# srvk/eesen

Measured on AMD Instinct MI355X. Metric: CTC training frames/sec (whole node), 4x512 BiLSTM, higher is better.
Workload: dtype f32

## Files before the change

eesen_amd/csrc/capi.cpp:

```cpp
#include <cstdio>
#include <cstring>

#include <algorithm>

#include "guard.h"
#include "net.h"

using namespace eesen;

#include "handles.h"

namespace eesen {
std::string& last_error_slot() {
  thread_local std::string g_err;
  return g_err;
}
}

extern "C" {

const char* eesen_last_error(void) { return last_error_slot().c_str(); }
const char* eesen_version(void) { return "eesen_hip 0.1.0 (gfx950)"; }

int eesen_device_count(int* count) {
// ... 107 lines not shown
}
int eesen_net_set_train_options(eesen_net_t* net, float learn_rate, float momentum) {
  return guard([&] { REQ_PTR(net); net->lr = learn_rate; net->mmt = momentum; });
}
int eesen_net_set_update_algorithm(eesen_net_t* net, const char* name) {
  return guard([&] {
    REQ_PTR(net); REQ_PTR(name);
    const std::string a(name);
    if (a == "SGD") net->rule = 0;
    else if (a == "Adagrad") net->rule = 1;
    else if (a == "RMSProp") net->rule = 2;
    else throw Error(EESEN_ERR_INVALID, "unknown optimization algorithm '" + a + "' (SGD|Adagrad|RMSProp)");
  });
}
int eesen_net_set_adaptive_options(eesen_net_t* net, float adagrad_epsilon, float rmsprop_rho) {
  return guard([&] { REQ_PTR(net); net->ada_eps = adagrad_epsilon; net->rms_rho = rmsprop_rho; net->rms_one_minus_rho = 1.0f - rmsprop_rho; });
}
int eesen_net_get_accumulators(eesen_net_t* net, float* host_flat, long n) {
  return guard([&] { REQ_PTR(net); REQ_PTR(host_flat); net->init_accu(); net->get_flat(net->accu, host_flat, n); });
}
int eesen_net_set_accumulators(eesen_net_t* net, const float* host_flat, long n) {
  return guard([&] { REQ_PTR(net); REQ_PTR(host_flat); net->set_accu(host_flat, n); });
}
int eesen_net_set_seq_lengths(eesen_net_t* net, const int* lens, int S) {
  return guard([&] { REQ_PTR(net); REQ_PTR(lens); net->set_seq_lengths(lens, S); });
}
int eesen_net_propagate(eesen_net_t* net, const float* in, int rows, int in_ld, int in_is_device, const float** out_dev,
                        int* out_cols, int* out_ld) {
  return guard([&] {
    REQ_PTR(net); REQ_PTR(in);
    net->propagate(in, rows, in_ld, in_is_device != 0);
    if (out_dev) *out_dev = net->out_ptr;
    if (out_cols) *out_cols = net->out_cols;
    if (out_ld) *out_ld = net->out_ld;
  });
}
int eesen_net_get_output(eesen_net_t* net, float* host_out, long n) {
  return guard([&] {
    REQ_PTR(net); REQ_PTR(host_out);
    EESEN_REQUIRE(net->propagated, EESEN_ERR_STATE, "no Propagate output");
    EESEN_REQUIRE(n == (long)net->rows * net->out_cols, EESEN_ERR_INVALID, "output size mismatch");
    net->sync();
    EESEN_HIP_CHECK(hipMemcpy2D(host_out, (size_t)net->out_cols * 4, net->out_ptr, (size_t)net->out_ld * 4, (size_t)net->out_cols * 4,
                                net->rows, hipMemcpyDeviceToHost));
  });
}
int eesen_net_backpropagate(eesen_net_t* net, const float* out_diff_dev, int out_diff_ld, float* in_diff_dev, int in_diff_ld) {
  return guard([&] { REQ_PTR(net); REQ_PTR(out_diff_dev); net->backpropagate(out_diff_dev, out_diff_ld, in_diff_dev, in_diff_ld); });
}
int eesen_net_grad_buffer(eesen_net_t* net, float** dev_ptr, long* n) {
  return guard([&] { REQ_PTR(net); REQ_PTR(dev_ptr); REQ_PTR(n); *dev_ptr = net->fresh.p; *n = (long)net->P; });
}
int eesen_net_get_grads(eesen_net_t* net, float* host_flat, long n) {
  return guard([&] { REQ_PTR(net); REQ_PTR(host_flat); net->get_flat(net->fresh, host_flat, n); });
}
int eesen_net_update(eesen_net_t* net) {
  return guard([&] { REQ_PTR(net); net->update(); });
}
int eesen_net_set_forward_precision(eesen_net_t* net, int bf16) {
  return guard([&] { REQ_PTR(net); net->fwd_bf16 = bf16 != 0; net->fwd_bf16_rec = bf16 == 1; });
}
int eesen_net_bf16_recurrence_layers(eesen_net_t* net, int* layers) {
  return guard([&] { REQ_PTR(net); REQ_PTR(layers); *layers = net->info_fwd_bf16; });
}
int eesen_net_plan_string(eesen_net_t* net, char* json, int cap) {
  return guard([&] {
    REQ_PTR(net); REQ_PTR(json);
    const std::string s = net->plan_string();
    EESEN_REQUIRE(cap > (int)s.size(), EESEN_ERR_INVALID, "eesen_net_plan_string: buffer too small (" + std::to_string(s.size() + 1) + " bytes needed)");
    std::memcpy(json, s.c_str(), s.size() + 1);
  });
}
int eesen_net_recurrence_info(eesen_net_t* net, int* out3) {
  return guard([&] {
    REQ_PTR(net); REQ_PTR(out3);
    out3[0] = net->info_lstm_layers; out3[1] = net->info_fwd_persistent; out3[2] = net->info_bwd_persistent;
    out3[3] = net->recoveries;
  });
}
int eesen_net_debug_set_error_word(eesen_net_t* net, unsigned value) {
  return guard([&] {
    REQ_PTR(net);
    EESEN_HIP_CHECK(hipSetDevice(net->device));
    EESEN_HIP_CHECK(hipMemsetD32Async(reinterpret_cast<hipDeviceptr_t>(net->ctl.p + kCtlWords - 1), (int)value, 1, net->st));
  });
}
int eesen_net_synchronize(eesen_net_t* net) {
  return guard([&] { REQ_PTR(net); net->sync(); });
}
int eesen_net_set_profiling(eesen_net_t* net, int on) {
  return guard([&] { REQ_PTR(net); net->timer.enable(on != 0); net->timer.set_accumulate(on == 2); });
}
int eesen_net_get_phase_spans(eesen_net_t* net, int* phases, float* seconds, int cap, int* n) {
  return guard([&] { REQ_PTR(net); REQ_PTR(n); *n = net->timer.spans(phases, seconds, cap); });
}
int eesen_net_get_phase_times(eesen_net_t* net, float* out6) {
  return guard([&] { REQ_PTR(net); REQ_PTR(out6); net->timer.collect(out6, 6); });
}

int eesen_ctc_create(int device, void* stream, eesen_ctc_t** out) {
  return guard([&] { REQ_PTR(out); *out = new eesen_ctc(device, stream); });
}
int eesen_ctc_destroy(eesen_ctc_t* ctc) {
  return guard([&] { delete ctc; });
}
int eesen_ctc_eval_parallel(eesen_ctc_t* ctc, const int* frame_num_utt, int S, const float* net_out_dev, int rows, int K,
                            int ld, const int* label_ids, const int* label_off, float* diff_dev, int diff_ld,
                            float* pzx_host) {
  return guard([&] {
    REQ_PTR(ctc); REQ_PTR(frame_num_utt); REQ_PTR(net_out_dev); REQ_PTR(label_ids); REQ_PTR(label_off); REQ_PTR(diff_dev);
    ctc->eval_parallel(frame_num_utt, S, net_out_dev, rows, K, ld, label_ids, label_off, diff_dev, diff_ld, pzx_host);
  });
}
int eesen_ctc_error_rate_mseq(eesen_ctc_t* ctc, const int* frame_num_utt, int S, const float* net_out_dev, int rows, int K,
                              int ld, const int* label_ids, const int* label_off, int* num_err, int* num_ref) {
  return guard([&] {
    REQ_PTR(ctc); REQ_PTR(frame_num_utt); REQ_PTR(net_out_dev); REQ_PTR(label_ids); REQ_PTR(label_off);
    ctc->error_rate_mseq(frame_num_utt, S, net_out_dev, rows, K, ld, label_ids, label_off, num_err, num_ref);
  });
}
int eesen_ctc_stats(eesen_ctc_t* ctc, double* obj_sum, long* sequences, long* frames, long* err_tokens, long* ref_tokens) {
  return guard([&] {
    REQ_PTR(ctc);
    ctc->flush();
    if (obj_sum) *obj_sum = ctc->obj_sum;
    if (sequences) *sequences = ctc->sequences;
    if (frames) *frames = ctc->frames;
    if (err_tokens) *err_tokens = ctc->err_tokens;
    if (ref_tokens) *ref_tokens = ctc->ref_tokens;
  });
}
int eesen_ctc_get_alpha_beta(eesen_ctc_t* ctc, float* alpha_host, float* beta_host, int* Lprime) {
  return guard([&] { REQ_PTR(ctc); ctc->get_alpha_beta(alpha_host, beta_host, Lprime); });
}
int eesen_ctc_set_sequence_out_file(eesen_ctc_t* ctc, const char* path) {
  return guard([&] {
    REQ_PTR(ctc);
    ctc->flush();
    ctc->seq_out = path ? path : "";
    if (!ctc->seq_out.empty()) std::remove(ctc->seq_out.c_str());
  });
}
int eesen_ctc_set_guard(eesen_ctc_t* ctc, eesen_net_t* net) {
  return guard([&] {
    REQ_PTR(ctc);
    ctc->flush();
    if (net) EESEN_REQUIRE(net->device == ctc->device && net->st == ctc->st, EESEN_ERR_INVALID, "eesen_ctc_set_guard: the Ctc and the Net must live on the same device and stream");
    if (ctc->guard_net) {
      auto& g = ctc->guard_net->guards;
      g.erase(std::remove(g.begin(), g.end(), static_cast<Ctc*>(ctc)), g.end());
    }
    ctc->guard = net && net->ctl.p ? net->ctl.p + kCtlWords - 1 : nullptr;
    ctc->guard_net = ctc->guard ? net : nullptr;
    if (ctc->guard_net) net->guards.push_back(ctc);
  });
}
int eesen_ctc_dropped(eesen_ctc_t* ctc, long* minibatches) {
  return guard([&] { REQ_PTR(ctc); REQ_PTR(minibatches); ctc->flush(); *minibatches = ctc->dropped; });
}
int eesen_ctc_set_profiling(eesen_ctc_t* ctc, int mode) {
  return guard([&] { REQ_PTR(ctc); ctc->timer.enable(mode == 2); ctc->timer.set_accumulate(mode == 2); });
}
int eesen_ctc_get_phase_times(eesen_ctc_t* ctc, float* out3) {
  return guard([&] { REQ_PTR(ctc); REQ_PTR(out3); ctc->phase_times(out3); });
}

int eesen_ce_create(int device, void* stream, eesen_ce_t** out) {
  return guard([&] { REQ_PTR(out); *out = new eesen_ce(device, stream); });
}
int eesen_ce_destroy(eesen_ce_t* ce) {
  return guard([&] { delete ce; });
}
int eesen_ce_eval_parallel(eesen_ce_t* ce, const int* frame_num_utt, int S, const float* net_out_dev, int rows, int K, int ld,
                           const int* targets_host, float* diff_dev, int diff_ld, double* obj_host) {
  return guard([&] {
    REQ_PTR(ce); REQ_PTR(frame_num_utt); REQ_PTR(net_out_dev); REQ_PTR(targets_host); REQ_PTR(diff_dev);
    ce->eval_parallel(frame_num_utt, S, net_out_dev, rows, K, ld, targets_host, diff_dev, diff_ld, obj_host);
  });
}
int eesen_ce_set_report_step(eesen_ce_t* ce, int report_step) {
  return guard([&] { REQ_PTR(ce); ce->flush(); ce->report_step = report_step; });
}
int eesen_ce_stats(eesen_ce_t* ce, double* obj, long* correct, long* frames, long* sequences) {
  return guard([&] {
    REQ_PTR(ce);
    ce->flush();
    if (obj) *obj = ce->obj;
    if (correct) *correct = ce->correct;
    if (frames) *frames = ce->frames;
    if (sequences) *sequences = ce->sequences;
  });
}
int eesen_ce_report(eesen_ce_t* ce, char* buf, int cap) {
  return guard([&] {
    REQ_PTR(ce); REQ_PTR(buf);
    const std::string s = ce->report();
    EESEN_REQUIRE(cap > (int)s.size(), EESEN_ERR_INVALID, "eesen_ce_report: buffer too small (" + std::to_string(s.size() + 1) + " bytes needed)");
    std::memcpy(buf, s.c_str(), s.size() + 1);
  });
}
int eesen_ce_progress(eesen_ce_t* ce, int wait, char* buf, int cap) {
  return guard([&] {
    REQ_PTR(ce); REQ_PTR(buf);
    EESEN_REQUIRE(cap > 0, EESEN_ERR_INVALID, "eesen_ce_progress: no buffer");
    if (wait) ce->flush();
    if (ce->progress.empty()) { buf[0] = 0; return; }
    const std::string& s = ce->progress.front();
    EESEN_REQUIRE(cap > (int)s.size(), EESEN_ERR_INVALID, "eesen_ce_progress: buffer too small (" + std::to_string(s.size() + 1) + " bytes needed)");
    std::memcpy(buf, s.c_str(), s.size() + 1);
    ce->progress.erase(ce->progress.begin());
  });
}
int eesen_ce_set_guard(eesen_ce_t* ce, eesen_net_t* net) {
  return guard([&] {
    REQ_PTR(ce);
    ce->flush();
    if (net) EESEN_REQUIRE(net->device == ce->device && net->st == ce->st, EESEN_ERR_INVALID, "eesen_ce_set_guard: the CE and the Net must live on the same device and stream");
    if (ce->guard_net) {
      auto& g = ce->guard_net->ce_guards;
      g.erase(std::remove(g.begin(), g.end(), static_cast<CeLoss*>(ce)), g.end());
    }
    ce->guard = net && net->ctl.p ? net->ctl.p + kCtlWords - 1 : nullptr;
    ce->guard_net = ce->guard ? net : nullptr;
    if (ce->guard_net) net->ce_guards.push_back(ce);
  });
}
int eesen_ce_dropped(eesen_ce_t* ce, long* minibatches) {
  return guard([&] { REQ_PTR(ce); REQ_PTR(minibatches); ce->flush(); *minibatches = ce->dropped; });
}
int eesen_ce_set_profiling(eesen_ce_t* ce, int mode) {
  return guard([&] { REQ_PTR(ce); ce->timer.enable(mode == 2); ce->timer.set_accumulate(mode == 2); });
}
int eesen_ce_get_phase_times(eesen_ce_t* ce, float* out1) {
  return guard([&] { REQ_PTR(ce); REQ_PTR(out1); ce->phase_times(out1); });
}

int eesen_dev_alloc(int device, long bytes, void** dev_ptr) {
  return guard([&] {
    REQ_PTR(dev_ptr);
    EESEN_HIP_CHECK(hipSetDevice(device));
    EESEN_HIP_CHECK(hipMalloc(dev_ptr, (size_t)bytes));
  });
}
int eesen_dev_free(int device, void* dev_ptr) {
  return guard([&] {
    EESEN_HIP_CHECK(hipSetDevice(device));
    EESEN_HIP_CHECK(hipFree(dev_ptr));
  });
}
int eesen_dev_copy(int device, void* dst, const void* src, long bytes, int kind) {
  return guard([&] {
    EESEN_HIP_CHECK(hipSetDevice(device));
    const hipMemcpyKind k = kind == 1 ? hipMemcpyHostToDevice : kind == 2 ? hipMemcpyDeviceToHost : hipMemcpyDeviceToDevice;
    EESEN_HIP_CHECK(hipMemcpy(dst, src, (size_t)bytes, k));
  });
}

int eesen_op_gemm(int device, void* stream, int a_kc, int b_kc, int M, int N, int K, float alpha, const float* A, int lda,
                  const float* B, int ldb, float beta, float* C, int ldc, const float* bias) {
  return guard([&] {
    EESEN_HIP_CHECK(hipSetDevice(device));
    hipStream_t st = reinterpret_cast<hipStream_t>(stream);
    DevBuf<float> ws;
    ws.reserve((size_t)8 << 20);
    gemm_f32(st, a_kc != 0, b_kc != 0, M, N, K, alpha, A, lda, B, ldb, beta, C, ldc, bias, ws.p, ws.cap);
    EESEN_HIP_CHECK(hipStreamSynchronize(st));
  });
}

int eesen_op_gemm_async(int device, void* stream, int a_kc, int b_kc, int M, int N, int K, const float* A, int lda, const float* B, int ldb,
                        float* C, int ldc, float* ws, long ws_floats, int extra_lds_bytes) {
  return guard([&] {
    REQ_PTR(A); REQ_PTR(B); REQ_PTR(C);
    EESEN_REQUIRE(ws_floats >= 0 && (ws || ws_floats == 0) && extra_lds_bytes >= 0, EESEN_ERR_INVALID, "bad workspace / LDS cap");
    EESEN_HIP_CHECK(hipSetDevice(device));
    gemm_f32(reinterpret_cast<hipStream_t>(stream), a_kc != 0, b_kc != 0, M, N, K, 1.f, A, lda, B, ldb, 0.f, C, ldc, nullptr, ws, (size_t)ws_floats,
             extra_lds_bytes);
  });
}

int eesen_op_log_sub_prior(int device, void* stream, float* m_dev, int rows, int cols, int ld, int apply_log,
                           const float* log_priors_host, float prior_scale) {
  return guard([&] {
    REQ_PTR(m_dev);
    EESEN_HIP_CHECK(hipSetDevice(device));
    hipStream_t st = reinterpret_cast<hipStream_t>(stream);
    DevBuf<float> pri;
    if (log_priors_host) {
      pri.reserve(cols);
      EESEN_HIP_CHECK(hipMemcpyAsync(pri.p, log_priors_host, sizeof(float) * cols, hipMemcpyHostToDevice, st));
    }
    log_sub_prior(st, m_dev, ld, rows, cols, apply_log != 0, log_priors_host ? pri.p : nullptr, prior_scale);
    EESEN_HIP_CHECK(hipStreamSynchronize(st));
  });
}

int eesen_op_gemm_bench(int device, int a_kc, int b_kc, int M, int N, int K, const float* A, int lda, const float* B, int ldb,
                        float* C, int ldc, int iters, float* avg_ms) {
  return guard([&] {
    REQ_PTR(avg_ms);
    EESEN_HIP_CHECK(hipSetDevice(device));
    DevBuf<float> ws;
    ws.reserve((size_t)16 << 20);
    hipEvent_t e0, e1;
    EESEN_HIP_CHECK(hipEventCreate(&e0));
// ... 34 lines not shown
```

eesen_amd/csrc/comm.cpp:

```cpp
#include <arpa/inet.h>
#include <dlfcn.h>
#include <netdb.h>
#include <netinet/in.h>
#include <netinet/tcp.h>
#include <sys/socket.h>
#include <unistd.h>

#include <algorithm>
#include <atomic>
#include <chrono>
#include <condition_variable>
#include <cstring>
#include <deque>
#include <mutex>
#include <thread>

#include <rccl/rccl.h>

#include "guard.h"
#include "handles.h"
#include "net.h"

namespace eesen {

// ... 339 lines not shown
      double v[kScratch] = {0};
      if (rank >= base && rank < base + n) v[rank - base] = mine;
      allreduce_host(v, n, 0);
      ids.insert(ids.end(), v, v + n);
    }
    std::vector<double> uniq(ids);
    std::sort(uniq.begin(), uniq.end());
    const int distinct = (int)(std::unique(uniq.begin(), uniq.end()) - uniq.begin());
    std::string o = "{\"library\": \"" + rccl().path + "\", \"rccl_version\": " + std::to_string(version) + ", \"stand_in\": " + (rccl().stand_in ? "true" : "false") +
                    ", \"rank\": " + std::to_string(rank) + ", \"world\": " + std::to_string(world) + ", \"world_seen\": " + std::to_string(seen) +
                    ", \"rank_seen\": " + std::to_string(nccl_rank) + ", \"device\": " + std::to_string(device) + ", \"device_seen\": " + std::to_string(nccl_dev) + ", \"devices\": [";
    for (int r = 0; r < world; ++r) {
      const unsigned long long u = (unsigned long long)(ids[r] - 1.0);
      char t[64];
      snprintf(t, sizeof(t), "%s\"%05x/%04x:%02x:%02x.%x\"", r ? ", " : "", (unsigned)((u >> 32) & 0xfffffu), (unsigned)((u >> 16) & 0xffffu), (unsigned)((u >> 8) & 0xffu),
               (unsigned)((u >> 3) & 0x1fu), (unsigned)(u & 7u));
      o += t;
    }
    o += "], \"distinct_devices\": " + std::to_string(distinct) + ", \"ranks_share_devices\": " + (distinct < world ? "true" : "false") + "}";
    return o;
  }
  void abort_now(const std::string& why) {
    std::unique_lock<std::mutex> lk(mu);
    if (dead.load()) return;
    dead_msg = "data-parallel exchange aborted on rank " + std::to_string(rank) + ": " + why;
    fprintf(stderr, "ERROR (eesen_hip) %s\n", dead_msg.c_str());
    dead.store(true, std::memory_order_release);
    ncclComm_t c = comm;
    comm = nullptr;
    lk.unlock();
    if (rccl().CommAbort && c) (void)rccl().CommAbort(c);
  }
};

void comm_check_alive(const Comm* c) {
  if (c) c->check_alive();
}

void Net::set_comm(Comm* c) {
  EESEN_REQUIRE(finalized, EESEN_ERR_STATE, "net not finalized");
  EESEN_REQUIRE(!c || c->device == device, EESEN_ERR_INVALID, "communicator and net live on different devices");
  wait_buckets_host();
  comm = c;
  if (c && !tn.spin_limit_set) spin_limit = std::max(spin_limit, 4000000);
  if (c && ev_ready.size() < layers.size()) {
    EESEN_HIP_CHECK(hipSetDevice(device));
    const size_t old = ev_ready.size();
    ev_ready.resize(layers.size(), nullptr);
    ev_bucket.resize(layers.size(), nullptr);
    for (size_t i = old; i < layers.size(); ++i) {
      EESEN_HIP_CHECK(hipEventCreateWithFlags(&ev_ready[i], hipEventDisableTiming));
      EESEN_HIP_CHECK(hipEventCreateWithFlags(&ev_bucket[i], hipEventDisableTiming));
    }
  }
  bucket_pending.assign(layers.size(), 0);
}

int Net::top_trainable() const {
  for (int li = (int)layers.size() - 1; li >= 0; --li)
    if (layers[li].p_n) return li;
  return -1;
}

void Net::bucket_allreduce(int li, hipStream_t producer) {
  if (!comm || !layers[li].p_n) return;
  bucket_log.push_back(li);
  EESEN_HIP_CHECK(hipEventRecord(ev_ready[li], producer));
  if (exchange_deferred) { deferred_buckets.push_back(li); return; }
  issue_bucket(li);
}

void Net::flush_deferred_buckets() {
  if (!comm || deferred_buckets.empty()) return;
  if (!ev_bwd_done) EESEN_HIP_CHECK(hipEventCreateWithFlags(&ev_bwd_done, hipEventDisableTiming));
  EESEN_HIP_CHECK(hipEventRecord(ev_bwd_done, st));
  EESEN_HIP_CHECK(hipStreamWaitEvent(comm->st, ev_bwd_done, 0));
  for (int li : deferred_buckets) issue_bucket(li);
  deferred_buckets.clear();
}

void Net::issue_bucket(int li) {
  EESEN_HIP_CHECK(hipStreamWaitEvent(comm->st, ev_ready[li], 0));
  const bool top = li == top_trainable();
  if (ctl.p) zero_if_set(comm->st, fresh.p + layers[li].p_off, (long)(layers[li].p_n + (top ? kLiveWords : 0)), ctl.p + kCtlWords - 1);
  grads_sanitized = true;
  const int ti_ = timer.begin(comm->st, 6);
  comm->allreduce_f32(fresh.p + layers[li].p_off, layers[li].p_n + (top ? kLiveWords : 0), comm->st);
  timer.end(comm->st, ti_);
  EESEN_HIP_CHECK(hipEventRecord(ev_bucket[li], comm->st));
  bucket_pending[li] = 1;
}

void Net::fail_step_buckets() noexcept {
  if (!comm) return;
  try {
    EESEN_HIP_CHECK(hipSetDevice(device));
    std::vector<char> logged(layers.size(), 0);
    for (int li : bucket_log) logged[li] = 1;
    flush_deferred_buckets();
    if (!ev_bwd_done) EESEN_HIP_CHECK(hipEventCreateWithFlags(&ev_bwd_done, hipEventDisableTiming));
    for (hipStream_t s : {st, st2}) {
      if (!s) continue;
      EESEN_HIP_CHECK(hipEventRecord(ev_bwd_done, s));
      EESEN_HIP_CHECK(hipStreamWaitEvent(comm->st, ev_bwd_done, 0));
    }
    const int top = top_trainable();
    for (int li = (int)layers.size() - 1; li >= 0; --li) {
      if (!layers[li].p_n || logged[li]) continue;
      const size_t n = layers[li].p_n + (li == top ? kLiveWords : 0);
      EESEN_HIP_CHECK(hipMemsetAsync(fresh.p + layers[li].p_off, 0, n * sizeof(float), comm->st));
      bucket_log.push_back(li);
      EESEN_HIP_CHECK(hipEventRecord(ev_ready[li], comm->st));
      issue_bucket(li);
    }
    fprintf(stderr, "WARNING (eesen_hip) Backpropagate failed on this rank in a data-parallel step: its unfinished gradient buckets were "
                    "all-reduced as zeros so that the other ranks are not left waiting\n");
  } catch (...) {
    try { comm->abort_now("Backpropagate failed and the step's remaining gradient buckets could not be issued"); } catch (...) {}
  }
}

void Net::wait_buckets_host() {
  if (!comm) return;
  bool any = false;
  for (char p : bucket_pending) any |= p != 0;
  if (any) EESEN_HIP_CHECK(hipStreamSynchronize(comm->st));
  comm->check_alive();
}

void Net::backpropagate_zero() {
  EESEN_REQUIRE(finalized, EESEN_ERR_STATE, "net not finalized");
  comm_check_alive(comm);
  EESEN_HIP_CHECK(hipSetDevice(device));
  if (P) EESEN_HIP_CHECK(hipMemsetAsync(fresh.p, 0, (P + kLiveWords) * sizeof(float), st));
  bucket_log.clear();
  deferred_buckets.clear();
  exchange_deferred = false;
  live_valid = comm != nullptr;
  for (int li = (int)layers.size() - 1; li >= 0; --li) bucket_allreduce(li, st);
  flush_deferred_buckets();
}

int Net::live_ranks() {
  EESEN_REQUIRE(finalized && comm, EESEN_ERR_STATE, "live_ranks needs an attached communicator");
  comm->check_alive();
  EESEN_HIP_CHECK(hipSetDevice(device));
  const int top = top_trainable();
  EESEN_REQUIRE(top >= 0, EESEN_ERR_STATE, "the net has no trainable layer");
  if (bucket_pending[top]) EESEN_HIP_CHECK(hipStreamWaitEvent(st, ev_bucket[top], 0));
  if (!live_pin) EESEN_HIP_CHECK(hipHostMalloc(reinterpret_cast<void**>(&live_pin), sizeof(float), hipHostMallocDefault));
  EESEN_HIP_CHECK(hipMemcpyAsync(live_pin, fresh.p + P, sizeof(float), hipMemcpyDeviceToHost, st));
  EESEN_HIP_CHECK(hipStreamSynchronize(st));
  comm->check_alive();
  return (int)(*live_pin + 0.5f);
}

void Net::allreduce_grads(Comm* c) {
  EESEN_REQUIRE(finalized, EESEN_ERR_STATE, "net not finalized");
  EESEN_REQUIRE(c && c->device == device, EESEN_ERR_INVALID, "communicator missing or on another device");
  EESEN_HIP_CHECK(hipSetDevice(device));
  if (ctl.p) zero_if_set(st, fresh.p, (long)P, ctl.p + kCtlWords - 1);
  grads_sanitized = true;
  c->allreduce_f32(fresh.p, P, st);
}

}

using namespace eesen;
struct eesen_comm : public Comm { using Comm::Comm; };

extern "C" {

int eesen_comm_get_unique_id(char* id128) {
  return guard([&] {
    REQ_PTR(id128);
    ncclUniqueId id;
    EESEN_NCCL_CHECK(rccl().GetUniqueId(&id));
    std::memcpy(id128, id.internal, NCCL_UNIQUE_ID_BYTES);
  });
}
int eesen_comm_exchange(const char* addr, int port, int rank, int world, char* buf, int nbytes, int timeout_s) {
  return guard([&] { REQ_PTR(buf); comm_exchange(addr, port, rank, world, buf, nbytes, timeout_s); });
}
int eesen_comm_create(int device, const char* id128, int rank, int world, eesen_comm_t** out) {
  return guard([&] { REQ_PTR(id128); REQ_PTR(out); *out = new eesen_comm(device, id128, rank, world); });
}
int eesen_comm_create_tcp(int device, const char* addr, int port, int rank, int world, int timeout_s, eesen_comm_t** out) {
  return guard([&] {
    REQ_PTR(out);
    char id[NCCL_UNIQUE_ID_BYTES] = {0};
    if (rank == 0) {
      ncclUniqueId u;
      EESEN_NCCL_CHECK(rccl().GetUniqueId(&u));
      std::memcpy(id, u.internal, NCCL_UNIQUE_ID_BYTES);
    }
    comm_exchange(addr, port, rank, world, id, NCCL_UNIQUE_ID_BYTES, timeout_s);
    *out = new eesen_comm(device, id, rank, world);
  });
}
int eesen_comm_destroy(eesen_comm_t* comm) {
  return guard([&] { delete comm; });
}
int eesen_comm_info(eesen_comm_t* comm, int* rank, int* world) {
  return guard([&] { REQ_PTR(comm); if (rank) *rank = comm->rank; if (world) *world = comm->world; });
}
int eesen_comm_describe(eesen_comm_t* comm, char* json, int cap) {
  return guard([&] {
    REQ_PTR(comm); REQ_PTR(json);
    const std::string s = comm->describe();
    EESEN_REQUIRE(cap > (int)s.size(), EESEN_ERR_INVALID, "eesen_comm_describe: buffer too small (" + std::to_string(s.size() + 1) + " bytes needed)");
    std::memcpy(json, s.c_str(), s.size() + 1);
  });
}
int eesen_comm_allreduce_host(eesen_comm_t* comm, double* values, int n, int op) {
  return guard([&] { REQ_PTR(comm); REQ_PTR(values); comm->allreduce_host(values, n, op); });
}
int eesen_net_set_comm(eesen_net_t* net, eesen_comm_t* comm) {
  return guard([&] { REQ_PTR(net); net->set_comm(comm); });
}
int eesen_net_allreduce_grads(eesen_net_t* net, eesen_comm_t* comm) {
  return guard([&] { REQ_PTR(net); net->allreduce_grads(comm); });
}
int eesen_net_backpropagate_zero(eesen_net_t* net) {
  return guard([&] { REQ_PTR(net); net->backpropagate_zero(); });
}
int eesen_net_live_ranks(eesen_net_t* net, int* live) {
  return guard([&] { REQ_PTR(net); REQ_PTR(live); *live = net->live_ranks(); });
}
int eesen_net_bucket_order(eesen_net_t* net, int* layers_out, int cap, int* n) {
  return guard([&] {
    REQ_PTR(net); REQ_PTR(n);
    *n = (int)net->bucket_log.size();
    for (int i = 0; i < *n && i < cap && layers_out; ++i) layers_out[i] = net->bucket_log[i];
  });
}

}
```

eesen_amd/csrc/gemm.hip:

```cpp
#include <cstring>
#include <mutex>
#include <type_traits>

#include "kernels.h"

namespace eesen {
namespace {

constexpr int BM = 128, BN = 128, BK = 16, LDP = 4;
constexpr int NLD = BM * BK / 4 / 256;
constexpr int KQ_BITS = BK == 16 ? 2 : 3;
typedef float f32x16 __attribute__((ext_vector_type(16)));

struct GemmParams {
  const float* A;
  const float* B;
  float* C;
  const float* bias;
  int M, N, K;
  int lda, ldb, ldc;
  float alpha, beta;
  int splits;
  int k_chunk;
  int tiles_n;
// ... 633 lines not shown
      unsigned m0 = 0u, m1 = 0u;
#pragma unroll
      for (int j = 0; j < 8; ++j) {
        v[j].x &= 0x7fffffffu; v[j].y &= 0x7fffffffu; v[j].z &= 0x7fffffffu; v[j].w &= 0x7fffffffu;
        const unsigned mj = max(max(v[j].x, v[j].y), max(v[j].z, v[j].w));
        if (j < 4) m0 = max(m0, mj); else m1 = max(m1, mj);
        if (COLS) { uint4& q = cm[j & 3]; q.x = max(q.x, v[j].x); q.y = max(q.y, v[j].y); q.z = max(q.z, v[j].z); q.w = max(q.w, v[j].w); }
      }
      if (ROWS || ALL) {
#pragma unroll
        for (int o = 32; o > 0; o >>= 1) { m0 = max(m0, (unsigned)__shfl_xor((int)m0, o)); m1 = max(m1, (unsigned)__shfl_xor((int)m1, o)); }
        if (ROWS && lane == 0) {
          if (nslab > 1 || row_acc) { atomicMax(&out_rows[r], m0); if (two) atomicMax(&out_rows[r + rstep], m1); }
          else { out_rows[r] = m0; if (two) out_rows[r + rstep] = m1; }
        }
        all = max(all, max(m0, m1));
      }
    }
    if (COLS) {
#pragma unroll
      for (int j = 0; j < 4; ++j) {
        const int c = c0 + 256 * j;
        if (c < C) { atomicMax(&smax[c], cm[j].x); atomicMax(&smax[c + 1], cm[j].y); atomicMax(&smax[c + 2], cm[j].z); atomicMax(&smax[c + 3], cm[j].w); }
      }
    }
  } else {
    for (long r = (long)blockIdx.x * kAmaxWaves + wave; r < R; r += (long)gridDim.x * kAmaxWaves) {
      const float* row = P + r * ld;
      unsigned m = 0u;
      for (int c = lane; c < C; c += 64) {
        const unsigned v = __builtin_bit_cast(unsigned, row[c]) & 0x7fffffffu;
        m = max(m, v);
        if (COLS) atomicMax(&smax[c], v);
      }
      if (ROWS || ALL) {
#pragma unroll
        for (int o = 32; o > 0; o >>= 1) m = max(m, (unsigned)__shfl_xor((int)m, o));
        if (ROWS && lane == 0) { if (row_acc) atomicMax(&out_rows[r], m); else out_rows[r] = m; }
        all = max(all, m);
      }
    }
  }
  if (COLS) {
    __syncthreads();
    for (int c = tid; c < Cp; c += kAmaxWaves * 64) part_cols[(size_t)blockIdx.x * Cp + c] = smax[c];
  }
  if (ALL) {
    unsigned* red = smax + (COLS ? Cp : 0);
    __syncthreads();
    if (lane == 0) red[wave] = all;
    __syncthreads();
    if (tid == 0) {
      unsigned m = 0u;
      for (int w = 0; w < kAmaxWaves; ++w) m = max(m, red[w]);
      if (m) atomicMax(out_all, m);
    }
  }
}
__global__ __launch_bounds__(256) void amax_fold_kernel(const unsigned* __restrict__ part, int nb, int Cp, int C, unsigned* __restrict__ out) {
  __shared__ uint4 red[16][16];
  const int cq = threadIdx.x & 15, g = threadIdx.x >> 4;
  const int c = blockIdx.x * 64 + cq * 4;
  uint4 m = make_uint4(0u, 0u, 0u, 0u);
  if (c < Cp)
    for (int b = g; b < nb; b += 16 * 8) {
      uint4 v[8];
#pragma unroll
      for (int k = 0; k < 8; ++k) v[k] = b + 16 * k < nb ? *reinterpret_cast<const uint4*>(part + (size_t)(b + 16 * k) * Cp + c) : make_uint4(0u, 0u, 0u, 0u);
#pragma unroll
      for (int k = 0; k < 8; ++k) { m.x = max(m.x, v[k].x); m.y = max(m.y, v[k].y); m.z = max(m.z, v[k].z); m.w = max(m.w, v[k].w); }
    }
  red[g][cq] = m;
  __syncthreads();
  if (g == 0 && c < Cp) {
#pragma unroll
    for (int k = 1; k < 16; ++k) { const uint4 o = red[k][cq]; m.x = max(m.x, o.x); m.y = max(m.y, o.y); m.z = max(m.z, o.z); m.w = max(m.w, o.w); }
    if (c + 0 < C) out[c + 0] = m.x;
    if (c + 1 < C) out[c + 1] = m.y;
    if (c + 2 < C) out[c + 2] = m.z;
    if (c + 3 < C) out[c + 3] = m.w;
  }
}

__global__ __launch_bounds__(256) void splitk_reduce_kernel(const float* __restrict__ ws, int splits, int M, int N,
                                                            float alpha, float beta, float* __restrict__ C, int ldc,
                                                            const float* __restrict__ bias) {
  const size_t total = (size_t)M * N;
  for (size_t i = (size_t)blockIdx.x * blockDim.x + threadIdx.x; i < total; i += (size_t)gridDim.x * blockDim.x) {
    float s = 0.f;
    for (int k = 0; k < splits; ++k) s += ws[(size_t)k * total + i];
    const int row = (int)(i / N), col = (int)(i % N);
    float v = alpha * s + (bias ? bias[col] : 0.f);
    float* dst = C + (size_t)row * ldc + col;
    if (beta != 0.f) v += beta * *dst;
    *dst = v;
  }
}

}

static int g_gemm_mode = -1;
int gemm_mode() {
  if (g_gemm_mode >= 0) return g_gemm_mode;
  const char* e = getenv("EESEN_GEMM_MODE");
  if (e && (!strcmp(e, "f32") || !strcmp(e, "0"))) return 0;
  if (e && (!strcmp(e, "split") || !strcmp(e, "1"))) return 1;
  if (e && (!strcmp(e, "half") || !strcmp(e, "2"))) return 2;
  return kDefaultGemmMode;
}
void set_gemm_mode(int mode) { g_gemm_mode = mode; }

void amax_abs(hipStream_t st, const float* P, long rows, int cols, int ld, float* out) {
  EESEN_HIP_CHECK(hipMemsetAsync(out, 0, sizeof(float), st));
  amax_abs_accumulate(st, P, rows, cols, ld, out);
}
static int amax_blocks(long rows, int slabs) { return (int)std::max<long>(1, std::min<long>((rows * slabs + 2 * kAmaxWaves - 1) / (2 * kAmaxWaves), kAmaxBlocks)); }
#define EESEN_AMAX_LAUNCH(R_, C_, A_, LDS)                                                                                                        \
  do {                                                                                                                                            \
    if (vec) hipLaunchKernelGGL((amax_kernel<R_, C_, A_, true>), dim3(nb), dim3(kAmaxWaves * 64), LDS, st, Pc, rows, cc, ld, r, w, a, racc);     \
    else hipLaunchKernelGGL((amax_kernel<R_, C_, A_, false>), dim3(nb), dim3(kAmaxWaves * 64), LDS, st, Pc, rows, cc, ld, r, w, a, racc);        \
  } while (0)
constexpr int kAmaxSlabCols = 16384;
void amax_abs_accumulate(hipStream_t st, const float* P, long rows, int cols, int ld, float* out) {
  if (rows <= 0 || cols <= 0) return;
  if (cols == ld && cols < 1024 && (rows * cols) % 1024 == 0) { rows = rows * cols / 1024; cols = ld = 1024; }
  unsigned *r = nullptr, *w = nullptr, *a = reinterpret_cast<unsigned*>(out);
  const int racc = 0;
  const bool vec = (cols & 3) == 0 && (ld & 3) == 0;
  for (int c0 = 0; c0 < cols; c0 += kAmaxSlabCols) {
    const float* Pc = P + c0;
    const int cc = std::min(kAmaxSlabCols, cols - c0), nb = amax_blocks(rows, vec ? (cc + 1023) / 1024 : 1);
    EESEN_AMAX_LAUNCH(false, false, true, kAmaxWaves * sizeof(unsigned));
  }
  check_launch("amax_abs");
}
void amax_rows_cols(hipStream_t st, const float* P, long rows, int cols, int ld, float* out_rows, float* out_cols, float* ws) {
  if (rows <= 0 || cols <= 0) return;
  EESEN_REQUIRE(!out_cols || ws, EESEN_ERR_INVALID, "amax: column bounds need a workspace");
  unsigned* r = reinterpret_cast<unsigned*>(out_rows);
  unsigned* w = reinterpret_cast<unsigned*>(ws);
  unsigned* a = nullptr;
  const bool vec = (cols & 3) == 0 && (ld & 3) == 0;
  const bool multi = out_rows && ((vec && cols > 1024) || cols > kAmaxSlabCols);
  if (multi) EESEN_HIP_CHECK(hipMemsetAsync(out_rows, 0, (size_t)rows * sizeof(float), st));
  for (int c0 = 0; c0 < cols; c0 += kAmaxSlabCols) {
    const float* Pc = P + c0;
    const int cc = std::min(kAmaxSlabCols, cols - c0), racc = multi ? 1 : 0;
    const int nb = amax_blocks(rows, vec ? (cc + 1023) / 1024 : 1);
    const int cp = (cc + 3) & ~3;
    if (out_rows && out_cols) EESEN_AMAX_LAUNCH(true, true, false, (size_t)cp * sizeof(unsigned));
    else if (out_cols) EESEN_AMAX_LAUNCH(false, true, false, (size_t)cp * sizeof(unsigned));
    else if (out_rows) EESEN_AMAX_LAUNCH(true, false, false, 0);
    check_launch("amax_rows_cols");
    if (out_cols) {
      hipLaunchKernelGGL(amax_fold_kernel, dim3((cp + 63) / 64), dim3(256), 0, st, w, nb, cp, cc, reinterpret_cast<unsigned*>(out_cols) + c0);
      check_launch("amax_fold");
    }
  }
}
#undef EESEN_AMAX_LAUNCH

static GemmBound arena_bound(hipStream_t st, const float* P, bool kc, int R, int K, int ld) {
  constexpr size_t kArena = (size_t)4 << 20, kDevs = 16;
  static std::mutex mu;
  static float* arena[kDevs] = {nullptr};
  static size_t next[kDevs] = {0};
  int dev = 0;
  EESEN_HIP_CHECK(hipGetDevice(&dev));
  EESEN_REQUIRE(dev >= 0 && dev < (int)kDevs, EESEN_ERR_INVALID, "gemm: device index beyond the bounds arena table");
  const size_t need = ((size_t)R + 3) & ~(size_t)3;
  EESEN_REQUIRE(need <= kArena / 8, EESEN_ERR_INVALID, "gemm: operand too large for the bounds arena");
  float* slot;
  {
    std::lock_guard<std::mutex> lk(mu);
    if (!arena[dev]) EESEN_HIP_CHECK(hipMalloc(reinterpret_cast<void**>(&arena[dev]), kArena * sizeof(float)));
    if (next[dev] + need > kArena) next[dev] = 0;
    slot = arena[dev] + next[dev];
    next[dev] += need;
  }
  if (kc) amax_rows_cols(st, P, R, K, ld, slot, nullptr, nullptr);
  else {
    float* ws = nullptr;
    EESEN_HIP_CHECK(hipMallocAsync(reinterpret_cast<void**>(&ws), (size_t)kAmaxBlocks * std::min<size_t>(need, kAmaxSlabCols) * sizeof(float), st));
    amax_rows_cols(st, P, K, R, ld, nullptr, slot, ws);
    EESEN_HIP_CHECK(hipFreeAsync(ws, st));
  }
  return GemmBound{slot, 1};
}

static int xcd_group_rows(int tiles_m, int tiles_n, unsigned* grid_x) {
  if (tiles_m < 8) return 0;
  int gm = 8;
  while (gm > 1 && cdiv(tiles_m, gm) < 16) gm >>= 1;
  const long groups = cdiv(tiles_m, gm), rounds = cdivl(groups, 8);
  const long gx = rounds * 8 * gm * tiles_n;
  if (gx > 0x7fffffffL) return 0;
  *grid_x = (unsigned)gx;
  return gm;
}

void gemm_f32(hipStream_t st, bool a_kc, bool b_kc, int M, int N, int K, float alpha, const float* A, int lda,
              const float* B, int ldb, float beta, float* C, int ldc, const float* bias, float* ws, size_t ws_floats,
              int extra_lds_bytes, bool bf16_operands, GemmBound bound_a, GemmBound bound_b) {
  if (M <= 0 || N <= 0) return;
  EESEN_REQUIRE((lda % 4) == 0 && (ldb % 4) == 0, EESEN_ERR_INVALID, "gemm: leading dimensions must be multiples of 4");
  EESEN_REQUIRE((((uintptr_t)A | (uintptr_t)B) & 15) == 0, EESEN_ERR_INVALID, "gemm: operands must be 16-byte aligned");
  const bool use_split = gemm_mode() >= 1 || bf16_operands;
  const bool half = gemm_mode() == 2 && !bf16_operands;
  GemmParams p;
  p.amax_a = p.amax_b = nullptr;
  p.a_vec = p.b_vec = 0;
  if (half) {
    if (!bound_a.p) bound_a = arena_bound(st, A, a_kc, M, K, lda);
    if (!bound_b.p) bound_b = arena_bound(st, B, b_kc, N, K, ldb);
    p.amax_a = bound_a.p; p.a_vec = bound_a.per_index;
    p.amax_b = bound_b.p; p.b_vec = bound_b.per_index;
  }
  p.A = A; p.B = B; p.C = C; p.bias = bias;
  p.M = M; p.N = N; p.K = K; p.lda = lda; p.ldb = ldb; p.ldc = ldc;
  p.alpha = alpha; p.beta = beta;
  p.gate = GemmGate{nullptr, nullptr, 0, 0, 0, 0, 0, 0};
  p.nprod = bf16_operands ? 1 : 6;
  const bool big = use_split && !bf16_operands && extra_lds_bytes == 0 && M % 256 == 0 && N % 256 == 0 && K % 16 == 0 &&
                   (long)(M / 256) * (N / 256) >= 16;
  const int TB = big ? 256 : BM;
  p.bm = p.bn = TB;
  const int tiles_m = cdiv(M, TB), tiles_n = cdiv(N, TB);
  p.tiles_n = tiles_n;
  p.tiles_m = tiles_m;
  const long tiles = (long)tiles_m * tiles_n;
  int splits = 1;
  const int target = big ? 256 : 1024;
  if (ws && tiles < target && K >= 2048) {
    splits = (int)std::min<long>((target + tiles - 1) / tiles, K / 1024);
    splits = std::max(1, std::min(splits, 64));
    while (splits > 1 && (size_t)splits * M * N > ws_floats) --splits;
  }
  int k_chunk = cdiv(cdiv(K, splits), 16) * 16;
  if (k_chunk < BK) k_chunk = BK;
  splits = std::max(1, cdiv(K, k_chunk));
  p.splits = splits;
  p.k_chunk = k_chunk;
  if (splits > 1) p.C = ws;
// ... 74 lines not shown
```

eesen_amd/csrc/kernels.h:

```cpp
#pragma once
#include "common.h"

namespace eesen {

struct GemmBound {
  const float* p = nullptr;
  int per_index = 0;
};
void gemm_f32(hipStream_t st, bool a_kc, bool b_kc, int M, int N, int K, float alpha, const float* A, int lda,
              const float* B, int ldb, float beta, float* C, int ldc, const float* bias, float* ws,
              size_t ws_floats, int extra_lds_bytes = 0,
              bool bf16_operands = false,
              GemmBound bound_a = {}, GemmBound bound_b = {});

constexpr int kDefaultGemmMode = 2;
int gemm_mode();
void set_gemm_mode(int mode);
void amax_abs(hipStream_t st, const float* P, long rows, int cols, int ld, float* out);
void amax_abs_accumulate(hipStream_t st, const float* P, long rows, int cols, int ld, float* out);
constexpr int kAmaxBlocks = 512;
void amax_rows_cols(hipStream_t st, const float* P, long rows, int cols, int ld, float* out_rows, float* out_cols, float* ws);

#ifndef EESEN_SHARDS
#define EESEN_SHARDS 8
#endif
constexpr int kShards = EESEN_SHARDS, kShardStride = 32;
constexpr int kCtlHalf = 2048 * kShards;

struct GemmGate {
  const unsigned* cnt;
  unsigned* err;
  int ndir, nz, nblk;
  int T, S;
  int spin_limit;
};
void gemm_f32_nt_gated(hipStream_t st, int M, int N, int K, const float* A, int lda, const float* B, int ldb, float* C,
                       int ldc, const float* bias, const GemmGate& gate, GemmBound bound_a = {}, GemmBound bound_b = {});

struct LstmLayerDev {
  int T, S, H, ndir;
  float* G;
  float* C;
  float* Y;
  float* X = nullptr;
  const float* Wm;
  const float* WmT;
  const float* peep;
  const int* lens;
  const float* rmask = nullptr;
  int drop_mode = 0;
  int s_begin = 0, s_count = 0;
  float* PX = nullptr;
  size_t px_floats = 0;
  int poll_delay = 0;
  int poll_raw = 0;
  unsigned* milestone = nullptr;
  int milestone_step = 0;
  int xcd_map = 1, fwd_mux = 1, bwd_q4 = 1, bwd_ksplit = 1, bwd_mux = 1;
  int fwd_t16_small = 1;
  int fwd_narrow2 = 1;
  int bwd_q4_st8 = 1;
  int fwd_bf16 = 0;
  int fwd_split = 0;
  int fwd_f16 = 0;
  const float* wm_amax = nullptr;
  int bwd_f16 = 0;
  unsigned char* DGH = nullptr;
  float* EX = nullptr;
};
float handoff_flight_ns();
void set_gpu_share(int n);
int gpu_share_value();
void wait_for_word(hipStream_t st, const unsigned* word, unsigned target, unsigned* err, double limit_s = 2.0);
void lstm_fwd_step(hipStream_t st, const LstmLayerDev& L, int step);
void lstm_bwd_step(hipStream_t st, const LstmLayerDev& L, int step, const float* dY, int lddy, float* DG, float* DCF);
void dropout_mask(hipStream_t st, float* out, long rows, int cols, int ld, float p, unsigned long long seed, bool per_column);
void activation_rows(hipStream_t st, bool tanh_, const float* x, int ldx, float* y, int ldy, long rows, int cols);
void activation_diff_rows(hipStream_t st, bool tanh_, const float* y, int ldy, float* d, int ldd, long rows, int cols);
void mul_elements(hipStream_t st, const float* a, int lda, const float* m, int ldm, float* out, int ldo, long rows, int cols);
enum { kRecNone = 0, kRecFwdBf = 1, kRecFwdMux = 2, kRecFwdF32 = 3, kRecBwdQ4 = 4, kRecBwdKsplit = 5, kRecBwdKsplitMux = 6, kRecBwdGeneric = 7 };
struct RecPlan {
  int kind = kRecNone;
  const char* kernel = "";
  int seq_tile = 0;
  int units = 0;
  int windows = 0;
  int grid[3] = {0, 0, 0};
  int wgs = 0;
  int wgs_per_cu = 0;
  int vgprs = 0, lds = 0;
  int free_vgprs = -1;
  int seq_tiles = 1;
  bool one_window = false;
  bool leaves_room = false;
  bool bf16 = false;
  bool light = false;
  size_t need_px = 0, need_ex = 0;
  bool need_dgh = false;
  size_t ctl_words = 0;
  int chunk = 0;
  const void* fn = nullptr;
};
RecPlan lstm_fwd_plan(const LstmLayerDev& L);
RecPlan lstm_bwd_plan(const LstmLayerDev& L);
void lstm_fwd_launch(hipStream_t st, const RecPlan& plan, const LstmLayerDev& L, unsigned* cnt, unsigned* err, int spin_limit,
                     unsigned long long* trace = nullptr, hipEvent_t after_reset = nullptr);
void lstm_bwd_launch(hipStream_t st, const RecPlan& plan, const LstmLayerDev& L, const float* dY, int lddy, float* DG, unsigned* cnt,
                     unsigned* err, int spin_limit, unsigned long long* trace = nullptr);
void lstm_bias_peep_grads(hipStream_t st, const LstmLayerDev& L, const float* DG, float* bias_grad, float* peep_grad,
                          float* ws, size_t ws_floats);
size_t lstm_bias_peep_ws_floats(int T, int S, int H, int ndir);

void col_sums(hipStream_t st, const float* M, int rows, int cols, int ld, float* out, float* ws, size_t ws_floats);
size_t col_sums_ws_floats(int rows, int cols);

void softmax_rows(hipStream_t st, const float* x, int ldx, float* y, int ldy, int rows, int K);
void log_rows(hipStream_t st, const float* in, int ldi, float* out, int ldo, int rows, int K);
void ctc_alpha_beta(hipStream_t st, const float* logp, int ld, int T, int S, int Lpad, const int* labx, const int* lens,
                    const int* lablens, float* alpha, float* beta, float* pzx, int waves = 0);
int ctc_sweep_waves(int Lpad, int waves = 0);
void ctc_error_diff(hipStream_t st, const float* probs, int ld, int T, int S, int K, int Lpad, int Lmax, const int* lens,
                    const int* lablens, const int* labx, const float* alpha, const float* beta,
                    const float* pzx, float* diff, int ldd);
void log_sub_prior(hipStream_t st, float* m, int ld, int rows, int K, bool apply_log, const float* log_prior, float prior_scale);
void row_argmax(hipStream_t st, const float* m, int ld, int rows, int K, int* ids);

struct CeSums {
  double obj;
  long long correct;
};
int ce_eval_blocks(int rows);
void ce_eval(hipStream_t st, const float* y, int ld, int rows, int K, int S, const int* lens, const int* tgt, float* diff,
             int ldd, CeSums* part, CeSums* out);

void sgd_update(hipStream_t st, float* param, float* corr, const float* fresh, long n, float mmt, float lr_coef,
                float max_grad, const unsigned* skip = nullptr, const float* live = nullptr);
void zero_if_set(hipStream_t st, float* p, long n, const unsigned* word);
void adaptive_update(hipStream_t st, float* param, float* corr, const float* fresh, float* accu, long n, float mmt, float lr,
                     float max_grad, float eps, float rho, float one_minus_rho, bool rmsprop, const unsigned* skip = nullptr,
                     const float* live = nullptr);
void tensor_moments(hipStream_t st, const float* base, long rows, int cols, long ld, double* out6, double* ws,
                    int nb = 0, int hf = 0, int hi = 0);
void transpose2d(hipStream_t st, const float* src, int rows, int cols, float* dst);
void copy2d(hipStream_t st, const float* src, int lds, float* dst, int ldd, int rows, int cols);

}
```

eesen_amd/csrc/net.cpp:

```cpp
#include "net.h"

#include <algorithm>
#include <cmath>
#include <cstdio>
#include <cstring>

namespace eesen {


PhaseTimer::~PhaseTimer() {
  for (auto& s : spans_) {
    (void)hipEventDestroy(s.a);
    (void)hipEventDestroy(s.b);
  }
}
int PhaseTimer::begin(hipStream_t st, int phase) {
  if (!on_) return -1;
  if (used_ == spans_.size()) {
    Span s;
    EESEN_HIP_CHECK(hipEventCreate(&s.a));
    EESEN_HIP_CHECK(hipEventCreate(&s.b));
    spans_.push_back(s);
  }
  spans_[used_].phase = phase;
// ... 8 lines not shown
  for (int i = 0; i < nphase; ++i) out[i] = 0.f;
  for (size_t i = 0; i < used_; ++i) {
    EESEN_HIP_CHECK(hipEventSynchronize(spans_[i].b));
    float ms = 0.f;
    EESEN_HIP_CHECK(hipEventElapsedTime(&ms, spans_[i].a, spans_[i].b));
    if (spans_[i].phase >= 0 && spans_[i].phase < nphase) out[spans_[i].phase] += ms * 1e-3f;
  }
  if (accumulate_) used_ = 0;
}

int PhaseTimer::spans(int* phases, float* secs, int cap) {
  for (size_t i = 0; i < used_ && (int)i < cap; ++i) {
    EESEN_HIP_CHECK(hipEventSynchronize(spans_[i].b));
    float ms = 0.f;
    EESEN_HIP_CHECK(hipEventElapsedTime(&ms, spans_[i].a, spans_[i].b));
    if (phases) phases[i] = spans_[i].phase;
    if (secs) secs[i] = ms * 1e-3f;
  }
  return (int)used_;
}

long Layer::file_params() const {
  if (is_lstm()) return (long)ndir * ((long)4 * Hf * din_f + (long)4 * Hf * Hf + 4 * Hf + 3 * Hf);
  if (kind == EESEN_LAYER_AFFINE) return (long)dout_f * din_f + dout_f;
  return 0;
}

const char* Layer::marker() const {
  switch (kind) {
    case EESEN_LAYER_BILSTM_PARALLEL: return nonparallel ? "<BiLstm>" : "<BiLstmParallel>";
    case EESEN_LAYER_LSTM_PARALLEL: return nonparallel ? "<Lstm>" : "<LstmParallel>";
    case EESEN_LAYER_AFFINE: return "<AffineTransform>";
    case EESEN_LAYER_SOFTMAX: return "<Softmax>";
    case EESEN_LAYER_SIGMOID: return "<Sigmoid>";
    case EESEN_LAYER_TANH: return "<Tanh>";
  }
  return "<Unknown>";
}

template <class F>
static void for_each_param(const Layer& L, F f) {
  long fi = 0;
  if (L.is_lstm()) {
    const int H = L.H, Hf = L.Hf, D = L.din_f, D4 = pad4(L.din);
    for (int dir = 0; dir < L.ndir; ++dir) {
      for (int r = 0; r < 4 * Hf; ++r) {
        const int q = r / Hf, u = r % Hf;
        for (int d = 0; d < D; ++d) f(fi++, L.off_wx + ((size_t)dir * 4 * H + u * 4 + q) * D4 + L.in_col(d));
      }
      for (int r = 0; r < 4 * Hf; ++r) {
        const int q = r / Hf, u = r % Hf;
        for (int k = 0; k < Hf; ++k) f(fi++, L.off_wm + ((size_t)dir * 4 * H + u * 4 + q) * H + k);
      }
      for (int r = 0; r < 4 * Hf; ++r) f(fi++, L.off_bias + (size_t)dir * 4 * H + (r % Hf) * 4 + r / Hf);
      for (int g = 0; g < 3; ++g)
        for (int u = 0; u < Hf; ++u) f(fi++, L.off_peep + ((size_t)dir * 3 + g) * H + u);
    }
  } else if (L.kind == EESEN_LAYER_AFFINE) {
    const int D4 = pad4(L.din);
    for (int r = 0; r < L.dout; ++r)
      for (int d = 0; d < L.din_f; ++d) f(fi++, L.off_w + (size_t)r * D4 + L.in_col(d));
    for (int r = 0; r < L.dout; ++r) f(fi++, L.off_b + r);
  }
}

Net::Net(int dev, void* stream) : device(dev) {
  int n = 0;
  hipError_t e = hipGetDeviceCount(&n);
  if (e != hipSuccess || n <= 0)
    throw Error(EESEN_ERR_HIP, "no HIP device available: this library has no CPU fallback (hipGetDeviceCount: " +
                                   std::string(e == hipSuccess ? "0 devices" : hipGetErrorString(e)) + ")");
  EESEN_REQUIRE(dev >= 0 && dev < n, EESEN_ERR_INVALID, "device index out of range");
  EESEN_HIP_CHECK(hipSetDevice(dev));
  st = reinterpret_cast<hipStream_t>(stream);
  int lo = 0, hi = 0;
  EESEN_HIP_CHECK(hipDeviceGetStreamPriorityRange(&lo, &hi));
  EESEN_HIP_CHECK(hipStreamCreateWithPriority(&st2, hipStreamNonBlocking, lo));
  EESEN_HIP_CHECK(hipEventCreateWithFlags(&ev_rec, hipEventDisableTiming));
  for (auto& e : ev_grad) EESEN_HIP_CHECK(hipEventCreateWithFlags(&e, hipEventDisableTiming));
  EESEN_HIP_CHECK(hipEventCreateWithFlags(&ev_gate_reset, hipEventDisableTiming));
  EESEN_HIP_CHECK(hipEventCreateWithFlags(&ev_gate_done, hipEventDisableTiming));
  tn = Tuning::from_env();
  persistent = tn.persistent;
  gate_fwd = tn.gate_fwd >= 0 ? tn.gate_fwd != 0 : gemm_mode() == 0;
  overlap = tn.overlap >= 0 ? tn.overlap != 0 : persistent != 0;
  spin_limit = tn.spin_limit;
  if (tn.trace) {
    trace.reserve(1280);
    EESEN_HIP_CHECK(hipMemset(trace.p, 0, 1280 * sizeof(unsigned long long)));
  }
  ctl.reserve(kCtlWords);
  EESEN_HIP_CHECK(hipMemset(ctl.p, 0, kCtlWords * sizeof(unsigned)));
  {
    constexpr float kFwdNs = 400.f, kBwdNs = 280.f, kBwdSideNs = 420.f, kRefFlightNs = 400.f;
    flight_ns = handoff_flight_ns();
    const float fscale = flight_ns >= 300.f && flight_ns <= 700.f ? 1.f : flight_ns / kRefFlightNs;
    auto ticks = [&](float ns) { return std::min(300, std::max(0, (int)std::lround(fscale * ns / 10.f))); };
    delay_fwd = ticks(kFwdNs); delay_bwd = ticks(kBwdNs); delay_bwd_side = ticks(kBwdSideNs);
    if (const char* e = tn.poll_ns) {
      int a = -1, b2 = -1;
      if (sscanf(e, "%d,%d", &a, &b2) == 2) { delay_fwd = a / 10; delay_bwd = delay_bwd_side = b2 / 10; poll_raw = 1; }
    }
    if (tn.print_flight)
      fprintf(stderr, "eesen_hip: increment flight %.0f ns; first-poll delays forward %d0, backward %d0 (beside side-stream GEMMs %d0) ns\n", flight_ns, delay_fwd, delay_bwd, delay_bwd_side);
  }
}

Net::~Net() {
  (void)hipSetDevice(device);
  (void)hipStreamSynchronize(st);
  for (Ctc* c : guards) {
    (void)hipStreamSynchronize(c->st);
    c->guard = nullptr;
    c->guard_net = nullptr;
  }
  for (CeLoss* c : ce_guards) {
    (void)hipStreamSynchronize(c->st);
    c->guard = nullptr;
    c->guard_net = nullptr;
  }
  if (trace.p) {
    std::vector<unsigned long long> h(1280);
    if (hipMemcpy(h.data(), trace.p, h.size() * 8, hipMemcpyDeviceToHost) == hipSuccess)
      for (int pass = 0; pass < 2; ++pass) {
        double seg[5] = {0, 0, 0, 0, 0};
        int n = 0;
        for (int s = 8; s < 120; ++s) {
          const unsigned long long* a = h.data() + pass * 640 + s * 5;
          if (!a[0] || !a[5]) continue;
          seg[0] += (double)(a[1] - a[0]); seg[1] += (double)(a[2] - a[1]); seg[2] += (double)(a[3] - a[2]);
          seg[3] += (double)(a[4] - a[3]); seg[4] += (double)(a[5] - a[4]);
          ++n;
        }
        if (n) fprintf(stderr, "EESEN_TRACE %s: wait %.0f | A-load+MFMA+reduce %.0f | epilogue %.0f | drain+barrier %.0f | publish->next %.0f ticks/step (%d steps)\n",
                       pass ? "bwd" : "fwd", seg[0] / n, seg[1] / n, seg[2] / n, seg[3] / n, seg[4] / n, n);
      }
  }
  if (lens_pin) (void)hipHostFree(lens_pin);
  if (err_pin) (void)hipHostFree(err_pin);
  if (live_pin) (void)hipHostFree(live_pin);
  for (auto& h : in_stage) { if (h.p) (void)hipHostFree(h.p); if (h.ev) (void)hipEventDestroy(h.ev); }
  if (lens_ev) (void)hipEventDestroy(lens_ev);
  if (err_ev) (void)hipEventDestroy(err_ev);
  if (st2) { (void)hipStreamSynchronize(st2); (void)hipStreamDestroy(st2); }
  if (ev_rec) (void)hipEventDestroy(ev_rec);
  for (auto& e : ev_grad) if (e) (void)hipEventDestroy(e);
  if (ev_gate_reset) (void)hipEventDestroy(ev_gate_reset);
  if (ev_gate_done) (void)hipEventDestroy(ev_gate_done);
  for (auto& e : ev_ready) if (e) (void)hipEventDestroy(e);
  for (auto& e : ev_bucket) if (e) (void)hipEventDestroy(e);
  if (ev_bwd_done) (void)hipEventDestroy(ev_bwd_done);
  if (own_stream) (void)hipStreamDestroy(st);
}

void Net::sync() {
  EESEN_HIP_CHECK(hipSetDevice(device));
  EESEN_HIP_CHECK(hipStreamSynchronize(st));
  wait_buckets_host();
  comm_check_alive(comm);
  check_device_error(true);
}

void Net::check_device_error(bool consumer) {
  if (!ctl.p) return;
  unsigned e = 0;
  EESEN_HIP_CHECK(hipMemcpy(&e, ctl.p + kCtlWords - 1, sizeof(unsigned), hipMemcpyDeviceToHost));
  if (!e) { steps_since_clean = 0; return; }
  EESEN_HIP_CHECK(hipStreamSynchronize(st));
  EESEN_HIP_CHECK(hipMemset(ctl.p + kCtlWords - 1, 0, sizeof(unsigned)));
  const bool only_waiter = e == 2 && tn.fwd_mid;
  if (only_waiter) tn.fwd_mid = 0;
  else { persistent = 0; gate_fwd = false; overlap = false; }
  ++recoveries;
  const int lost = std::max(1, steps_since_clean);
  steps_since_clean = 0;
  const bool rerun = consumer && propagated && input.p && rows > 0;
  const char* what = comm ? "contributed a ZERO gradient to the data-parallel sum (the ranks' models stay identical)" : "were NOT applied";
  if (only_waiter)
    fprintf(stderr, "WARNING (eesen_hip) the side stream's wait for a forward-recurrence milestone gave up (kernels serialised by a tool?): "
                    "%d minibatch(es) in flight %s%s; continuing without the early input GEMM (EESEN_FWD_MID=0)\n", lost, what,
            rerun ? " and the last forward pass is re-run" : "");
  else
    fprintf(stderr, "WARNING (eesen_hip) a persistent recurrence kernel gave up waiting for a peer workgroup (GPU shared or preempted?): "
                    "%d minibatch(es) in flight %s%s; continuing with the one-launch-per-step kernels\n", lost, what,
            rerun ? " and the last forward pass is re-run" : "");
  if (rerun) {
    forward_pass();
    EESEN_HIP_CHECK(hipStreamSynchronize(st));
  }
}

void Net::arm_device_error_poll() {
  if (!ctl.p) return;
  if (!err_pin) {
    EESEN_HIP_CHECK(hipHostMalloc(reinterpret_cast<void**>(&err_pin), sizeof(unsigned), hipHostMallocDefault));
    *err_pin = 0;
    EESEN_HIP_CHECK(hipEventCreateWithFlags(&err_ev, hipEventDisableTiming));
  }
  EESEN_HIP_CHECK(hipMemcpyAsync(err_pin, ctl.p + kCtlWords - 1, sizeof(unsigned), hipMemcpyDeviceToHost, st));
  EESEN_HIP_CHECK(hipEventRecord(err_ev, st));
  err_armed = true;
}

void Net::poll_device_error() {
  if (!err_armed || hipEventQuery(err_ev) != hipSuccess) return;
  err_armed = false;
  if (*err_pin) check_device_error(false);
  else steps_since_clean = 0;
}

void Net::add_layer(int kind, int din, int dout, float coef, float max_grad) {
  EESEN_REQUIRE(!finalized, EESEN_ERR_STATE, "net already finalized");
  EESEN_REQUIRE(din > 0 && dout > 0, EESEN_ERR_INVALID, "layer dimensions must be positive");
  const Layer* prev = layers.empty() ? nullptr : &layers.back();
  if (prev)
    EESEN_REQUIRE(prev->dout_f == din, EESEN_ERR_INVALID, "Dimensionality mismatch between consecutive layers");
  Layer L;
  L.kind = kind; L.coef = coef; L.max_grad = max_grad;
  L.din_f = din; L.dout_f = dout;
  L.din = prev ? prev->dout : din;
  if (prev) { L.in_nb = prev->out_nb; L.in_hf = prev->out_hf; L.in_hi = prev->out_hi; }
  L.dout = dout;
  const char* sees_pad = "directly on an LSTM layer whose cell count per direction is not a multiple of 4 is not supported: it would see the "
                         "zero cells the library pads such a layer with";
  switch (kind) {
    case EESEN_LAYER_BILSTM_PARALLEL:
      EESEN_REQUIRE(dout % 2 == 0, EESEN_ERR_INVALID, "<CellDim> of a BiLstm layer must be even");
      L.ndir = 2; L.Hf = dout / 2;
      break;
    case EESEN_LAYER_LSTM_PARALLEL:
      L.ndir = 1; L.Hf = dout;
      break;
    case EESEN_LAYER_AFFINE:
      break;
    case EESEN_LAYER_SOFTMAX:
      EESEN_REQUIRE(din == dout, EESEN_ERR_INVALID, "Softmax needs InputDim == OutputDim");
      if (L.in_nb) throw Error(EESEN_ERR_INVALID, std::string("a <Softmax> ") + sees_pad);
      break;
    case EESEN_LAYER_SIGMOID:
    case EESEN_LAYER_TANH:
      EESEN_REQUIRE(din == dout, EESEN_ERR_INVALID, "an activation layer needs InputDim == OutputDim");
      if (L.in_nb && kind == EESEN_LAYER_SIGMOID) throw Error(EESEN_ERR_INVALID, std::string("a <Sigmoid> ") + sees_pad + " (sigmoid(0) = 1/2)");
      L.dout = L.din;
      L.out_nb = L.in_nb; L.out_hf = L.in_hf; L.out_hi = L.in_hi;
      break;
    default:
      throw Error(EESEN_ERR_INVALID, "unsupported layer kind " + std::to_string(kind));
  }
  if (L.is_lstm()) {
    L.H = pad4(L.Hf);
    L.dout = L.ndir * L.H;
    if (L.H != L.Hf) { L.out_nb = L.ndir; L.out_hf = L.Hf; L.out_hi = L.H; }
  }
  layers.push_back(std::move(L));
}

void Net::finalize() {
  EESEN_REQUIRE(!finalized, EESEN_ERR_STATE, "net already finalized");
  EESEN_REQUIRE(!layers.empty(), EESEN_ERR_INVALID, "empty net");
  EESEN_HIP_CHECK(hipSetDevice(device));
  size_t off = 0;
  for (Layer& L : layers) {
    L.p_off = off;
    size_t n = 0;
    if (L.is_lstm()) {
      const size_t H = L.H, D4 = pad4(L.din), nd = L.ndir;
      L.off_wx = n;   n += nd * 4 * H * D4;
      L.off_bias = n; n += nd * 4 * H;
      L.off_wm = n;   n += nd * 4 * H * H;
      L.off_peep = n; n += nd * 3 * H;
      L.WmT.reserve(nd * H * 4 * H);
    } else if (L.kind == EESEN_LAYER_AFFINE) {
      L.off_w = n; n += (size_t)L.dout * pad4(L.din);
      L.off_b = n; n += pad4(L.dout);
    }
    L.p_n = (n + 3) & ~(size_t)3;
    off += L.p_n;
  }
  P = off;
  if (P) {
    params.reserve(P); corr.reserve(P); fresh.reserve(P + kLiveWords);
    EESEN_HIP_CHECK(hipMemsetAsync(params.p, 0, P * sizeof(float), st));
    EESEN_HIP_CHECK(hipMemsetAsync(corr.p, 0, P * sizeof(float), st));
    EESEN_HIP_CHECK(hipMemsetAsync(fresh.p, 0, (P + kLiveWords) * sizeof(float), st));
  }
  if (tn.overlap < 0)
    for (const Layer& L : layers)
      if (L.is_lstm() && L.H > 512) overlap = false;
  amax.reserve(1 + layers.size());
  EESEN_HIP_CHECK(hipMemsetAsync(amax.p, 0, amax.cap * sizeof(float), st));
  EESEN_HIP_CHECK(hipMemsetD32Async(reinterpret_cast<hipDeviceptr_t>(amax.p), 0x3f800000, 1, st));
  finalized = true;
  refresh_derived();
  sync();
}

void Net::measure(const float* Pm, long nrows, int cols, int ld, DevBuf<float>& out_rows, DevBuf<float>& out_cols) {
  out_rows.reserve((size_t)nrows);
  out_cols.reserve((size_t)cols);
  amax_ws.reserve((size_t)kAmaxBlocks * std::min(16384, (cols + 3) & ~3));
  amax_rows_cols(st, Pm, nrows, cols, ld, out_rows.p, out_cols.p, amax_ws.p);
}
bool Net::x_is_bounded(int li) const {
  if (li == 0) return false;
  const Layer& Pv = layers[li - 1];
  return (Pv.is_lstm() && !Pv.cur_fwd_drop) || Pv.is_activation() || Pv.kind == EESEN_LAYER_SOFTMAX;
}
void Net::ensure_weight_amax() {
  const bool mode2 = gemm_mode() == 2;
  const bool need_w = mode2 && !wamax_valid;
  if (wm_valid && !need_w) return;
  if (!wm_valid) EESEN_HIP_CHECK(hipMemsetAsync(am_wm(0), 0, layers.size() * sizeof(float), st));
  for (size_t li = 0; li < layers.size(); ++li) {
    Layer& L = layers[li];
    if (L.is_lstm()) {
      if (need_w) measure(params.p + L.p_off + L.off_wx, (long)L.ndir * 4 * L.H, pad4(L.din), pad4(L.din), L.bw.rows, L.bw.cols);
      if (!wm_valid) amax_abs_accumulate(st, params.p + L.p_off + L.off_wm, (long)L.ndir * 4 * L.H, L.H, L.H, am_wm((int)li));
    } else if (L.kind == EESEN_LAYER_AFFINE && need_w) measure(params.p + L.p_off + L.off_w, L.dout, pad4(L.din), pad4(L.din), L.bw.rows, L.bw.cols);
  }
  wm_valid = true;
  if (mode2) wamax_valid = true;
}

long Net::num_params() const {
  long n = 0;
  for (const Layer& L : layers) n += L.file_params();
  return n;
}

void Net::init_accu() {
  if (accu_init) return;
  accu.reserve(P);
  EESEN_HIP_CHECK(hipMemsetAsync(accu.p, 0, P * sizeof(float), st));
  accu_init = true;
}

void Net::refresh_derived() {
  wamax_valid = wm_valid = false;
  for (Layer& L : layers)
    if (L.is_lstm())
      for (int dir = 0; dir < L.ndir; ++dir)
        transpose2d(st, params.p + L.p_off + L.off_wm + (size_t)dir * 4 * L.H * L.H, 4 * L.H, L.H,
                    L.WmT.p + (size_t)dir * L.H * 4 * L.H);
}

int Net::tensor_moments(int which, int layer, double* out6_host, int cap_tensors) {
  EESEN_REQUIRE(finalized, EESEN_ERR_STATE, "net not finalized");
  EESEN_REQUIRE(layer >= 0 && layer < (int)layers.size(), EESEN_ERR_INVALID, "layer index out of range");
  EESEN_REQUIRE(which >= 0 && which <= 2, EESEN_ERR_INVALID, "which: 0 parameters, 1 momentum buffers, 2 accumulators");
  const Layer& L = layers[layer];
  struct Region { size_t off; long rows; int cols; long ld; int nb, hf, hi; };
  std::vector<Region> reg;
  if (L.is_lstm()) {
    const int H = L.H, Hf = L.Hf, D4 = pad4(L.din);
    for (int dir = 0; dir < L.ndir; ++dir) {
      reg.push_back({L.off_wx + (size_t)dir * 4 * H * D4, 4L * Hf, L.din_f, D4, L.in_nb, L.in_hf, L.in_hi});
      reg.push_back({L.off_wm + (size_t)dir * 4 * H * H, 4L * Hf, Hf, H, 0, 0, 0});
      reg.push_back({L.off_bias + (size_t)dir * 4 * H, 1, 4 * Hf, 4L * H, 0, 0, 0});
      for (int g = 0; g < 3; ++g) reg.push_back({L.off_peep + ((size_t)dir * 3 + g) * H, 1, Hf, H, 0, 0, 0});
    }
  } else if (L.kind == EESEN_LAYER_AFFINE) {
    reg.push_back({L.off_w, L.dout, L.din_f, pad4(L.din), L.in_nb, L.in_hf, L.in_hi});
    reg.push_back({L.off_b, 1, L.dout, L.dout, 0, 0, 0});
  }
  const int n = (int)reg.size();
  if (!out6_host || n == 0) return n;
  EESEN_REQUIRE(cap_tensors >= n, EESEN_ERR_INVALID, "moments buffer too small");
  EESEN_HIP_CHECK(hipSetDevice(device));
  if (which == 2) init_accu();
  sync();
  const float* base = (which == 0 ? params.p : which == 1 ? corr.p : accu.p) + L.p_off;
  DevBuf<double> d;
  d.reserve((size_t)n * 6 + 8);
  for (int i = 0; i < n; ++i)
    eesen::tensor_moments(st, base + reg[i].off, reg[i].rows, reg[i].cols, reg[i].ld, d.p + (size_t)i * 6, d.p + (size_t)n * 6, reg[i].nb, reg[i].hf, reg[i].hi);
  EESEN_HIP_CHECK(hipStreamSynchronize(st));
  EESEN_HIP_CHECK(hipMemcpy(out6_host, d.p, (size_t)n * 6 * sizeof(double), hipMemcpyDeviceToHost));
  return n;
}

static void upload_flat(Net& net, DevBuf<float>& dst, const float* host, long n) {
  EESEN_REQUIRE(net.finalized, EESEN_ERR_STATE, "net not finalized");
  EESEN_REQUIRE(n == net.num_params(), EESEN_ERR_INVALID, "parameter count mismatch");
  EESEN_HIP_CHECK(hipSetDevice(net.device));
  std::vector<float> h(net.P, 0.f);
  long base = 0;
  for (const Layer& L : net.layers) {
    for_each_param(L, [&](long fi, size_t io) { h[L.p_off + io] = host[base + fi]; });
    base += L.file_params();
  }
  net.sync();
  if (net.P) EESEN_HIP_CHECK(hipMemcpy(dst.p, h.data(), net.P * sizeof(float), hipMemcpyHostToDevice));
}

void Net::set_params(const float* host, long n) {
  upload_flat(*this, params, host, n);
  refresh_derived();
  sync();
}

void Net::set_accu(const float* host, long n) {
  init_accu();
  upload_flat(*this, accu, host, n);
}

void Net::get_flat(const DevBuf<float>& buf, float* host, long n) {
  EESEN_REQUIRE(finalized, EESEN_ERR_STATE, "net not finalized");
  EESEN_REQUIRE(n == num_params(), EESEN_ERR_INVALID, "parameter count mismatch");
  sync();
  std::vector<float> h(P);
  if (P) EESEN_HIP_CHECK(hipMemcpy(h.data(), buf.p, P * sizeof(float), hipMemcpyDeviceToHost));
  long base = 0;
  for (const Layer& L : layers) {
    for_each_param(L, [&](long fi, size_t io) { host[base + fi] = h[L.p_off + io]; });
    base += L.file_params();
  }
}

void Net::set_seq_lengths(const int* l, int s) {
  EESEN_REQUIRE(s > 0, EESEN_ERR_INVALID, "need at least one sequence");
  EESEN_HIP_CHECK(hipSetDevice(device));
  lens.assign(l, l + s);
  for (int v : lens) EESEN_REQUIRE(v >= 0, EESEN_ERR_INVALID, "negative sequence length");
  poll_device_error();
  lens_d.reserve(s);
  if ((size_t)s > lens_pin_cap) {
// ... 107 lines not shown
    }
  }
  L.cur_twiddle_coin = coin;
  const bool rec = (rnndrop || nml) && (!twiddle || !coin);
  const bool fwd = fwd_p > 0.f && (!twiddle || coin);
  if (rec) {
    EESEN_REQUIRE(rec_step != rec_seq, EESEN_ERR_INVALID,
                  "recurrent dropout needs exactly one of RecurrentTimeStepDropout / RecurrentSequenceDropout (bilstm-layer.h:102-113)");
    EESEN_REQUIRE(!(rnndrop && nml), EESEN_ERR_INVALID, "RNNDrop and NoMemLossDropout are mutually exclusive");
    const long mrows = (long)(T + 2) * S;
    L.rmask.reserve((size_t)mrows * ldY);
    if (!L.inj_rmask.empty()) {
      EESEN_REQUIRE((L.inj_rmask_rows == mrows || L.inj_rmask_rows == S) && (long)L.inj_rmask.size() == (long)L.inj_rmask_rows * ldY,
                    EESEN_ERR_INVALID, "injected recurrent mask has the wrong shape");
      const size_t chunk = (size_t)L.inj_rmask_rows * ldY;
      for (long r0 = 0; r0 < mrows; r0 += L.inj_rmask_rows)
        EESEN_HIP_CHECK(hipMemcpyAsync(L.rmask.p + (size_t)r0 * ldY, L.inj_rmask.data(), chunk * sizeof(float), hipMemcpyHostToDevice, net.st));
      EESEN_HIP_CHECK(hipStreamSynchronize(net.st));
    } else {
      dropout_mask(net.st, L.rmask.p, mrows, ldY, ldY, rec_p, net.drop_seed + (++net.drop_counter) * 0x632BE59BD9B4E019ull, rec_seq);
    }
    L.cur_drop_mode = rnndrop ? 2 : 1;
  }
  if (fwd) {
    L.fmask.reserve((size_t)net.rows * ldY);
    L.Yd.reserve((size_t)net.rows * ldY);
    if (!L.inj_fmask.empty()) {
      EESEN_REQUIRE((long)L.inj_fmask.size() == (long)net.rows * ldY, EESEN_ERR_INVALID, "injected forward mask has the wrong shape");
      EESEN_HIP_CHECK(hipMemcpyAsync(L.fmask.p, L.inj_fmask.data(), L.inj_fmask.size() * sizeof(float), hipMemcpyHostToDevice, net.st));
      EESEN_HIP_CHECK(hipStreamSynchronize(net.st));
    } else {
      dropout_mask(net.st, L.fmask.p, net.rows, ldY, ldY, fwd_p, net.drop_seed + (++net.drop_counter) * 0x632BE59BD9B4E019ull, fw_seq);
    }
    L.cur_fwd_drop = true;
  }
  L.inj_fmask.clear(); L.inj_rmask.clear(); L.inj_rmask_rows = 0; L.inj_coin = -1;
}

void Net::propagate(const float* in, int nrows, int ld, bool is_device) {
  EESEN_REQUIRE(finalized, EESEN_ERR_STATE, "net not finalized");
  EESEN_REQUIRE(S > 0, EESEN_ERR_STATE, "SetSeqLengths must precede Propagate");
  EESEN_REQUIRE(nrows > 0 && nrows % S == 0, EESEN_ERR_INVALID, "row count must be a positive multiple of the sequence count");
  const int D = layers[0].din, D4 = pad4(D);
  EESEN_REQUIRE(ld >= D, EESEN_ERR_INVALID, "input leading dimension smaller than InputDim");
  EESEN_HIP_CHECK(hipSetDevice(device));
  rows = nrows;
  T = rows / S;
  for (int v : lens) EESEN_REQUIRE(v <= T, EESEN_ERR_INVALID, "sequence length exceeds the number of frames");
  timer.reset();

  if (input.reserve((size_t)rows * D4) || D4 != D) EESEN_HIP_CHECK(hipMemsetAsync(input.p, 0, (size_t)rows * D4 * sizeof(float), st));
  if (is_device) {
    EESEN_HIP_CHECK(hipMemcpy2DAsync(input.p, (size_t)D4 * sizeof(float), in, (size_t)ld * sizeof(float), (size_t)D * sizeof(float), rows,
                                     hipMemcpyDeviceToDevice, st));
  } else {
    HostStage& hs = in_stage[in_stage_idx++ & 1];
    const size_t bytes = (size_t)rows * D * sizeof(float);
    if (!hs.ev) EESEN_HIP_CHECK(hipEventCreateWithFlags(&hs.ev, hipEventDisableTiming));
    if (hs.busy) { EESEN_HIP_CHECK(hipEventSynchronize(hs.ev)); hs.busy = false; }
    if (bytes > hs.cap) {
      if (hs.p) EESEN_HIP_CHECK(hipHostFree(hs.p));
      hs.p = nullptr;
      hs.cap = bytes + bytes / 4;
      EESEN_HIP_CHECK(hipHostMalloc(reinterpret_cast<void**>(&hs.p), hs.cap, hipHostMallocDefault));
    }
    for (int r = 0; r < rows; ++r) std::memcpy(hs.p + (size_t)r * D, in + (size_t)r * ld, (size_t)D * sizeof(float));
    EESEN_HIP_CHECK(hipMemcpy2DAsync(input.p, (size_t)D4 * sizeof(float), hs.p, (size_t)D * sizeof(float), (size_t)D * sizeof(float), rows,
                                     hipMemcpyHostToDevice, st));
    EESEN_HIP_CHECK(hipEventRecord(hs.ev, st));
    hs.busy = true;
  }
  forward_pass();
}

void Net::forward_pass() {
  const float* x = input.p;
  int ldx = pad4(layers[0].din);
  ++steps_since_clean;
  info_fwd_persistent = info_lstm_layers = info_fwd_bf16 = 0;
  bool g_gated = false;
  int gated_rows = 0;
  int mid_r0 = 0, mid_r1 = 0;
  const bool half = gemm_mode() == 2;
  ensure_weight_amax();
  amx_valid = half;
  for (Layer& L : layers) {
    const int li_ = (int)(&L - layers.data());
    GemmBound x_amax, w_amax;
    if (half && L.trainable()) {
      if (x_is_bounded(li_)) x_amax = bound_one();
      else { measure(x, rows, L.din, ldx, L.bx.rows, L.bx.cols); x_amax = GemmBound{L.bx.rows.p, 1}; }
      w_amax = GemmBound{L.bw.rows.p, 1};
    }
    if (L.is_lstm()) {
      const int H = L.H, nd = L.ndir, ldY = nd * H, ldG = nd * 4 * H;
      L.G.reserve((size_t)rows * ldG);
      const size_t state = (size_t)(T + 2) * S * ldY;
      L.C.reserve(state);
      L.Y.reserve(state);
      if (persistent && H % 32 == 0) L.X.reserve((size_t)T * nd * ((S + 15) / 16) * (size_t)(H / 32) * 768);
      const size_t blk = (size_t)S * ldY * sizeof(float);
      EESEN_HIP_CHECK(hipMemsetAsync(L.C.p, 0, blk, st));
      EESEN_HIP_CHECK(hipMemsetAsync(L.Y.p, 0, blk, st));
      EESEN_HIP_CHECK(hipMemsetAsync(L.C.p + (size_t)(T + 1) * S * ldY, 0, blk, st));
      EESEN_HIP_CHECK(hipMemsetAsync(L.Y.p + (size_t)(T + 1) * S * ldY, 0, blk, st));
      prepare_dropout(*this, L);
      if (g_gated) {
        if (gated_rows < rows) {
          const int ti_ = timer.begin(st, 0);
          gemm_f32(st, true, true, rows - gated_rows, ldG, L.din, 1.f, x + (size_t)gated_rows * ldx, ldx, params.p + L.p_off + L.off_wx,
                   pad4(L.din), 0.f, L.G.p + (size_t)gated_rows * ldG, ldG, params.p + L.p_off + L.off_bias, nullptr, 0, 0, fwd_bf16, x_amax, w_amax);
          timer.end(st, ti_);
        }
        EESEN_HIP_CHECK(hipStreamWaitEvent(st, ev_gate_done, 0));
        g_gated = false;
      } else if (mid_r1 > mid_r0) {
        const int ti_ = timer.begin(st, 0);
        const int parts[2][2] = {{0, mid_r0}, {mid_r1, rows}};
        for (const auto& pr : parts)
          if (pr[1] > pr[0])
            gemm_f32(st, true, true, pr[1] - pr[0], ldG, L.din, 1.f, x + (size_t)pr[0] * ldx, ldx, params.p + L.p_off + L.off_wx, pad4(L.din),
                     0.f, L.G.p + (size_t)pr[0] * ldG, ldG, params.p + L.p_off + L.off_bias, nullptr, 0, 0, fwd_bf16, x_amax, w_amax);
        timer.end(st, ti_);
        EESEN_HIP_CHECK(hipStreamWaitEvent(st, ev_gate_done, 0));
        mid_r0 = mid_r1 = 0;
      } else {
        const int ti_ = timer.begin(st, 0);
        gemm_f32(st, true, true, rows, ldG, L.din, 1.f, x, ldx, params.p + L.p_off + L.off_wx, pad4(L.din), 0.f, L.G.p, ldG,
                 params.p + L.p_off + L.off_bias, nullptr, 0, 0, fwd_bf16, x_amax, w_amax);
        timer.end(st, ti_);
      }
      Layer* nxt = (&L - layers.data()) + 1 < (long)layers.size() ? &layers[(&L - layers.data()) + 1] : nullptr;
      LstmLayerDev v = lstm_view(*this, L, T);
      const RecPlan fp = persistent ? lstm_fwd_plan(v) : RecPlan{};
      const bool pers = fp.kind != kRecNone;
      const bool plan_gate = pers && overlap && gate_fwd && !fwd_bf16 && !L.cur_fwd_drop && fp.units <= 8 && nxt && nxt->is_lstm() && T >= 2 && rows >= 128 &&
                             fp.one_window &&
                             (nxt->ndir * 4 * nxt->H) % 128 == 0 && ldY % 16 == 0 && nd * fp.seq_tiles * kShards <= 64;
      const int mile_step = (3 * T) / 4;
      const bool plan_mid = pers && overlap && tn.fwd_mid && !plan_gate && !L.cur_fwd_drop && fp.leaves_room && nd == 2 && nxt && nxt->is_lstm() &&
                            T >= 32 && mile_step + 1 < T && fp.one_window;
      { const int ti_ = timer.begin(st, 1);
      v.poll_delay = delay_fwd;
      v.poll_raw = poll_raw;
      if (plan_mid) {
        mile.reserve(32);
        EESEN_HIP_CHECK(hipMemsetAsync(mile.p, 0, 2 * sizeof(unsigned), st));
        EESEN_HIP_CHECK(hipEventRecord(ev_gate_reset, st));
        v.milestone = mile.p;
        v.milestone_step = mile_step;
      }
      if (pers) lstm_fwd_launch(st, fp, v, ctl.p, ctl.p + kCtlWords - 1, spin_limit, trace.p, plan_gate ? ev_gate_reset : nullptr);
      else
        for (int step = 0; step < T; ++step) lstm_fwd_step(st, v, step);
      info_fwd_persistent += pers ? 1 : 0;
      info_fwd_bf16 += fp.bf16 ? 1 : 0;
      ++info_lstm_layers;
      check_launch("lstm_fwd");
      timer.end(st, ti_);
      if (pers && plan_gate) {
        const int ldG2 = nxt->ndir * 4 * nxt->H;
        nxt->G.reserve((size_t)rows * ldG2);
        EESEN_HIP_CHECK(hipStreamWaitEvent(st2, ev_gate_reset, 0));
        const int tj_ = timer.begin(st2, 0);
        GemmGate gate{ctl.p, ctl.p + kCtlWords - 1, nd, fp.seq_tiles, fp.grid[0], T, S, spin_limit};
        gated_rows = rows / 128 * 128;
        gemm_f32_nt_gated(st2, gated_rows, ldG2, ldY, L.Y.p + (size_t)S * ldY, ldY, params.p + nxt->p_off + nxt->off_wx, pad4(nxt->din),
                          nxt->G.p, ldG2, params.p + nxt->p_off + nxt->off_bias, gate, half ? bound_one() : GemmBound{}, half ? GemmBound{nxt->bw.rows.p, 1} : GemmBound{});
        timer.end(st2, tj_);
        EESEN_HIP_CHECK(hipEventRecord(ev_gate_done, st2));
        g_gated = true;
      }
      if (plan_mid) {
        EESEN_HIP_CHECK(hipMemsetD32Async(reinterpret_cast<hipDeviceptr_t>(mile.p + 1), 1, 1, st));
        const int ldG2 = nxt->ndir * 4 * nxt->H;
        nxt->G.reserve((size_t)rows * ldG2);
        mid_r0 = ((T - 1 - mile_step) * S + 255) / 256 * 256;
        mid_r1 = (mile_step + 1) * S / 256 * 256;
        if (mid_r1 <= mid_r0) mid_r0 = mid_r1 = 0;
      }
      if (plan_mid && mid_r1 > mid_r0) {
        const int ldG2 = nxt->ndir * 4 * nxt->H;
        EESEN_HIP_CHECK(hipStreamWaitEvent(st2, ev_gate_reset, 0));
        wait_for_word(st2, mile.p + 1, 1u, ctl.p + kCtlWords - 1, 2.0 * std::max(1.0, T / 1000.0) * std::max(1.0, spin_limit / 400000.0));
        const int tj_ = timer.begin(st2, 0);
        gemm_f32(st2, true, true, mid_r1 - mid_r0, ldG2, nxt->din, 1.f, L.Y.p + (size_t)S * ldY + (size_t)mid_r0 * ldY, ldY,
                 params.p + nxt->p_off + nxt->off_wx, pad4(nxt->din), 0.f, nxt->G.p + (size_t)mid_r0 * ldG2, ldG2,
                 params.p + nxt->p_off + nxt->off_bias, nullptr, 0,  64, fwd_bf16,
                 half ? bound_one() : GemmBound{}, half ? GemmBound{nxt->bw.rows.p, 1} : GemmBound{});
        timer.end(st2, tj_);
        EESEN_HIP_CHECK(hipEventRecord(ev_gate_done, st2));
      } }
      if (L.cur_fwd_drop)
        mul_elements(st, L.Y.p + (size_t)S * ldY, ldY, L.fmask.p, ldY, L.Yd.p, ldY, rows, ldY);
      x = L.output(S);
      ldx = ldY;
    } else if (L.kind == EESEN_LAYER_AFFINE) {
      const int ldo = pad4(L.dout);
      if (L.out.reserve((size_t)rows * ldo)) EESEN_HIP_CHECK(hipMemsetAsync(L.out.p, 0, L.out.cap * sizeof(float), st));
      { const int ti_ = timer.begin(st, 2);
      gemm_f32(st, true, true, rows, L.dout, L.din, 1.f, x, ldx, params.p + L.p_off + L.off_w, pad4(L.din), 0.f, L.out.p, ldo,
               params.p + L.p_off + L.off_b, nullptr, 0, 0, fwd_bf16, x_amax, w_amax);
      timer.end(st, ti_); }
      x = L.out.p;
      ldx = ldo;
    } else if (L.is_activation()) {
      const int ldo = pad4(L.dout);
      if (L.out.reserve((size_t)rows * ldo)) EESEN_HIP_CHECK(hipMemsetAsync(L.out.p, 0, L.out.cap * sizeof(float), st));
      { const int ti_ = timer.begin(st, 2);
      activation_rows(st, L.kind == EESEN_LAYER_TANH, x, ldx, L.out.p, ldo, rows, L.dout);
      timer.end(st, ti_); }
      x = L.out.p;
      ldx = ldo;
    } else {
      const int ldo = pad4(L.dout);
      if (L.out.reserve((size_t)rows * ldo)) EESEN_HIP_CHECK(hipMemsetAsync(L.out.p, 0, L.out.cap * sizeof(float), st));
      { const int ti_ = timer.begin(st, 2);
      softmax_rows(st, x, ldx, L.out.p, ldo, rows, L.dout);
      timer.end(st, ti_); }
      x = L.out.p;
      ldx = ldo;
    }
  }
  out_ptr = x;
  out_cols = layers.back().dout;
  out_ld = ldx;
  if (const Layer& Lb = layers.back(); Lb.out_nb) {
    const int ldo = pad4(Lb.dout_f);
    if (out_f.reserve((size_t)rows * ldo) && ldo != Lb.dout_f) EESEN_HIP_CHECK(hipMemsetAsync(out_f.p, 0, out_f.cap * sizeof(float), st));
    for (int b = 0; b < Lb.out_nb; ++b) copy2d(st, x + (size_t)b * Lb.out_hi, ldx, out_f.p + (size_t)b * Lb.out_hf, ldo, rows, Lb.out_hf);
    out_ptr = out_f.p; out_cols = Lb.dout_f; out_ld = ldo;
  }
  propagated = true;
  if (persistent) arm_device_error_poll();
}

void Net::backpropagate(const float* out_diff, int ldd, float* in_diff, int ldi) {
  bucket_log.clear();
  deferred_buckets.clear();
  try {
    backpropagate_impl(out_diff, ldd, in_diff, ldi);
  } catch (...) {
    fail_step_buckets();
    throw;
  }
}

void Net::backpropagate_impl(const float* out_diff, int ldd, float* in_diff, int ldi) {
  EESEN_REQUIRE(propagated, EESEN_ERR_STATE, "Backpropagate needs a preceding Propagate");
  EESEN_HIP_CHECK(hipSetDevice(device));
  int maxdim = 0, max_g = 0, max_y = 0;
  size_t need_ws = 0;
  for (const Layer& L : layers) {
    maxdim = std::max(maxdim, std::max(pad4(L.din), pad4(L.dout)));
    if (L.is_lstm()) {
      max_g = std::max(max_g, L.ndir * 4 * L.H);
      max_y = std::max(max_y, L.ndir * L.H);
      need_ws = std::max(need_ws, lstm_bias_peep_ws_floats(T, S, L.H, L.ndir));
    }
    need_ws = std::max(need_ws, col_sums_ws_floats(rows, L.dout));
  }
  need_ws = std::max(need_ws, (size_t)16 << 20);
  ws.reserve(need_ws);
  ws_floats = need_ws;
  dA.reserve((size_t)rows * maxdim);
  dB.reserve((size_t)rows * maxdim);
  if (max_g) {
    DGb[0].reserve((size_t)rows * max_g);
    DGb[1].reserve((size_t)rows * max_g);
  }
  if (max_y) DCF.reserve((size_t)S * max_y);
  ws2.reserve(need_ws);
  int dg_slot = 0;
  bool side_pending[2] = {false, false};
  deferred_buckets.clear();
  const std::vector<RecPlan> bwd = bwd_plans(T);
  const bool overlap = overlap_for_minibatch(bwd);
  exchange_deferred = comm && exchange_deferred_for_minibatch(bwd);
  bucket_log.clear();
  info_bwd_persistent = 0;
  live_valid = comm != nullptr;
  if (comm) {
    comm_check_alive(comm);
    EESEN_HIP_CHECK(hipMemsetD32Async(reinterpret_cast<hipDeviceptr_t>(fresh.p + P), 0x3f800000, 1, st));
  }

  const int Kout = layers.back().dout;
  float* d = dA.p;
  int ld_d = pad4(Kout);
  float* dn = dB.p;
  const bool half = gemm_mode() == 2;
  ensure_weight_amax();
  auto x_cols = [&](int li) -> GemmBound {
    if (!half || !amx_valid) return GemmBound{};
    return x_is_bounded(li) ? bound_one() : GemmBound{layers[li].bx.cols.p, 1};
  };
  if (const Layer& Lb = layers.back(); Lb.out_nb) {
    EESEN_HIP_CHECK(hipMemsetAsync(d, 0, (size_t)rows * ld_d * sizeof(float), st));
    for (int b = 0; b < Lb.out_nb; ++b) copy2d(st, out_diff + (size_t)b * Lb.out_hf, ldd, d + (size_t)b * Lb.out_hi, ld_d, rows, Lb.out_hf);
  } else {
    if (ld_d != Kout) EESEN_HIP_CHECK(hipMemsetAsync(d, 0, (size_t)rows * ld_d * sizeof(float), st));
    copy2d(st, out_diff, ldd, d, ld_d, rows, Kout);
  }

  for (int li = (int)layers.size() - 1; li >= 0; --li) {
    Layer& L = layers[li];
    const float* x;
    int ldx;
    if (li == 0) { x = input.p; ldx = pad4(L.din); }
    else {
      const Layer& Pv = layers[li - 1];
      if (Pv.is_lstm()) { ldx = Pv.ndir * Pv.H; x = Pv.output(S); }
      else { ldx = pad4(Pv.dout); x = Pv.out.p; }
    }
    const bool want_in = li > 0 || in_diff != nullptr;
    const int ld_n = pad4(L.din);
    float* fr = fresh.p + L.p_off;
    if (L.kind == EESEN_LAYER_SOFTMAX) {
      continue;
    } else if (L.is_activation()) {
      { const int ti_ = timer.begin(st, 4);
      activation_diff_rows(st, L.kind == EESEN_LAYER_TANH, L.out.p, pad4(L.dout), d, ld_d, rows, L.dout);
      timer.end(st, ti_); }
      continue;
    } else if (L.kind == EESEN_LAYER_AFFINE) {
      { const int ti_ = timer.begin(st, 4);
      if (half) measure(d, rows, L.dout, ld_d, L.bd.rows, L.bd.cols);
      if (want_in) {
        if (ld_n != L.din) EESEN_HIP_CHECK(hipMemsetAsync(dn, 0, (size_t)rows * ld_n * sizeof(float), st));
        gemm_f32(st, true, false, rows, L.din, L.dout, 1.f, d, ld_d, params.p + L.p_off + L.off_w, pad4(L.din), 0.f, dn, ld_n,
                 nullptr, nullptr, 0, 0, false, half ? GemmBound{L.bd.rows.p, 1} : GemmBound{}, half ? GemmBound{L.bw.cols.p, 1} : GemmBound{});
      }
      gemm_f32(st, false, false, L.dout, L.din, rows, 1.f, d, ld_d, x, ldx, 0.f, fr + L.off_w, pad4(L.din), nullptr, ws.p, ws_floats, 0, false,
               half ? GemmBound{L.bd.cols.p, 1} : GemmBound{}, x_cols(li));
      col_sums(st, d, rows, L.dout, ld_d, fr + L.off_b, ws.p, ws_floats);
      timer.end(st, ti_); }
      bucket_allreduce(li, st);
    } else {
      const int H = L.H, nd = L.ndir, ldG = nd * 4 * H, ldY = nd * H;
      LstmLayerDev v = lstm_view(*this, L, T);
      v.poll_delay = overlap ? delay_bwd_side : delay_bwd;
      v.poll_raw = poll_raw;
      const RecPlan& bp = bwd[li];
      if (bp.need_px) { bwd_px.reserve(bp.need_px); v.PX = bwd_px.p; v.px_floats = bwd_px.cap; }
      if (bp.need_dgh) {
        bwd_dgh.reserve((size_t)rows * ldG);
        bwd_ex.reserve(bp.need_ex);
        v.DGH = reinterpret_cast<unsigned char*>(bwd_dgh.p);
        v.EX = bwd_ex.p;
      }
      EESEN_REQUIRE(in_train || !L.has_dropout(), EESEN_ERR_STATE, "Can't backpropagate a dropout layer in test mode (bilstm-parallel-layer.h:425)");
      if (L.cur_fwd_drop) mul_elements(st, d, ld_d, L.fmask.p, ldY, d, ld_d, rows, ldY);
      float* DGl = DGb[dg_slot].p;
      if (side_pending[dg_slot]) {
        EESEN_HIP_CHECK(hipStreamWaitEvent(st, ev_grad[dg_slot], 0));
        side_pending[dg_slot] = false;
      }
      { const int ti_ = timer.begin(st, 3);
      if (bp.kind != kRecNone) {
        lstm_bwd_launch(st, bp, v, d, ld_d, DGl, ctl.p + kCtlHalf, ctl.p + kCtlWords - 1, spin_limit, trace.p ? trace.p + 640 : nullptr);
        ++info_bwd_persistent;
      } else
        for (int step = 0; step < T; ++step) lstm_bwd_step(st, v, step, d, ld_d, DGl, DCF.p);
      check_launch("lstm_bwd");
      timer.end(st, ti_); }
      if (half) { const int ti_ = timer.begin(st, 4); measure(DGl, rows, ldG, ldG, L.bd.rows, L.bd.cols); timer.end(st, ti_); }
      EESEN_HIP_CHECK(hipEventRecord(ev_rec, st));
      if (want_in) {
        const int ti_ = timer.begin(st, 4);
        if (ld_n != L.din) EESEN_HIP_CHECK(hipMemsetAsync(dn, 0, (size_t)rows * ld_n * sizeof(float), st));
        gemm_f32(st, true, false, rows, L.din, ldG, 1.f, DGl, ldG, params.p + L.p_off + L.off_wx, pad4(L.din), 0.f, dn, ld_n,
                 nullptr, nullptr, 0, 0, false, half ? GemmBound{L.bd.rows.p, 1} : GemmBound{}, half ? GemmBound{L.bw.cols.p, 1} : GemmBound{});
        timer.end(st, ti_);
        EESEN_HIP_CHECK(hipEventRecord(ev_rec, st));
      }
      hipStream_t sg = overlap ? st2 : st;
      const int side_lds_env = (tn.side_lds_kb >= 0 ? tn.side_lds_kb : (gemm_mode() >= 1 ? 48 : 32)) * 1024;
      bool lstm_below = false;
      for (int lj = 0; lj < li; ++lj) lstm_below |= layers[lj].is_lstm();
      const int side_lds = overlap && lstm_below ? side_lds_env : 0;
      if (overlap) EESEN_HIP_CHECK(hipStreamWaitEvent(st2, ev_rec, 0));
      { const int ti_ = timer.begin(sg, 4);
      gemm_f32(sg, false, false, ldG, L.din, rows, 1.f, DGl, ldG, x, ldx, 0.f, fr + L.off_wx, pad4(L.din), nullptr, ws2.p, need_ws, side_lds, false,
               half ? GemmBound{L.bd.cols.p, 1} : GemmBound{}, x_cols(li));
      for (int dir = 0; dir < nd; ++dir)
        gemm_f32(sg, false, false, 4 * H, H, rows, 1.f, DGl + (size_t)dir * 4 * H, ldG,
                 L.Y.p + (size_t)(dir == 0 ? 0 : 2 * S) * ldY + (size_t)dir * H, ldY, 0.f,
                 fr + L.off_wm + (size_t)dir * 4 * H * H, H, nullptr, ws2.p, need_ws, side_lds, false,
                 half ? GemmBound{L.bd.cols.p + (size_t)dir * 4 * H, 1} : GemmBound{}, half ? bound_one() : GemmBound{});
      lstm_bias_peep_grads(sg, v, DGl, fr + L.off_bias, fr + L.off_peep, ws2.p, need_ws);
      timer.end(sg, ti_); }
      bucket_allreduce(li, sg);
      if (overlap) {
        EESEN_HIP_CHECK(hipEventRecord(ev_grad[dg_slot], st2));
        side_pending[dg_slot] = true;
      }
      dg_slot ^= 1;
    }
    if (want_in) {
      std::swap(d, dn);
      ld_d = ld_n;
    }
  }
  if (in_diff) copy2d(st, d, ld_d, in_diff, ldi, rows, layers[0].din);
  flush_deferred_buckets();
  for (int k = 0; k < 2; ++k)
    if (side_pending[k]) EESEN_HIP_CHECK(hipStreamWaitEvent(st, ev_grad[k], 0));
}

std::vector<RecPlan> Net::bwd_plans(int T) const {
  std::vector<RecPlan> plans(layers.size());
  for (size_t li = 0; li < layers.size(); ++li)
    if (persistent && layers[li].is_lstm()) plans[li] = lstm_bwd_plan(lstm_view(*this, layers[li], T));
  return plans;
}
bool Net::overlap_for_minibatch(const std::vector<RecPlan>& bwd) const {
  bool ov = overlap;
  if (ov && tn.overlap < 0 && persistent)
    for (size_t li = 0; li < layers.size(); ++li)
      if (const Layer& L = layers[li]; L.is_lstm() && L.H > 320 && L.H <= 512 && S > 32 && !bwd[li].light) ov = false;
  return ov;
}
bool Net::exchange_deferred_for_minibatch(const std::vector<RecPlan>& bwd) const {
  if (tn.comm_defer >= 0) return tn.comm_defer != 0;
  if (!persistent) return false;
  for (const RecPlan& bp : bwd)
    if (bp.kind != kRecNone && bp.free_vgprs < kRcclVgprsPerSimdLane) return true;
  return false;
}

std::string Net::plan_string() const {
  EESEN_REQUIRE(finalized, EESEN_ERR_STATE, "net not finalized");
  EESEN_REQUIRE(S > 0, EESEN_ERR_STATE, "call eesen_net_set_seq_lengths first: the plan depends on the minibatch shape");
  EESEN_HIP_CHECK(hipSetDevice(device));
  int T = this->T;
  if (!propagated) { T = 0; for (int v : lens) T = std::max(T, v); }
  auto one = [](const RecPlan& P) {
    char b[512];
    if (P.kind == kRecNone) { snprintf(b, sizeof(b), "{\"kernel\": \"per-step kernels (lstm.hip)\", \"persistent\": false}"); return std::string(b); }
    snprintf(b, sizeof(b), "{\"kernel\": \"%s\", \"persistent\": true, \"sequences_per_workgroup\": %d, \"units_per_workgroup\": %d, \"grid\": [%d, %d, %d], "
             "\"workgroups\": %d, \"workgroups_per_cu\": %d, \"launches\": %d, \"vgprs\": %d, \"lds_bytes\": %d, \"free_vgprs_per_simd_lane\": %d}",
             P.kernel, P.seq_tile, P.units, P.grid[0], P.grid[1], P.grid[2], P.wgs, P.wgs_per_cu, P.windows, P.vgprs, P.lds, P.free_vgprs);
    return std::string(b);
  };
  const std::vector<RecPlan> bwd = bwd_plans(T);
  std::string o = "{\"T\": " + std::to_string(T) + ", \"S\": " + std::to_string(S) + ", \"persistent\": " + (persistent ? "true" : "false") + ", \"layers\": [";
  bool first = true;
  for (size_t li = 0; li < layers.size(); ++li) {
    const Layer& L = layers[li];
    if (!L.is_lstm()) continue;
    const RecPlan fp = persistent && T >= 1 ? lstm_fwd_plan(lstm_view(*this, L, T)) : RecPlan{}, &bp = bwd[li];
    o += std::string(first ? "" : ", ") + "{\"layer\": " + std::to_string(li) + ", \"cells\": " + std::to_string(L.H) + ", \"directions\": " + std::to_string(L.ndir) +
         ", \"forward\": " + one(fp) + ", \"backward\": " + one(bp) + "}";
    first = false;
  }
  const bool ov = overlap_for_minibatch(bwd);
  o += std::string("], \"weight_gradient_gemms\": \"") + (ov ? "side stream, under the next-lower recurrence" : "main stream, serial") + "\"";
  o += std::string(", \"gemm_arithmetic\": \"") + (gemm_mode() == 2 ? "two fp16 planes, three products (fp32-class)" : gemm_mode() == 1 ? "3-way bf16 split (fp32-class)" : "f32-input MFMA") + "\"";
  o += std::string(", \"exchange\": ") + (comm ? (exchange_deferred_for_minibatch(bwd) ? "\"deferred: every bucket behind the backward pass's last recurrence\""
                                                                                      : "\"overlapped: each bucket as soon as its layer's gradients are enqueued\"") : "null");
  o += std::string(", \"exchange_rule\": \"") + (tn.comm_defer >= 0 ? "EESEN_COMM_DEFER" : "auto: deferred when a persistent backward grid leaves < 256 registers per SIMD lane") + "\"";
  o += ", \"gpu_share\": " + std::to_string(gpu_share_value()) + "}";
  return o;
}

void Net::update() {
  EESEN_REQUIRE(finalized, EESEN_ERR_STATE, "net not finalized");
  EESEN_HIP_CHECK(hipSetDevice(device));
  const unsigned* skip = persistent && !grads_sanitized ? ctl.p + kCtlWords - 1 : nullptr;
  const float* live = comm && live_valid ? fresh.p + P : nullptr;
  comm_check_alive(comm);
  { const int ti_ = timer.begin(st, 5);
  for (int li = (int)layers.size() - 1; li >= 0; --li) {
    Layer& L = layers[li];
    if (L.p_n) {
      if (comm && li < (int)bucket_pending.size() && bucket_pending[li]) {
        const int tw_ = timer.begin(st, 7);
        EESEN_HIP_CHECK(hipStreamWaitEvent(st, ev_bucket[li], 0));
        timer.end(st, tw_);
        bucket_pending[li] = 0;
      }
      if (rule == 0) {
        sgd_update(st, params.p + L.p_off, corr.p + L.p_off, fresh.p + L.p_off, (long)L.p_n, mmt, lr * L.coef, L.max_grad, skip, live);
      } else {
        init_accu();
        adaptive_update(st, params.p + L.p_off, corr.p + L.p_off, fresh.p + L.p_off, accu.p + L.p_off, (long)L.p_n, mmt, lr,
                        L.max_grad, ada_eps, rms_rho, rms_one_minus_rho, rule == 2, skip, live);
      }
    }
  }
  refresh_derived();
  timer.end(st, ti_); }
  grads_sanitized = false;
  live_valid = false;
  if (persistent) arm_device_error_poll();
}

}
```

eesen_amd/csrc/net.h:

```cpp
#pragma once
#include <string>
#include <vector>

#include "kernels.h"
#include "tuning.h"

namespace eesen {

inline int pad4(int x) { return (x + 3) & ~3; }
constexpr size_t kCtlWords = 2 * kCtlHalf + 32;

struct Layer {
  int kind = 0, din = 0, dout = 0;
  float coef = 1.f, max_grad = 0.f;
  size_t p_off = 0, p_n = 0;
  int H = 0, ndir = 0;
  int din_f = 0, dout_f = 0, Hf = 0;
  int in_nb = 0, in_hf = 0, in_hi = 0, out_nb = 0, out_hf = 0, out_hi = 0;
  int in_col(int d) const { return in_nb ? (d / in_hf) * in_hi + d % in_hf : d; }
  size_t off_wx = 0, off_bias = 0, off_wm = 0, off_peep = 0;
  DevBuf<float> WmT;
  DevBuf<float> G, C, Y;
  DevBuf<float> X;
  size_t off_w = 0, off_b = 0;
  DevBuf<float> out;
  struct Bounds { DevBuf<float> rows, cols; } bw, bx, bd;
  float drop[9] = {0, 0, 0, 0, 0, 0, 0, 0, 0};
  bool has_dropout() const { return drop[0] > 0.f || drop[5] != 0.f || drop[6] != 0.f; }
  DevBuf<float> fmask;
  DevBuf<float> rmask;
  DevBuf<float> Yd;
  bool cur_fwd_drop = false;
  int cur_drop_mode = 0;
  bool cur_twiddle_coin = false;
  std::vector<float> inj_fmask, inj_rmask;
  int inj_rmask_rows = 0, inj_coin = -1;
  const float* output(int S) const { return cur_fwd_drop ? Yd.p : Y.p + (size_t)S * ndir * H; }
  bool is_lstm() const { return kind == EESEN_LAYER_LSTM_PARALLEL || kind == EESEN_LAYER_BILSTM_PARALLEL; }
  bool nonparallel = false;
  bool is_activation() const { return kind == EESEN_LAYER_SIGMOID || kind == EESEN_LAYER_TANH; }
  bool trainable() const { return is_lstm() || kind == EESEN_LAYER_AFFINE; }
  long file_params() const;
  const char* marker() const;
};

class PhaseTimer {
 public:
  ~PhaseTimer();
  void enable(bool on) { on_ = on; }
  bool enabled() const { return on_; }
  void set_accumulate(bool a) { accumulate_ = a; used_ = 0; }
  void reset() { if (!accumulate_) used_ = 0; }
  int begin(hipStream_t st, int phase);
  void end(hipStream_t st, int idx);
  void collect(float* out, int nphase);
  int spans(int* phases, float* secs, int cap);
 private:
  struct Span { hipEvent_t a, b; int phase; };
  std::vector<Span> spans_;
  size_t used_ = 0;
  bool on_ = false, accumulate_ = false;
};

struct Comm;
void comm_check_alive(const Comm* c);
constexpr size_t kLiveWords = 4;
constexpr int kRcclVgprsPerSimdLane = 256;

struct Net {
  int device = 0;
  hipStream_t st = nullptr;
  bool own_stream = false;
  std::vector<Layer> layers;
  bool finalized = false;
  size_t P = 0;
  DevBuf<float> params, corr, fresh;
  float lr = 0.f, mmt = 0.f;
  int rule = 0;
  float ada_eps = 1e-6f, rms_rho = 0.9f, rms_one_minus_rho = 0.1f;
  DevBuf<float> accu;
  bool accu_init = false;
  void init_accu();
  void set_accu(const float* host, long n);
  std::vector<int> lens;
  DevBuf<int> lens_d;
  int T = 0, S = 0, rows = 0;
  bool propagated = false;
  DevBuf<float> input;
  struct HostStage { float* p = nullptr; size_t cap = 0; hipEvent_t ev = nullptr; bool busy = false; } in_stage[2];
  unsigned in_stage_idx = 0;
  const float* out_ptr = nullptr;
  int out_cols = 0, out_ld = 0;
  DevBuf<float> out_f;
  DevBuf<float> DGb[2], DCF, dA, dB, ws, ws2;
  DevBuf<float> bwd_px;
  DevBuf<float> bwd_dgh, bwd_ex;
  hipStream_t st2 = nullptr;
  hipEvent_t ev_rec = nullptr, ev_grad[2] = {nullptr, nullptr};
  bool overlap = true;
  hipEvent_t ev_gate_reset = nullptr, ev_gate_done = nullptr;
  DevBuf<unsigned> mile;
  bool gate_fwd = true;
  bool fwd_bf16 = false;
  bool fwd_bf16_rec = false;
  int info_fwd_bf16 = 0;
  DevBuf<unsigned> ctl;
  Tuning tn;
  int persistent = 1;
  int info_fwd_persistent = 0, info_bwd_persistent = 0, info_lstm_layers = 0;
  int spin_limit = 400000;
  float flight_ns = 0.f;
  int delay_fwd = 61, delay_bwd = 43, delay_bwd_side = 64, poll_raw = 0;
  int recoveries = 0;
  DevBuf<unsigned long long> trace;
  void check_device_error(bool consumer);
  int steps_since_clean = 0;
  int* lens_pin = nullptr;
  size_t lens_pin_cap = 0;
  hipEvent_t lens_ev = nullptr, err_ev = nullptr;
  unsigned* err_pin = nullptr;
  bool err_armed = false;
  void poll_device_error();
  void arm_device_error_poll();
  bool in_train = true;
  unsigned long long drop_seed = 777, drop_counter = 0;
  void set_train_mode(bool train) { in_train = train; }
  void set_layer_dropout(int layer, const float* nine);
  void get_layer_dropout(int layer, float* nine) const;
  void set_dropout_masks(int layer, const float* fwd, long fwd_n, const float* rec, int rec_rows, long rec_n, int coin);
  void get_dropout_masks(int layer, float* fwd_host, float* rec_host, int* info4);
  size_t ws_floats = 0;
  DevBuf<float> amax, amax_ws;
  bool wamax_valid = false, wm_valid = false;
  bool amx_valid = false;
  float* am_wm(int li) { return amax.p + 1 + li; }
  GemmBound bound_one() const { return GemmBound{amax.p, 0}; }
  bool x_is_bounded(int li) const;
  void measure(const float* P, long rows, int cols, int ld, DevBuf<float>& out_rows, DevBuf<float>& out_cols);
  void ensure_weight_amax();
  PhaseTimer timer;
  Comm* comm = nullptr;
  std::vector<hipEvent_t> ev_ready, ev_bucket;
  std::vector<char> bucket_pending;
  std::vector<int> deferred_buckets;
  bool exchange_deferred = false;
  std::vector<RecPlan> bwd_plans(int T) const;
  bool overlap_for_minibatch(const std::vector<RecPlan>& bwd) const;
  bool exchange_deferred_for_minibatch(const std::vector<RecPlan>& bwd) const;
  std::string plan_string() const;
  hipEvent_t ev_bwd_done = nullptr;
  void issue_bucket(int li);
  void fail_step_buckets() noexcept;
  void flush_deferred_buckets();
  std::vector<struct Ctc*> guards;
  std::vector<struct CeLoss*> ce_guards;
  bool grads_sanitized = false;
  bool live_valid = false;
  std::vector<int> bucket_log;
  float* live_pin = nullptr;
  void set_comm(Comm* c);
  int top_trainable() const;
  int live_ranks();
  void bucket_allreduce(int li, hipStream_t producer);
  void wait_buckets_host();
  void backpropagate_zero();
  void allreduce_grads(Comm* c);

  Net(int device, void* stream);
  ~Net();
  void add_layer(int kind, int din, int dout, float coef, float max_grad);
  void finalize();
  long num_params() const;
  void set_params(const float* host, long n);
  void get_flat(const DevBuf<float>& buf, float* host, long n);
  void set_seq_lengths(const int* lens, int S);
  void propagate(const float* in, int rows, int ld, bool is_device);
  void forward_pass();
  void backpropagate(const float* out_diff, int ldd, float* in_diff, int ldi);
  void backpropagate_impl(const float* out_diff, int ldd, float* in_diff, int ldi);
  void update();
  void refresh_derived();
  int tensor_moments(int which, int layer, double* out6_host, int cap_tensors);
  void read(const std::string& path);
  void write(const std::string& path, bool binary);
  void sync();
};

struct Ctc {
  int device = 0;
  hipStream_t st = nullptr;
  bool own_stream = false;
  DevBuf<float> logp, alpha, beta, pzx_d;
  DevBuf<int> labx, lens_d, lablens_d, cls_off, cls_pos, ids_d;
  std::vector<int> last_lens;
  int last_T = 0, last_S = 0, last_Lpad = 0, last_Lprime = 0;
  int sweep_waves = 0;
  double obj_sum = 0;
  long sequences = 0, frames = 0, err_tokens = 0, ref_tokens = 0;
  hipEvent_t ev[4] = {nullptr, nullptr, nullptr, nullptr};
  PhaseTimer timer;
  struct Pin {
    void* p = nullptr;
    size_t cap = 0;
    hipEvent_t ev = nullptr;
    bool busy = false;
  };
  Pin stage[2];
  unsigned stage_idx = 0;
  struct PendingPzx { Pin pin; int S = 0; long nframes = 0; bool active = false; } ppzx[2];
  struct PendingErr { Pin pin, probs; int S = 0, K = 0, rows = 0; bool active = false, with_probs = false, guarded = false; std::vector<int> frames, ids, off; } perr[2];
  const unsigned* guard = nullptr;
  struct Net* guard_net = nullptr;
  long dropped = 0;
  std::string seq_out;
  unsigned ppzx_idx = 0, perr_idx = 0;
  static void* pin_reserve(Pin& pin, size_t bytes);
  void flush_pzx(PendingPzx& q);
  void flush_err(PendingErr& q, int* num_err, int* num_ref);
  void flush();

  Ctc(int device, void* stream);
  ~Ctc();
// ... 39 lines not shown
```

eesen_amd/csrc/optim.hip:

```cpp
#include "kernels.h"

namespace eesen {
namespace {

__global__ __launch_bounds__(256) void sgd_update_kernel(float* __restrict__ param, float* __restrict__ corr,
                                                         const float* __restrict__ fresh, long n, float mmt,
                                                         float lr_coef, float max_grad, const unsigned* __restrict__ skip,
                                                         const float* __restrict__ live) {
  if (skip && *skip) return;
  if (live && *live == 0.f) return;
  const long n4 = n >> 2;
  const long stride = (long)gridDim.x * blockDim.x;
  for (long i = (long)blockIdx.x * blockDim.x + threadIdx.x; i < n4; i += stride) {
    float4 p = reinterpret_cast<float4*>(param)[i];
    float4 c = reinterpret_cast<float4*>(corr)[i];
    const float4 g = reinterpret_cast<const float4*>(fresh)[i];
    c.x = mmt * c.x + g.x; c.y = mmt * c.y + g.y; c.z = mmt * c.z + g.z; c.w = mmt * c.w + g.w;
    if (max_grad > 0.f) {
      c.x = fminf(fmaxf(c.x, -max_grad), max_grad); c.y = fminf(fmaxf(c.y, -max_grad), max_grad);
      c.z = fminf(fmaxf(c.z, -max_grad), max_grad); c.w = fminf(fmaxf(c.w, -max_grad), max_grad);
    }
    p.x -= lr_coef * c.x; p.y -= lr_coef * c.y; p.z -= lr_coef * c.z; p.w -= lr_coef * c.w;
    reinterpret_cast<float4*>(corr)[i] = c;
    reinterpret_cast<float4*>(param)[i] = p;
  }
  for (long i = (n4 << 2) + (long)blockIdx.x * blockDim.x + threadIdx.x; i < n; i += stride) {
    float c = mmt * corr[i] + fresh[i];
    if (max_grad > 0.f) c = fminf(fmaxf(c, -max_grad), max_grad);
    corr[i] = c;
    param[i] -= lr_coef * c;
  }
}

__global__ __launch_bounds__(256) void adaptive_update_kernel(float* __restrict__ param, float* __restrict__ corr,
                                                              const float* __restrict__ fresh, float* __restrict__ accu,
                                                              long n, float mmt, float lr, float max_grad, float eps,
                                                              float rho, float one_minus_rho, int rmsprop,
                                                              const unsigned* __restrict__ skip, const float* __restrict__ live) {
  if (skip && *skip) return;
  if (live && *live == 0.f) return;
  const long stride = (long)gridDim.x * blockDim.x;
  for (long i = (long)blockIdx.x * blockDim.x + threadIdx.x; i < n; i += stride) {
    float c = mmt * corr[i] + fresh[i];
    if (max_grad > 0.f) c = fminf(fmaxf(c, -max_grad), max_grad);
    const float g2 = c * c;
    float a = accu[i];
    a = rmsprop ? (rho * a + one_minus_rho * g2) : (a + g2);
    const float scale = 1.0f / sqrtf(a + eps);
    corr[i] = c;
    accu[i] = a;
    param[i] += -lr * scale * c;
  }
}

__global__ __launch_bounds__(256) void zero_if_set_kernel(float* __restrict__ p, long n, const unsigned* __restrict__ word) {
  if (*word == 0u) return;
  const long stride = (long)gridDim.x * blockDim.x;
  for (long i = (long)blockIdx.x * blockDim.x + threadIdx.x; i < n; i += stride) p[i] = 0.f;
}

__global__ __launch_bounds__(256) void transpose2d_kernel(const float* __restrict__ src, int rows, int cols,
                                                          float* __restrict__ dst) {
  __shared__ float tile[32][33];
  const int tx = threadIdx.x & 31, ty = threadIdx.x >> 5;
  const int c0 = blockIdx.x * 32, r0 = blockIdx.y * 32;
#pragma unroll
  for (int i = 0; i < 32; i += 8) {
    const int r = r0 + ty + i, c = c0 + tx;
    if (r < rows && c < cols) tile[ty + i][tx] = src[(size_t)r * cols + c];
  }
  __syncthreads();
#pragma unroll
  for (int i = 0; i < 32; i += 8) {
    const int c = c0 + ty + i, r = r0 + tx;
    if (r < rows && c < cols) dst[(size_t)c * rows + r] = tile[tx][ty + i];
  }
}

__global__ __launch_bounds__(256) void copy2d_kernel(const float* __restrict__ src, int lds, float* __restrict__ dst,
                                                     int ldd, int rows, int cols) {
  const size_t total = (size_t)rows * cols;
  for (size_t i = (size_t)blockIdx.x * blockDim.x + threadIdx.x; i < total; i += (size_t)gridDim.x * blockDim.x) {
    const size_t r = i / cols, c = i % cols;
    dst[r * ldd + c] = src[r * lds + c];
  }
}

}

void sgd_update(hipStream_t st, float* param, float* corr, const float* fresh, long n, float mmt, float lr_coef,
                float max_grad, const unsigned* skip, const float* live) {
  if (n <= 0) return;
  const int blocks = (int)std::min<long>(cdivl(n / 4 + 1, 256), 2048);
  hipLaunchKernelGGL(sgd_update_kernel, dim3(blocks), dim3(256), 0, st, param, corr, fresh, n, mmt, lr_coef, max_grad, skip, live);
  check_launch("sgd_update");
}

void zero_if_set(hipStream_t st, float* p, long n, const unsigned* word) {
  if (n <= 0 || !word) return;
  hipLaunchKernelGGL(zero_if_set_kernel, dim3(256), dim3(256), 0, st, p, n, word);
  check_launch("zero_if_set");
}

void adaptive_update(hipStream_t st, float* param, float* corr, const float* fresh, float* accu, long n, float mmt, float lr,
                     float max_grad, float eps, float rho, float one_minus_rho, bool rmsprop, const unsigned* skip, const float* live) {
  if (n <= 0) return;
  const int blocks = (int)std::min<long>(cdivl(n, 256), 4096);
  hipLaunchKernelGGL(adaptive_update_kernel, dim3(blocks), dim3(256), 0, st, param, corr, fresh, accu, n, mmt, lr, max_grad, eps,
                     rho, one_minus_rho, rmsprop ? 1 : 0, skip, live);
  check_launch("adaptive_update");
}

void transpose2d(hipStream_t st, const float* src, int rows, int cols, float* dst) {
  hipLaunchKernelGGL(transpose2d_kernel, dim3(cdiv(cols, 32), cdiv(rows, 32)), dim3(256), 0, st, src, rows, cols, dst);
  check_launch("transpose2d");
}

void copy2d(hipStream_t st, const float* src, int lds, float* dst, int ldd, int rows, int cols) {
  if (rows <= 0 || cols <= 0) return;
  const size_t total = (size_t)rows * cols;
  const int blocks = (int)std::min<size_t>((total + 255) / 256, 4096);
  hipLaunchKernelGGL(copy2d_kernel, dim3(blocks), dim3(256), 0, st, src, lds, dst, ldd, rows, cols);
  check_launch("copy2d");
}


namespace {
__device__ __forceinline__ float hash_uniform(unsigned long long seed, unsigned long long idx) {
  unsigned long long z = seed + (idx + 1ull) * 0x9E3779B97F4A7C15ull;
  z = (z ^ (z >> 30)) * 0xBF58476D1CE4E5B9ull;
  z = (z ^ (z >> 27)) * 0x94D049BB133111EBull;
  z ^= z >> 31;
  return (float)(z >> 40) * (1.0f / 16777216.0f);
}
__global__ __launch_bounds__(256) void dropout_mask_kernel(float* __restrict__ out, long rows, int cols, int ld, float p, float scale,
                                                           unsigned long long seed, int per_column) {
  const long n = rows * cols;
  for (long i = (long)blockIdx.x * blockDim.x + threadIdx.x; i < n; i += (long)gridDim.x * blockDim.x) {
    const long r = i / cols;
    const int c = (int)(i % cols);
    const float u = hash_uniform(seed, per_column ? (unsigned long long)c : (unsigned long long)i);
    out[r * ld + c] = (u - p > 0.f) ? scale : 0.f;
  }
}
__global__ __launch_bounds__(256) void mul_elements_kernel(const float* __restrict__ a, int lda, const float* __restrict__ m, int ldm,
                                                           float* __restrict__ out, int ldo, long rows, int cols) {
  const long n = rows * cols;
  for (long i = (long)blockIdx.x * blockDim.x + threadIdx.x; i < n; i += (long)gridDim.x * blockDim.x) {
    const long r = i / cols;
    const int c = (int)(i % cols);
    out[r * ldo + c] = a[r * lda + c] * m[r * ldm + c];
  }
}
template <bool TANH>
__global__ __launch_bounds__(256) void activation_kernel(const float* __restrict__ x, int ldx, float* __restrict__ y, int ldy, long rows, int cols) {
  const long n = rows * cols;
  for (long i = (long)blockIdx.x * blockDim.x + threadIdx.x; i < n; i += (long)gridDim.x * blockDim.x) {
    const long r = i / cols;
    const int c = (int)(i % cols);
    const float v = x[r * ldx + c];
    float o;
    if (TANH) {
      const float e = expf(2.0f * v);
      o = isinf(e) ? 1.0f : (e - 1.0f) / (e + 1.0f);
    } else {
      o = 1.0f / (1.0f + expf(-v));
    }
    y[r * ldy + c] = o;
  }
}
template <bool TANH>
__global__ __launch_bounds__(256) void activation_diff_kernel(const float* __restrict__ y, int ldy, float* __restrict__ d, int ldd, long rows, int cols) {
  const long n = rows * cols;
  for (long i = (long)blockIdx.x * blockDim.x + threadIdx.x; i < n; i += (long)gridDim.x * blockDim.x) {
    const long r = i / cols;
    const int c = (int)(i % cols);
    const float o = y[r * ldy + c];
    d[r * ldd + c] *= TANH ? (1.0f - o * o) : o * (1.0f - o);
  }
}
}

void activation_rows(hipStream_t st, bool tanh_, const float* x, int ldx, float* y, int ldy, long rows, int cols) {
  if (rows <= 0 || cols <= 0) return;
  const int blocks = (int)std::min<long>(cdivl(rows * cols, 256), 256L * 16);
  if (tanh_) hipLaunchKernelGGL(activation_kernel<true>, dim3(blocks), dim3(256), 0, st, x, ldx, y, ldy, rows, cols);
  else hipLaunchKernelGGL(activation_kernel<false>, dim3(blocks), dim3(256), 0, st, x, ldx, y, ldy, rows, cols);
  check_launch("activation_rows");
}

void activation_diff_rows(hipStream_t st, bool tanh_, const float* y, int ldy, float* d, int ldd, long rows, int cols) {
  if (rows <= 0 || cols <= 0) return;
  const int blocks = (int)std::min<long>(cdivl(rows * cols, 256), 256L * 16);
  if (tanh_) hipLaunchKernelGGL(activation_diff_kernel<true>, dim3(blocks), dim3(256), 0, st, y, ldy, d, ldd, rows, cols);
  else hipLaunchKernelGGL(activation_diff_kernel<false>, dim3(blocks), dim3(256), 0, st, y, ldy, d, ldd, rows, cols);
  check_launch("activation_diff_rows");
}

void dropout_mask(hipStream_t st, float* out, long rows, int cols, int ld, float p, unsigned long long seed, bool per_column) {
  if (rows <= 0 || cols <= 0) return;
  const int blocks = (int)std::min<long>(cdivl(rows * cols, 256), 256L * 16);
  hipLaunchKernelGGL(dropout_mask_kernel, dim3(blocks), dim3(256), 0, st, out, rows, cols, ld, p, 1.0f / (1.0f - p), seed, per_column ? 1 : 0);
  check_launch("dropout_mask");
}

void mul_elements(hipStream_t st, const float* a, int lda, const float* m, int ldm, float* out, int ldo, long rows, int cols) {
  if (rows <= 0 || cols <= 0) return;
  const int blocks = (int)std::min<long>(cdivl(rows * cols, 256), 256L * 16);
// ... 50 lines not shown
```

eesen_amd/csrc/rec_plan.cpp:

```cpp
#include "rec_kernels.h"

#include <atomic>
#include <map>
#include <mutex>
#include <tuple>

namespace eesen {
namespace {

constexpr int NW = kRecWaves;

std::atomic<int> g_share_override{0};
int gpu_share() {
  static const int env = [] { const char* e = getenv("EESEN_GPU_SHARE"); const int v = e && *e ? atoi(e) : 0; return v < 1 ? 0 : v; }();
  if (env) return env;
  const int o = g_share_override.load(std::memory_order_relaxed);
  return o > 0 ? o : 1;
}
int share_of_cus() {
  int ncu = 256, dev = 0;
  (void)hipGetDevice(&dev);
  (void)hipDeviceGetAttribute(&ncu, hipDeviceAttributeMultiprocessorCount, dev);
  return std::max(1, ncu / gpu_share());
}
// ... 153 lines not shown
  static float cache[64] = {0};
  static std::mutex mu;
  std::lock_guard<std::mutex> lock(mu);
  int dev = 0;
  if (hipGetDevice(&dev) != hipSuccess || dev < 0 || dev >= 64) return 0.f;
  if (cache[dev] > 0.f) return cache[dev];
  unsigned* flags = nullptr;
  unsigned long long* out = nullptr;
  EESEN_HIP_CHECK(hipMalloc(reinterpret_cast<void**>(&flags), 64 * sizeof(unsigned)));
  EESEN_HIP_CHECK(hipMalloc(reinterpret_cast<void**>(&out), sizeof(unsigned long long)));
  int rounds = 2000;
  double ns[5];
  for (int rep = 0; rep < 5; ++rep) {
    EESEN_HIP_CHECK(hipMemset(flags, 0, 64 * sizeof(unsigned)));
    void* argv[] = {&flags, &out, &rounds};
    (void)hipLaunchKernel(handoff_pingpong_fn(), dim3(2), dim3(64), argv, 0, nullptr);
    unsigned long long ticks = 0;
    EESEN_HIP_CHECK(hipMemcpy(&ticks, out, sizeof(ticks), hipMemcpyDeviceToHost));
    ns[rep] = ticks ? 10.0 * (double)ticks / (2.0 * rounds) : 500.0;
  }
  std::sort(ns, ns + 5);
  (void)hipFree(flags);
  (void)hipFree(out);
  cache[dev] = (float)std::min(2000.0, std::max(100.0, ns[2]));
  return cache[dev];
}

void wait_for_word(hipStream_t st, const unsigned* word, unsigned target, unsigned* err, double limit_s) {
  unsigned long long ticks = (unsigned long long)(std::max(0.05, limit_s) * 1e8);
  void* argv[] = {&word, &target, &err, &ticks};
  (void)hipLaunchKernel(wait_for_word_fn(), dim3(1), dim3(64), argv, 0, st);
  check_launch("wait_for_word");
}

RecPlan lstm_fwd_plan(const LstmLayerDev& L) {
  RecPlan P;
  const int need = ((L.H + 31) / 32 + NW - 1) / NW;
  const FwdTile ft = fwd_tile(L);
  if (need > 4 || (ft.nt == 2 && need > 2) || L.H % (4 * ft.nt) != 0 || L.T < 2) return P;
  if (!line_aligned(L.S, L.ndir * L.H)) return P;
  if ((size_t)(L.T + 2) * L.S * L.ndir * L.H * sizeof(float) >= ((size_t)1 << 31)) return P;
  BfPlan B = bf_plan_shape(L, ft);
  const bool drop = L.drop_mode != 0;
  const int cpw32 = ft.nt == 2 ? std::min(need, 2) : need <= 2 ? need : 4;
  int nwin = B.on ? pick_windows(L.S, 16, [&](int Sw) { return bf_fits(L, B, Sw); }) : 0;
  if (nwin == 0) {
    B.on = false;
    const RecKernel* probe = rec_kernel(kFwdF32, cpw32, ft.mt, ft.nt, drop, false);
    nwin = pick_windows(L.S, 16 * ft.mt, [&](int Sw) { return probe && fits(*probe, dim3(L.H / (4 * ft.nt), L.ndir, cdiv(Sw, 16 * ft.mt))); });
  }
  if (nwin == 0) return P;
  if (nwin > 1 && !line_aligned(L.S / nwin, L.ndir * L.H)) return P;
  const int mt = B.on ? 1 : ft.mt, nt = B.on ? B.nt : ft.nt, nz = cdiv(L.S, 16 * mt);
  auto answer = [&](const RecKernel& k, const dim3& grid, size_t words, int seq_tile, int windows, bool one_window) {
    take(P, k, grid, words, seq_tile, 4 * nt, windows);
    P.seq_tiles = nz;
    P.one_window = one_window;
    P.leaves_room = nt <= 2 && (!B.on || (long)(L.H / (4 * nt)) * L.ndir * nz <= share_of_cus());
    P.bf16 = L.fwd_bf16 && k.kind == kRecFwdBf;
  };
  const dim3 grid(L.H / (4 * nt), L.ndir, cdiv(L.S / nwin, 16 * mt));
  const size_t words = ctl_words(grid.y * grid.z);
  if (B.on) {
    if (words <= (size_t)kCtlHalf) answer(*rec_kernel(kFwdBf, B.cpw, B.nt, B.ap, B.wp, B.f16), grid, words, 16, nwin, nwin == 1);
    return P;
  }
  const bool xchg = L.X != nullptr && ft.mt == 1 && L.H % 32 == 0 && !drop && small_xchg(L, 2048);
  if (L.fwd_mux && nwin == 2 && ft.mt == 1 && ft.nt == 4 && need > 2 && need <= 4 && !drop && L.H % 32 == 0) {
    const RecKernel& k = *rec_kernel(kFwdMux, 4, 4, xchg);
    const dim3 mgrid(L.H / 16, L.ndir, cdiv(nz, 2));
    if (fits(k, mgrid) && ctl_words((size_t)L.ndir * nz) <= (size_t)kCtlHalf) {
      answer(k, mgrid, ctl_words((size_t)L.ndir * nz), 32, 1, false);
      return P;
    }
  }
  if (words > (size_t)kCtlHalf) return P;
  const RecKernel* k = rec_kernel(kFwdF32, cpw32, ft.mt, ft.nt, drop, xchg);
  EESEN_REQUIRE(k != nullptr, EESEN_ERR_STATE, "no instantiation of the fp32 forward tile for this plan");
  answer(*k, grid, words, 16 * ft.mt, nwin, nwin == 1);
  return P;
}

void lstm_fwd_launch(hipStream_t st, const RecPlan& P, const LstmLayerDev& L0, unsigned* cnt, unsigned* err, int spin_limit,
                     unsigned long long* trace, hipEvent_t after_reset) {
  EESEN_REQUIRE(P.kind == kRecFwdBf || P.kind == kRecFwdMux || P.kind == kRecFwdF32, EESEN_ERR_STATE, "not a forward recurrence plan");
  const RecRole role{P.grid[0], P.grid[1], P.grid[2], L0.xcd_map};
  for (int w = 0; w < P.windows; ++w) {
    LstmLayerDev L = L0;
    if (P.kind == kRecFwdMux) { L.s_begin = 0; L.s_count = 0; }
    else { L.s_count = L0.S / P.windows; L.s_begin = w * L.s_count; }
    if (P.kind != kRecFwdMux && P.wgs_per_cu >= 2 && !L0.poll_raw) L.poll_delay = L0.poll_delay * 7 / 4;
    EESEN_HIP_CHECK(hipMemsetAsync(cnt, 0, sizeof(unsigned) * P.ctl_words, st));
    if (after_reset && P.one_window) EESEN_HIP_CHECK(hipEventRecord(after_reset, st));
    if (P.kind == kRecFwdMux) plan_launch(st, P.fn, P.wgs, L, cnt, err, spin_limit, role);
    else plan_launch(st, P.fn, P.wgs, L, cnt, err, spin_limit, trace, role);
  }
}

RecPlan lstm_bwd_plan(const LstmLayerDev& L) {
  RecPlan P;
  const int need = ((4 * L.H + 31) / 32 + NW - 1) / NW;
  const int ldG = L.ndir * 4 * L.H;
  const long blocks16 = (long)cdiv(L.H, 16) * L.ndir * cdiv(L.S, 16);
  const int stile = 2 * blocks16 <= share_of_cus() && L.S > 8 ? 8 : 16;
  P.light = stile == 8;
  if (need > 16 || L.T < 2) return P;
  if (!line_aligned(L.S, ldG)) return P;
  const size_t blk_bytes = (size_t)L.S * ldG * sizeof(float);
  const long max_blocks = (long)((((size_t)1 << 31) - 1) / blk_bytes);
  if (max_blocks < 3) return P;
  int chunk = (int)std::min<long>(L.T, max_blocks - 1);
  if (chunk < L.T) { int p2 = 1; while (p2 * 2 <= chunk) p2 *= 2; chunk = p2; }
  P.chunk = chunk;
  auto in_windows = [&](const RecKernel* k, int gx, int seq_tile, int units, int quarters) {
    if (!k) return false;
    auto grid_of = [&](int Sw) { return dim3(gx, L.ndir, cdiv(Sw, seq_tile)); };
    auto words_of = [&](const dim3& g) { return ctl_words((size_t)g.y * g.z * quarters); };
    const int nwin = pick_windows(L.S, seq_tile, [&](int Sw) { return words_of(grid_of(Sw)) <= (size_t)kCtlHalf && fits(*k, grid_of(Sw)); });
    if (nwin == 0 || (nwin > 1 && !line_aligned(L.S / nwin, ldG))) return false;
    take(P, *k, grid_of(L.S / nwin), words_of(grid_of(L.S / nwin)), seq_tile, units, nwin);
    return true;
  };
  for (int pass = 0; pass < 2; ++pass) {
    const int stq = (L.bwd_q4_st8 == 2) == (pass == 0) ? 8 : 4;
    if (!L.bwd_q4 || L.drop_mode || L.H % 32 != 0 || L.H > 512 || chunk < L.T) break;
    if (stq == 4 && stile != 8) continue;
    if (stq == 8 && !(L.bwd_q4_st8 && L.S > 8)) continue;
    const int cpw = 2 * ((L.H + 127) / 128);
    const dim3 grid(L.H / 32, L.ndir, cdiv(L.S, stq));
    const size_t words = ctl_words((size_t)grid.y * grid.z);
    const RecKernel& k = *rec_kernel(kBwdQ4, cpw, stq);
    if (fits(k, grid) && words <= (size_t)kCtlHalf) {
      take(P, k, grid, words, stq, 32, 1);
      return P;
    }
  }
  if (bwd_ksplit_shape(L, stile)) {
    const int cpw = L.H / (32 * NW), gx = L.H / 64 * 4;
    const size_t px = (size_t)2 * L.ndir * cdiv(L.S, 16) * (size_t)(L.H / 64) * 4096 * 2;
    if (bwd_planes_shape(L, stile) && in_windows(rec_kernel(kBwdKsplitH, cpw), gx, 16, 64, 4)) {
      P.need_px = px; P.need_dgh = true;
      P.need_ex = (size_t)L.T * L.ndir * cdiv(L.S, 16) * (size_t)(L.H / 16) * 16;
      return P;
    }
    const RecKernel* k = rec_kernel(kBwdKsplit, cpw);
    const int nwin = !k ? 0 : pick_windows(L.S, 16, [&](int Sw) {
      const dim3 grid(gx, L.ndir, cdiv(Sw, 16));
      return ctl_words((size_t)grid.y * grid.z * 4) <= (size_t)kCtlHalf && fits(*k, grid);
    });
    if (nwin == 2 && L.bwd_mux && cpw >= 2 && cpw <= 4) {
      const int nz = cdiv(L.S, 16);
      const dim3 grid(gx, L.ndir, cdiv(nz, 2));
      const size_t words = ctl_words((size_t)L.ndir * nz * 4);
      const RecKernel& km = *rec_kernel(kBwdKsplitMux, cpw);
      if (words <= (size_t)kCtlHalf && fits(km, grid)) {
        take(P, km, grid, words, 32, 64, 1);
        P.need_px = px;
        return P;
      }
    }
    if (nwin > 0 && (nwin == 1 || line_aligned(L.S / nwin, ldG))) {
      const dim3 grid(gx, L.ndir, cdiv(L.S / nwin, 16));
      take(P, *k, grid, ctl_words((size_t)grid.y * grid.z * 4), 16, 64, nwin);
      P.need_px = px;
      return P;
    }
  }
  in_windows(rec_kernel(kBwdGeneric, need <= 1 ? 1 : need <= 2 ? 2 : need <= 4 ? 4 : need <= 8 ? 8 : 16, stile, L.drop_mode != 0), cdiv(L.H, 16), stile, 16, 1);
  return P;
}

void lstm_bwd_launch(hipStream_t st, const RecPlan& P, const LstmLayerDev& L0, const float* dY, int lddy, float* DG, unsigned* cnt,
                     unsigned* err, int spin_limit, unsigned long long* trace) {
  EESEN_REQUIRE(P.kind == kRecBwdQ4 || P.kind == kRecBwdKsplit || P.kind == kRecBwdKsplitMux || P.kind == kRecBwdGeneric, EESEN_ERR_STATE, "not a backward recurrence plan");
  EESEN_REQUIRE(!P.need_px || (L0.PX && L0.px_floats >= P.need_px), EESEN_ERR_STATE, "the backward plan's partial-sum exchange space (RecPlan::need_px) was not handed over");
  EESEN_REQUIRE(!P.need_dgh || (L0.DGH && L0.EX), EESEN_ERR_STATE, "the backward plan's plane and exponent buffers (RecPlan::need_dgh, need_ex) were not handed over");
  const RecRole role{P.grid[0], P.grid[1], P.grid[2], L0.xcd_map};
  const bool whole_batch = P.kind == kRecBwdQ4 || P.kind == kRecBwdKsplitMux;
  unsigned long long* px = reinterpret_cast<unsigned long long*>(L0.PX);
  int chunk = P.chunk;
  for (int w = 0; w < P.windows; ++w) {
    LstmLayerDev L = L0;
    if (whole_batch) { L.s_begin = 0; L.s_count = 0; }
    else { L.s_count = L0.S / P.windows; L.s_begin = w * L.s_count; }
    EESEN_HIP_CHECK(hipMemsetAsync(cnt, 0, sizeof(unsigned) * P.ctl_words, st));
    if (P.need_px) EESEN_HIP_CHECK(hipMemsetAsync(L.PX, 0, sizeof(float) * P.need_px, st));
    if (P.kind == kRecBwdQ4) plan_launch(st, P.fn, P.wgs, L, dY, lddy, DG, cnt, err, spin_limit, trace, role);
    else if (P.kind == kRecBwdKsplitMux) plan_launch(st, P.fn, P.wgs, L, dY, lddy, DG, px, cnt, err, spin_limit, role, chunk);
    else if (P.kind == kRecBwdKsplit) plan_launch(st, P.fn, P.wgs, L, dY, lddy, DG, px, cnt, err, spin_limit, role, chunk, trace);
    else plan_launch(st, P.fn, P.wgs, L, dY, lddy, DG, cnt, err, spin_limit, trace, role, chunk);
  }
}

}
```

eesen_amd/csrc/tuning.h:

```cpp
#pragma once
#include <cstdlib>

namespace eesen {

struct Tuning {
  int persistent = 1;
  int overlap = -1, gate_fwd = -1, side_lds_kb = -1;
  int spin_limit = 400000;
  bool spin_limit_set = false;
  int bwd_q4 = 1, bwd_q4_st8 = 1, fwd_narrow2 = 1, fwd_t16_small = 1, bwd_ksplit = 1, fwd_mux = 1, bwd_mux = 1, xcd_map = 1, fwd_mid = 1, fwd_split = 1, fwd_f16 = 1, bwd_f16 = 1;
  int comm_defer = -1;
  int trace = 0;
  bool print_flight = false;
  const char* poll_ns = nullptr;

  static Tuning from_env() {
    Tuning t;
    auto num = [](const char* name, int dflt) {
      const char* e = getenv(name);
      return e && *e ? atoi(e) : dflt;
    };
    t.persistent = num("EESEN_PERSISTENT", 1);
    t.overlap = num("EESEN_OVERLAP", -1);
    t.gate_fwd = num("EESEN_GATE_FWD", -1);
    t.fwd_mid = num("EESEN_FWD_MID", 1);
    t.side_lds_kb = num("EESEN_SIDE_LDS_KB", -1);
    t.spin_limit_set = getenv("EESEN_SPIN_LIMIT") != nullptr;
    t.spin_limit = num("EESEN_SPIN_LIMIT", 400000);
    t.bwd_q4 = num("EESEN_BWD_Q4", 1);
    t.bwd_q4_st8 = num("EESEN_BWD_Q4_ST8", 1);
    t.fwd_narrow2 = num("EESEN_FWD_NARROW2", 1);
    t.fwd_t16_small = num("EESEN_FWD_T16_SMALL", 1);
    t.bwd_ksplit = num("EESEN_BWD_KSPLIT", 1);
    t.fwd_mux = num("EESEN_FWD_MUX", 1);
    t.bwd_mux = num("EESEN_BWD_MUX", 1);
    t.fwd_split = num("EESEN_FWD_SPLIT", 1);
    t.fwd_f16 = num("EESEN_FWD_F16", 1);
    t.bwd_f16 = num("EESEN_BWD_F16", 1);
    t.xcd_map = num("EESEN_XCD_MAP", 1);
    t.comm_defer = num("EESEN_COMM_DEFER", -1);
    t.trace = num("EESEN_TRACE", 0);
    t.print_flight = getenv("EESEN_PRINT_FLIGHT") != nullptr;
    t.poll_ns = getenv("EESEN_POLL_NS");
    return t;
  }
};

}
```

Measured before the change: 1.013 million.

## Batch small memsets, transposes and amax passes into multi-job kernels

Adds multi-job kernels that each do several pieces of small work in one launch: memsets go through a FillList, per-layer weight transposes through transpose2d_multi, and weight amax measurements through amax_multi. The per-step resets of the recurrence counters and partial-sum buffers are also pre-zeroed together instead of issued per layer. The control-word area is enlarged to hold one slot per LSTM layer, so each layer's counters can be cleared up front. The goal is to cut kernel-launch and memset overhead per training step, at the cost of more complex bookkeeping and the risk of counter-reuse errors, which is guarded by rec_plan_counts_once.

Result: no change. 1.017 million (median of 5 runs) (+0.3%).

```diff
diff --git a/eesen_amd/csrc/capi.cpp b/eesen_amd/csrc/capi.cpp
--- a/eesen_amd/csrc/capi.cpp
+++ b/eesen_amd/csrc/capi.cpp
@@ -213,7 +213,7 @@
   return guard([&] {
     REQ_PTR(net);
     EESEN_HIP_CHECK(hipSetDevice(net->device));
-    EESEN_HIP_CHECK(hipMemsetD32Async(reinterpret_cast<hipDeviceptr_t>(net->ctl.p + kCtlWords - 1), (int)value, 1, net->st));
+    EESEN_HIP_CHECK(hipMemsetD32Async(reinterpret_cast<hipDeviceptr_t>(net->err_word()), (int)value, 1, net->st));
   });
 }
 int eesen_net_synchronize(eesen_net_t* net) {
@@ -281,7 +281,7 @@
       auto& g = ctc->guard_net->guards;
       g.erase(std::remove(g.begin(), g.end(), static_cast<Ctc*>(ctc)), g.end());
     }
-    ctc->guard = net && net->ctl.p ? net->ctl.p + kCtlWords - 1 : nullptr;
+    ctc->guard = net && net->ctl.p ? net->err_word() : nullptr;
     ctc->guard_net = ctc->guard ? net : nullptr;
     if (ctc->guard_net) net->guards.push_back(ctc);
   });
@@ -351,7 +351,7 @@
       auto& g = ce->guard_net->ce_guards;
       g.erase(std::remove(g.begin(), g.end(), static_cast<CeLoss*>(ce)), g.end());
     }
-    ce->guard = net && net->ctl.p ? net->ctl.p + kCtlWords - 1 : nullptr;
+    ce->guard = net && net->ctl.p ? net->err_word() : nullptr;
     ce->guard_net = ce->guard ? net : nullptr;
     if (ce->guard_net) net->ce_guards.push_back(ce);
   });
diff --git a/eesen_amd/csrc/comm.cpp b/eesen_amd/csrc/comm.cpp
--- a/eesen_amd/csrc/comm.cpp
+++ b/eesen_amd/csrc/comm.cpp
@@ -445,7 +445,7 @@
 void Net::issue_bucket(int li) {
   EESEN_HIP_CHECK(hipStreamWaitEvent(comm->st, ev_ready[li], 0));
   const bool top = li == top_trainable();
-  if (ctl.p) zero_if_set(comm->st, fresh.p + layers[li].p_off, (long)(layers[li].p_n + (top ? kLiveWords : 0)), ctl.p + kCtlWords - 1);
+  if (ctl.p) zero_if_set(comm->st, fresh.p + layers[li].p_off, (long)(layers[li].p_n + (top ? kLiveWords : 0)), err_word());
   grads_sanitized = true;
   const int ti_ = timer.begin(comm->st, 6);
   comm->allreduce_f32(fresh.p + layers[li].p_off, layers[li].p_n + (top ? kLiveWords : 0), comm->st);
@@ -522,7 +522,7 @@
   EESEN_REQUIRE(finalized, EESEN_ERR_STATE, "net not finalized");
   EESEN_REQUIRE(c && c->device == device, EESEN_ERR_INVALID, "communicator missing or on another device");
   EESEN_HIP_CHECK(hipSetDevice(device));
-  if (ctl.p) zero_if_set(st, fresh.p, (long)P, ctl.p + kCtlWords - 1);
+  if (ctl.p) zero_if_set(st, fresh.p, (long)P, err_word());
   grads_sanitized = true;
   c->allreduce_f32(fresh.p, P, st);
 }
diff --git a/eesen_amd/csrc/gemm.hip b/eesen_amd/csrc/gemm.hip
--- a/eesen_amd/csrc/gemm.hip
+++ b/eesen_amd/csrc/gemm.hip
@@ -739,6 +739,63 @@
   }
 }
 
+constexpr int kAmaxJobs = 24, kAmaxMultiRows = 64;
+struct AmaxMultiArgs {
+  struct Mat { const float* P; unsigned *out_rows, *out_cols, *out_all; int rows, cols, ld, nslab, block0, pad_; } m[kAmaxJobs];
+  int n;
+};
+__global__ __launch_bounds__(256) void amax_multi_kernel(const AmaxMultiArgs a) {
+  __shared__ unsigned red[kAmaxMultiRows][4];
+  __shared__ unsigned red_all[4];
+  const int bid = (int)blockIdx.x, tid = threadIdx.x, lane = tid & 63, wave = tid >> 6;
+  AmaxMultiArgs::Mat g = a.m[0];
+#pragma unroll
+  for (int i = 1; i < kAmaxJobs; ++i)
+    if (i < a.n && bid >= a.m[i].block0) g = a.m[i];
+  const int b = bid - g.block0, slab = b % g.nslab;
+  const long r0 = (long)(b / g.nslab) * kAmaxMultiRows;
+  const int c = slab * 1024 + tid * 4;
+  const bool in = c < g.cols;
+  uint4 cm = make_uint4(0u, 0u, 0u, 0u);
+  for (int i0 = 0; i0 < kAmaxMultiRows; i0 += 8) {
+    uint4 v[8];
+#pragma unroll
+    for (int k = 0; k < 8; ++k) {
+      const long r = r0 + i0 + k;
+      v[k] = in && r < g.rows ? *reinterpret_cast<const uint4*>(g.P + r * g.ld + c) : make_uint4(0u, 0u, 0u, 0u);
+    }
+#pragma unroll
+    for (int k = 0; k < 8; ++k) {
+      v[k].x &= 0x7fffffffu; v[k].y &= 0x7fffffffu; v[k].z &= 0x7fffffffu; v[k].w &= 0x7fffffffu;
+      cm.x = max(cm.x, v[k].x); cm.y = max(cm.y, v[k].y); cm.z = max(cm.z, v[k].z); cm.w = max(cm.w, v[k].w);
+      unsigned m = max(max(v[k].x, v[k].y), max(v[k].z, v[k].w));
+#pragma unroll
+      for (int o = 32; o > 0; o >>= 1) m = max(m, (unsigned)__shfl_xor((int)m, o));
+      if (lane == 0) red[i0 + k][wave] = m;
+    }
+  }
+  unsigned all = max(max(cm.x, cm.y), max(cm.z, cm.w));
+#pragma unroll
+  for (int o = 32; o > 0; o >>= 1) all = max(all, (unsigned)__shfl_xor((int)all, o));
+  if (lane == 0) red_all[wave] = all;
+  __syncthreads();
+  if (g.out_rows && tid < kAmaxMultiRows && r0 + tid < g.rows) {
+    const unsigned m = max(max(red[tid][0], red[tid][1]), max(red[tid][2], red[tid][3]));
+    if (g.nslab > 1) atomicMax(&g.out_rows[r0 + tid], m);
+    else g.out_rows[r0 + tid] = m;
+  }
+  if (g.out_cols && in) {
+    if (cm.x) atomicMax(&g.out_cols[c], cm.x);
+    if (cm.y) atomicMax(&g.out_cols[c + 1], cm.y);
+    if (cm.z) atomicMax(&g.out_cols[c + 2], cm.z);
+    if (cm.w) atomicMax(&g.out_cols[c + 3], cm.w);
+  }
+  if (g.out_all && tid == 0) {
+    const unsigned m = max(max(red_all[0], red_all[1]), max(red_all[2], red_all[3]));
+    if (m) atomicMax(g.out_all, m);
+  }
+}
+
 __global__ __launch_bounds__(256) void splitk_reduce_kernel(const float* __restrict__ ws, int splits, int M, int N,
                                                             float alpha, float beta, float* __restrict__ C, int ldc,
                                                             const float* __restrict__ bias) {
@@ -791,15 +848,16 @@
   }
   check_launch("amax_abs");
 }
-void amax_rows_cols(hipStream_t st, const float* P, long rows, int cols, int ld, float* out_rows, float* out_cols, float* ws) {
+bool amax_rows_accumulate(int cols, int ld) { return (((cols & 3) == 0 && (ld & 3) == 0) && cols > 1024) || cols > kAmaxSlabCols; }
+void amax_rows_cols(hipStream_t st, const float* P, long rows, int cols, int ld, float* out_rows, float* out_cols, float* ws, bool rows_zeroed) {
   if (rows <= 0 || cols <= 0) return;
   EESEN_REQUIRE(!out_cols || ws, EESEN_ERR_INVALID, "amax: column bounds need a workspace");
   unsigned* r = reinterpret_cast<unsigned*>(out_rows);
   unsigned* w = reinterpret_cast<unsigned*>(ws);
   unsigned* a = nullptr;
   const bool vec = (cols & 3) == 0 && (ld & 3) == 0;
-  const bool multi = out_rows && ((vec && cols > 1024) || cols > kAmaxSlabCols);
-  if (multi) EESEN_HIP_CHECK(hipMemsetAsync(out_rows, 0, (size_t)rows * sizeof(float), st));
+  const bool multi = out_rows && amax_rows_accumulate(cols, ld);
+  if (multi && !rows_zeroed) EESEN_HIP_CHECK(hipMemsetAsync(out_rows, 0, (size_t)rows * sizeof(float), st));
   for (int c0 = 0; c0 < cols; c0 += kAmaxSlabCols) {
     const float* Pc = P + c0;
     const int cc = std::min(kAmaxSlabCols, cols - c0), racc = multi ? 1 : 0;
@@ -816,6 +874,26 @@
   }
 }
 #undef EESEN_AMAX_LAUNCH
+
+void amax_multi(hipStream_t st, const AmaxJob* jobs, int n) {
+  for (int j0 = 0; j0 < n; j0 += kAmaxJobs) {
+    AmaxMultiArgs a{};
+    int blocks = 0;
+    a.n = std::min(kAmaxJobs, n - j0);
+    for (int k = 0; k < a.n; ++k) {
+      AmaxJob j = jobs[j0 + k];
+      EESEN_REQUIRE(j.rows > 0 && j.cols > 0 && (j.cols & 3) == 0 && (j.ld & 3) == 0 && (reinterpret_cast<size_t>(j.P) & 15) == 0, EESEN_ERR_INVALID,
+                    "amax_multi: rows of whole, 16-byte aligned quads");
+      if (!j.out_rows && !j.out_cols && j.cols == j.ld && j.cols < 1024 && (j.rows * j.cols) % 1024 == 0) { j.rows = j.rows * j.cols / 1024; j.cols = j.ld = 1024; }
+      const int nslab = (j.cols + 1023) / 1024;
+      a.m[k] = AmaxMultiArgs::Mat{j.P, reinterpret_cast<unsigned*>(j.out_rows), reinterpret_cast<unsigned*>(j.out_cols), reinterpret_cast<unsigned*>(j.out_all),
+                                  (int)j.rows, j.cols, j.ld, nslab, blocks, 0};
+      blocks += nslab * (int)((j.rows + kAmaxMultiRows - 1) / kAmaxMultiRows);
+    }
+    hipLaunchKernelGGL(amax_multi_kernel, dim3(blocks), dim3(256), 0, st, a);
+    check_launch("amax_multi");
+  }
+}
 
 static GemmBound arena_bound(hipStream_t st, const float* P, bool kc, int R, int K, int ld) {
   constexpr size_t kArena = (size_t)4 << 20, kDevs = 16;
diff --git a/eesen_amd/csrc/kernels.h b/eesen_amd/csrc/kernels.h
--- a/eesen_amd/csrc/kernels.h
+++ b/eesen_amd/csrc/kernels.h
@@ -19,7 +19,15 @@
 void amax_abs(hipStream_t st, const float* P, long rows, int cols, int ld, float* out);
 void amax_abs_accumulate(hipStream_t st, const float* P, long rows, int cols, int ld, float* out);
 constexpr int kAmaxBlocks = 512;
-void amax_rows_cols(hipStream_t st, const float* P, long rows, int cols, int ld, float* out_rows, float* out_cols, float* ws);
+void amax_rows_cols(hipStream_t st, const float* P, long rows, int cols, int ld, float* out_rows, float* out_cols, float* ws, bool rows_zeroed = false);
+bool amax_rows_accumulate(int cols, int ld);
+struct AmaxJob {
+  const float* P;
+  long rows;
+  int cols, ld;
+  float *out_rows, *out_cols, *out_all;
+};
+void amax_multi(hipStream_t st, const AmaxJob* jobs, int n);
 
 #ifndef EESEN_SHARDS
 #define EESEN_SHARDS 8
@@ -103,10 +111,13 @@
 };
 RecPlan lstm_fwd_plan(const LstmLayerDev& L);
 RecPlan lstm_bwd_plan(const LstmLayerDev& L);
+inline bool rec_plan_counts_once(const RecPlan& P) {
+  return P.kind != kRecNone && P.windows == 1 && P.kind != kRecFwdMux && P.kind != kRecBwdKsplitMux;
+}
 void lstm_fwd_launch(hipStream_t st, const RecPlan& plan, const LstmLayerDev& L, unsigned* cnt, unsigned* err, int spin_limit,
-                     unsigned long long* trace = nullptr, hipEvent_t after_reset = nullptr);
+                     unsigned long long* trace = nullptr, hipEvent_t after_reset = nullptr, bool counters_zeroed = false);
 void lstm_bwd_launch(hipStream_t st, const RecPlan& plan, const LstmLayerDev& L, const float* dY, int lddy, float* DG, unsigned* cnt,
-                     unsigned* err, int spin_limit, unsigned long long* trace = nullptr);
+                     unsigned* err, int spin_limit, unsigned long long* trace = nullptr, bool zeroed = false);
 void lstm_bias_peep_grads(hipStream_t st, const LstmLayerDev& L, const float* DG, float* bias_grad, float* peep_grad,
                           float* ws, size_t ws_floats);
 size_t lstm_bias_peep_ws_floats(int T, int S, int H, int ndir);
@@ -143,5 +154,30 @@
                     int nb = 0, int hf = 0, int hi = 0);
 void transpose2d(hipStream_t st, const float* src, int rows, int cols, float* dst);
 void copy2d(hipStream_t st, const float* src, int lds, float* dst, int ldd, int rows, int cols);
+void copy2d_pad(hipStream_t st, const float* src, int lds, float* dst, int ldd, int rows, int cols);
+struct TransposeJob {
+  const float* src;
+  int rows, cols;
+  float* dst;
+};
+void transpose2d_multi(hipStream_t st, const TransposeJob* jobs, int n);
+class FillList {
+ public:
+  static constexpr int kMax = 32;
+  struct Region {
+    void* p;
+    size_t bytes;
+    unsigned value;
+    int block0, blocks;
+  };
+  explicit FillList(hipStream_t st) : st_(st) {}
+  void add(void* p, size_t bytes, unsigned value = 0u);
+  void launch();
+  int size() const { return n_; }
+ private:
+  hipStream_t st_;
+  Region r_[kMax];
+  int n_ = 0, blocks_ = 0;
+};
 
 }
diff --git a/eesen_amd/csrc/net.cpp b/eesen_amd/csrc/net.cpp
--- a/eesen_amd/csrc/net.cpp
+++ b/eesen_amd/csrc/net.cpp
@@ -114,6 +114,7 @@
   EESEN_HIP_CHECK(hipEventCreateWithFlags(&ev_gate_done, hipEventDisableTiming));
   tn = Tuning::from_env();
   persistent = tn.persistent;
+  fuse_small = tn.fuse_small != 0;
   gate_fwd = tn.gate_fwd >= 0 ? tn.gate_fwd != 0 : gemm_mode() == 0;
   overlap = tn.overlap >= 0 ? tn.overlap != 0 : persistent != 0;
   spin_limit = tn.spin_limit;
@@ -196,10 +197,10 @@
 void Net::check_device_error(bool consumer) {
   if (!ctl.p) return;
   unsigned e = 0;
-  EESEN_HIP_CHECK(hipMemcpy(&e, ctl.p + kCtlWords - 1, sizeof(unsigned), hipMemcpyDeviceToHost));
+  EESEN_HIP_CHECK(hipMemcpy(&e, err_word(), sizeof(unsigned), hipMemcpyDeviceToHost));
   if (!e) { steps_since_clean = 0; return; }
   EESEN_HIP_CHECK(hipStreamSynchronize(st));
-  EESEN_HIP_CHECK(hipMemset(ctl.p + kCtlWords - 1, 0, sizeof(unsigned)));
+  EESEN_HIP_CHECK(hipMemset(err_word(), 0, sizeof(unsigned)));
   const bool only_waiter = e == 2 && tn.fwd_mid;
   if (only_waiter) tn.fwd_mid = 0;
   else { persistent = 0; gate_fwd = false; overlap = false; }
@@ -229,7 +230,7 @@
     *err_pin = 0;
     EESEN_HIP_CHECK(hipEventCreateWithFlags(&err_ev, hipEventDisableTiming));
   }
-  EESEN_HIP_CHECK(hipMemcpyAsync(err_pin, ctl.p + kCtlWords - 1, sizeof(unsigned), hipMemcpyDeviceToHost, st));
+  EESEN_HIP_CHECK(hipMemcpyAsync(err_pin, err_word(), sizeof(unsigned), hipMemcpyDeviceToHost, st));
   EESEN_HIP_CHECK(hipEventRecord(err_ev, st));
   err_armed = true;
 }
@@ -310,6 +311,19 @@
     off += L.p_n;
   }
   P = off;
+  n_lstm = 0;
+  for (Layer& L : layers)
+    if (L.is_lstm()) L.lstm_index = n_lstm++;
+  mile.reserve((size_t)32 * std::max(1, n_lstm));
+  EESEN_HIP_CHECK(hipMemset(mile.p, 0, mile.cap * sizeof(unsigned)));
+  if (n_lstm > 1) {
+    ctl_words = (size_t)2 * n_lstm * kCtlHalf + 32;
+    ctl.reserve(ctl_words);
+    ctl_words = ctl.cap;
+    EESEN_HIP_CHECK(hipMemset(ctl.p, 0, ctl_words * sizeof(unsigned)));
+    for (Ctc* c : guards) c->guard = err_word();
+    for (CeLoss* c : ce_guards) c->guard = err_word();
+  }
   if (P) {
     params.reserve(P); corr.reserve(P); fresh.reserve(P + kLiveWords);
     EESEN_HIP_CHECK(hipMemsetAsync(params.p, 0, P * sizeof(float), st));
@@ -327,21 +341,43 @@
   sync();
 }
 
-void Net::measure(const float* Pm, long nrows, int cols, int ld, DevBuf<float>& out_rows, DevBuf<float>& out_cols) {
+void Net::reserve_bounds(long nrows, int cols, DevBuf<float>& out_rows, DevBuf<float>& out_cols) {
   out_rows.reserve((size_t)nrows);
   out_cols.reserve((size_t)cols);
   amax_ws.reserve((size_t)kAmaxBlocks * std::min(16384, (cols + 3) & ~3));
-  amax_rows_cols(st, Pm, nrows, cols, ld, out_rows.p, out_cols.p, amax_ws.p);
+}
+void Net::measure(const float* Pm, long nrows, int cols, int ld, DevBuf<float>& out_rows, DevBuf<float>& out_cols, bool rows_zeroed) {
+  reserve_bounds(nrows, cols, out_rows, out_cols);
+  amax_rows_cols(st, Pm, nrows, cols, ld, out_rows.p, out_cols.p, amax_ws.p, rows_zeroed);
 }
 bool Net::x_is_bounded(int li) const {
   if (li == 0) return false;
   const Layer& Pv = layers[li - 1];
   return (Pv.is_lstm() && !Pv.cur_fwd_drop) || Pv.is_activation() || Pv.kind == EESEN_LAYER_SOFTMAX;
 }
-void Net::ensure_weight_amax() {
+void Net::ensure_weight_amax(FillList* fills) {
   const bool mode2 = gemm_mode() == 2;
   const bool need_w = mode2 && !wamax_valid;
+  wjobs.clear();
   if (wm_valid && !need_w) return;
+  if (fills) {
+    if (!wm_valid) fills->add(am_wm(0), layers.size() * sizeof(float));
+    for (size_t li = 0; li < layers.size(); ++li) {
+      Layer& L = layers[li];
+      const int D4 = pad4(L.din);
+      if (!L.trainable()) continue;
+      const long wrows = L.is_lstm() ? (long)L.ndir * 4 * L.H : L.dout;
+      if (need_w) {
+        L.bw.rows.reserve((size_t)wrows);
+        L.bw.cols.reserve((size_t)D4);
+        fills->add(L.bw.cols.p, (size_t)D4 * sizeof(float));
+        if (D4 > 1024) fills->add(L.bw.rows.p, (size_t)wrows * sizeof(float));
+        wjobs.push_back(AmaxJob{params.p + L.p_off + (L.is_lstm() ? L.off_wx : L.off_w), wrows, D4, D4, L.bw.rows.p, L.bw.cols.p, nullptr});
+      }
+      if (L.is_lstm() && !wm_valid) wjobs.push_back(AmaxJob{params.p + L.p_off + L.off_wm, wrows, L.H, L.H, nullptr, nullptr, am_wm((int)li)});
+    }
+    return;
+  }
   if (!wm_valid) EESEN_HIP_CHECK(hipMemsetAsync(am_wm(0), 0, layers.size() * sizeof(float), st));
   for (size_t li = 0; li < layers.size(); ++li) {
     Layer& L = layers[li];
@@ -353,6 +389,13 @@
   wm_valid = true;
   if (mode2) wamax_valid = true;
 }
+void Net::ensure_weight_amax_run() {
+  if (wjobs.empty()) return;
+  amax_multi(st, wjobs.data(), (int)wjobs.size());
+  wjobs.clear();
+  wm_valid = true;
+  if (gemm_mode() == 2) wamax_valid = true;
+}
 
 long Net::num_params() const {
   long n = 0;
@@ -369,11 +412,14 @@
 
 void Net::refresh_derived() {
   wamax_valid = wm_valid = false;
+  std::vector<TransposeJob> jobs;
   for (Layer& L : layers)
     if (L.is_lstm())
       for (int dir = 0; dir < L.ndir; ++dir)
-        transpose2d(st, params.p + L.p_off + L.off_wm + (size_t)dir * 4 * L.H * L.H, 4 * L.H, L.H,
-                    L.WmT.p + (size_t)dir * L.H * 4 * L.H);
+        jobs.push_back(TransposeJob{params.p + L.p_off + L.off_wm + (size_t)dir * 4 * L.H * L.H, 4 * L.H, L.H, L.WmT.p + (size_t)dir * L.H * 4 * L.H});
+  if (fuse_small) transpose2d_multi(st, jobs.data(), (int)jobs.size());
+  else
+    for (const TransposeJob& j : jobs) transpose2d(st, j.src, j.rows, j.cols, j.dst);
 }
 
 int Net::tensor_moments(int which, int layer, double* out6_host, int cap_tensors) {
@@ -647,7 +693,37 @@
   int gated_rows = 0;
   int mid_r0 = 0, mid_r1 = 0;
   const bool half = gemm_mode() == 2;
-  ensure_weight_amax();
+  for (Layer& L : layers)
+    if (L.is_lstm()) {
+      const int H = L.H, nd = L.ndir, ldY = nd * H;
+      const size_t state = (size_t)(T + 2) * S * ldY;
+      L.G.reserve((size_t)rows * nd * 4 * H);
+      L.C.reserve(state);
+      L.Y.reserve(state);
+      if (persistent && H % 32 == 0) L.X.reserve((size_t)T * nd * ((S + 15) / 16) * (size_t)(H / 32) * 768);
+    }
+  std::vector<RecPlan> fwd(layers.size());
+  if (fuse_small) {
+    FillList fills(st);
+    ensure_weight_amax(&fills);
+    for (Layer& L : layers)
+      if (L.is_lstm()) {
+        const size_t ldY = (size_t)L.ndir * L.H, blk = (size_t)S * ldY * sizeof(float), last = (size_t)(T + 1) * S * ldY;
+        fills.add(L.C.p, blk);
+        fills.add(L.Y.p, blk);
+        fills.add(L.C.p + last, blk);
+        fills.add(L.Y.p + last, blk);
+        prepare_dropout(*this, L);
+        RecPlan& fp = fwd[&L - layers.data()];
+        if (persistent) fp = lstm_fwd_plan(lstm_view(*this, L, T));
+        if (rec_plan_counts_once(fp)) fills.add(ctl_slot(false, L), fp.ctl_words * sizeof(unsigned));
+      }
+    if (n_lstm) fills.add(mile.p, (size_t)n_lstm * 32 * sizeof(unsigned));
+    fills.launch();
+    ensure_weight_amax_run();
+  } else {
+    ensure_weight_amax();
+  }
   amx_valid = half;
   for (Layer& L : layers) {
     const int li_ = (int)(&L - layers.data());
@@ -659,17 +735,14 @@
     }
     if (L.is_lstm()) {
       const int H = L.H, nd = L.ndir, ldY = nd * H, ldG = nd * 4 * H;
-      L.G.reserve((size_t)rows * ldG);
-      const size_t state = (size_t)(T + 2) * S * ldY;
-      L.C.reserve(state);
-      L.Y.reserve(state);
-      if (persistent && H % 32 == 0) L.X.reserve((size_t)T * nd * ((S + 15) / 16) * (size_t)(H / 32) * 768);
-      const size_t blk = (size_t)S * ldY * sizeof(float);
-      EESEN_HIP_CHECK(hipMemsetAsync(L.C.p, 0, blk, st));
-      EESEN_HIP_CHECK(hipMemsetAsync(L.Y.p, 0, blk, st));
-      EESEN_HIP_CHECK(hipMemsetAsync(L.C.p + (size_t)(T + 1) * S * ldY, 0, blk, st));
-      EESEN_HIP_CHECK(hipMemsetAsync(L.Y.p + (size_t)(T + 1) * S * ldY, 0, blk, st));
-      prepare_dropout(*this, L);
+      if (!fuse_small) {
+        const size_t blk = (size_t)S * ldY * sizeof(float);
+        EESEN_HIP_CHECK(hipMemsetAsync(L.C.p, 0, blk, st));
+        EESEN_HIP_CHECK(hipMemsetAsync(L.Y.p, 0, blk, st));
+        EESEN_HIP_CHECK(hipMemsetAsync(L.C.p + (size_t)(T + 1) * S * ldY, 0, blk, st));
+        EESEN_HIP_CHECK(hipMemsetAsync(L.Y.p + (size_t)(T + 1) * S * ldY, 0, blk, st));
+        prepare_dropout(*this, L);
+      }
       if (g_gated) {
         if (gated_rows < rows) {
           const int ti_ = timer.begin(st, 0);
@@ -697,7 +770,7 @@
       }
       Layer* nxt = (&L - layers.data()) + 1 < (long)layers.size() ? &layers[(&L - layers.data()) + 1] : nullptr;
       LstmLayerDev v = lstm_view(*this, L, T);
-      const RecPlan fp = persistent ? lstm_fwd_plan(v) : RecPlan{};
+      const RecPlan fp = fuse_small ? fwd[li_] : persistent ? lstm_fwd_plan(v) : RecPlan{};
       const bool pers = fp.kind != kRecNone;
       const bool plan_gate = pers && overlap && gate_fwd && !fwd_bf16 && !L.cur_fwd_drop && fp.units <= 8 && nxt && nxt->is_lstm() && T >= 2 && rows >= 128 &&
                              fp.one_window &&
@@ -709,13 +782,13 @@
       v.poll_delay = delay_fwd;
       v.poll_raw = poll_raw;
       if (plan_mid) {
-        mile.reserve(32);
-        EESEN_HIP_CHECK(hipMemsetAsync(mile.p, 0, 2 * sizeof(unsigned), st));
+        if (!fuse_small) EESEN_HIP_CHECK(hipMemsetAsync(mile_slot(L), 0, 2 * sizeof(unsigned), st));
         EESEN_HIP_CHECK(hipEventRecord(ev_gate_reset, st));
-        v.milestone = mile.p;
+        v.milestone = mile_slot(L);
         v.milestone_step = mile_step;
       }
-      if (pers) lstm_fwd_launch(st, fp, v, ctl.p, ctl.p + kCtlWords - 1, spin_limit, trace.p, plan_gate ? ev_gate_reset : nullptr);
+      if (pers) lstm_fwd_launch(st, fp, v, ctl_slot(false, L), err_word(), spin_limit, trace.p, plan_gate ? ev_gate_reset : nullptr,
+                                fuse_small && rec_plan_counts_once(fp));
       else
         for (int step = 0; step < T; ++step) lstm_fwd_step(st, v, step);
       info_fwd_persistent += pers ? 1 : 0;
@@ -728,7 +801,7 @@
         nxt->G.reserve((size_t)rows * ldG2);
         EESEN_HIP_CHECK(hipStreamWaitEvent(st2, ev_gate_reset, 0));
         const int tj_ = timer.begin(st2, 0);
-        GemmGate gate{ctl.p, ctl.p + kCtlWords - 1, nd, fp.seq_tiles, fp.grid[0], T, S, spin_limit};
+        GemmGate gate{ctl_slot(false, L), err_word(), nd, fp.seq_tiles, fp.grid[0], T, S, spin_limit};
         gated_rows = rows / 128 * 128;
         gemm_f32_nt_gated(st2, gated_rows, ldG2, ldY, L.Y.p + (size_t)S * ldY, ldY, params.p + nxt->p_off + nxt->off_wx, pad4(nxt->din),
                           nxt->G.p, ldG2, params.p + nxt->p_off + nxt->off_bias, gate, half ? bound_one() : GemmBound{}, half ? GemmBound{nxt->bw.rows.p, 1} : GemmBound{});
@@ -737,7 +810,7 @@
         g_gated = true;
       }
       if (plan_mid) {
-        EESEN_HIP_CHECK(hipMemsetD32Async(reinterpret_cast<hipDeviceptr_t>(mile.p + 1), 1, 1, st));
+        EESEN_HIP_CHECK(hipMemsetD32Async(reinterpret_cast<hipDeviceptr_t>(mile_slot(L) + 1), 1, 1, st));
         const int ldG2 = nxt->ndir * 4 * nxt->H;
         nxt->G.reserve((size_t)rows * ldG2);
         mid_r0 = ((T - 1 - mile_step) * S + 255) / 256 * 256;
@@ -747,7 +820,7 @@
       if (plan_mid && mid_r1 > mid_r0) {
         const int ldG2 = nxt->ndir * 4 * nxt->H;
         EESEN_HIP_CHECK(hipStreamWaitEvent(st2, ev_gate_reset, 0));
-        wait_for_word(st2, mile.p + 1, 1u, ctl.p + kCtlWords - 1, 2.0 * std::max(1.0, T / 1000.0) * std::max(1.0, spin_limit / 400000.0));
+        wait_for_word(st2, mile_slot(L) + 1, 1u, err_word(), 2.0 * std::max(1.0, T / 1000.0) * std::max(1.0, spin_limit / 400000.0));
         const int tj_ = timer.begin(st2, 0);
         gemm_f32(st2, true, true, mid_r1 - mid_r0, ldG2, nxt->din, 1.f, L.Y.p + (size_t)S * ldY + (size_t)mid_r0 * ldY, ldY,
                  params.p + nxt->p_off + nxt->off_wx, pad4(nxt->din), 0.f, nxt->G.p + (size_t)mid_r0 * ldG2, ldG2,
@@ -855,7 +928,30 @@
   int ld_d = pad4(Kout);
   float* dn = dB.p;
   const bool half = gemm_mode() == 2;
-  ensure_weight_amax();
+  std::vector<size_t> px_off(layers.size(), 0);
+  size_t px_total = 0;
+  for (size_t li = 0; li < layers.size(); ++li) { px_off[li] = px_total; px_total += bwd[li].need_px; }
+  if (px_total) bwd_px.reserve(px_total);
+  if (fuse_small) {
+    FillList fills(st);
+    ensure_weight_amax(&fills);
+    for (size_t li = 0; li < layers.size(); ++li) {
+      Layer& L = layers[li];
+      if (rec_plan_counts_once(bwd[li])) {
+        fills.add(ctl_slot(true, L), bwd[li].ctl_words * sizeof(unsigned));
+        if (bwd[li].need_px) fills.add(bwd_px.p + px_off[li], bwd[li].need_px * sizeof(float));
+      }
+      if (half && (L.is_lstm() || L.kind == EESEN_LAYER_AFFINE)) {
+        const int cols = L.is_lstm() ? L.ndir * 4 * L.H : L.dout;
+        reserve_bounds(rows, cols, L.bd.rows, L.bd.cols);
+        if (amax_rows_accumulate(cols, pad4(cols))) fills.add(L.bd.rows.p, (size_t)rows * sizeof(float));
+      }
+    }
+    fills.launch();
+    ensure_weight_amax_run();
+  } else {
+    ensure_weight_amax();
+  }
   auto x_cols = [&](int li) -> GemmBound {
     if (!half || !amx_valid) return GemmBound{};
     return x_is_bounded(li) ? bound_one() : GemmBound{layers[li].bx.cols.p, 1};
@@ -864,8 +960,11 @@
     EESEN_HIP_CHECK(hipMemsetAsync(d, 0, (size_t)rows * ld_d * sizeof(float), st));
     for (int b = 0; b < Lb.out_nb; ++b) copy2d(st, out_diff + (size_t)b * Lb.out_hf, ldd, d + (size_t)b * Lb.out_hi, ld_d, rows, Lb.out_hf);
   } else {
-    if (ld_d != Kout) EESEN_HIP_CHECK(hipMemsetAsync(d, 0, (size_t)rows * ld_d * sizeof(float), st));
-    copy2d(st, out_diff, ldd, d, ld_d, rows, Kout);
+    if (ld_d != Kout && fuse_small) copy2d_pad(st, out_diff, ldd, d, ld_d, rows, Kout);
+    else {
+      if (ld_d != Kout) EESEN_HIP_CHECK(hipMemsetAsync(d, 0, (size_t)rows * ld_d * sizeof(float), st));
+      copy2d(st, out_diff, ldd, d, ld_d, rows, Kout);
+    }
   }
 
   for (int li = (int)layers.size() - 1; li >= 0; --li) {
@@ -890,7 +989,7 @@
       continue;
     } else if (L.kind == EESEN_LAYER_AFFINE) {
       { const int ti_ = timer.begin(st, 4);
-      if (half) measure(d, rows, L.dout, ld_d, L.bd.rows, L.bd.cols);
+      if (half) measure(d, rows, L.dout, ld_d, L.bd.rows, L.bd.cols, fuse_small && ld_d == pad4(L.dout));
       if (want_in) {
         if (ld_n != L.din) EESEN_HIP_CHECK(hipMemsetAsync(dn, 0, (size_t)rows * ld_n * sizeof(float), st));
         gemm_f32(st, true, false, rows, L.din, L.dout, 1.f, d, ld_d, params.p + L.p_off + L.off_w, pad4(L.din), 0.f, dn, ld_n,
@@ -907,7 +1006,7 @@
       v.poll_delay = overlap ? delay_bwd_side : delay_bwd;
       v.poll_raw = poll_raw;
       const RecPlan& bp = bwd[li];
-      if (bp.need_px) { bwd_px.reserve(bp.need_px); v.PX = bwd_px.p; v.px_floats = bwd_px.cap; }
+      if (bp.need_px) { v.PX = bwd_px.p + px_off[li]; v.px_floats = bp.need_px; }
       if (bp.need_dgh) {
         bwd_dgh.reserve((size_t)rows * ldG);
         bwd_ex.reserve(bp.need_ex);
@@ -923,13 +1022,14 @@
       }
       { const int ti_ = timer.begin(st, 3);
       if (bp.kind != kRecNone) {
-        lstm_bwd_launch(st, bp, v, d, ld_d, DGl, ctl.p + kCtlHalf, ctl.p + kCtlWords - 1, spin_limit, trace.p ? trace.p + 640 : nullptr);
+        lstm_bwd_launch(st, bp, v, d, ld_d, DGl, ctl_slot(true, L), err_word(), spin_limit, trace.p ? trace.p + 640 : nullptr,
+                        fuse_small && rec_plan_counts_once(bp));
         ++info_bwd_persistent;
       } else
         for (int step = 0; step < T; ++step) lstm_bwd_step(st, v, step, d, ld_d, DGl, DCF.p);
       check_launch("lstm_bwd");
       timer.end(st, ti_); }
-      if (half) { const int ti_ = timer.begin(st, 4); measure(DGl, rows, ldG, ldG, L.bd.rows, L.bd.cols); timer.end(st, ti_); }
+      if (half) { const int ti_ = timer.begin(st, 4); measure(DGl, rows, ldG, ldG, L.bd.rows, L.bd.cols, fuse_small); timer.end(st, ti_); }
       EESEN_HIP_CHECK(hipEventRecord(ev_rec, st));
       if (want_in) {
         const int ti_ = timer.begin(st, 4);
@@ -1032,7 +1132,7 @@
 void Net::update() {
   EESEN_REQUIRE(finalized, EESEN_ERR_STATE, "net not finalized");
   EESEN_HIP_CHECK(hipSetDevice(device));
-  const unsigned* skip = persistent && !grads_sanitized ? ctl.p + kCtlWords - 1 : nullptr;
+  const unsigned* skip = persistent && !grads_sanitized ? err_word() : nullptr;
   const float* live = comm && live_valid ? fresh.p + P : nullptr;
   comm_check_alive(comm);
   { const int ti_ = timer.begin(st, 5);
diff --git a/eesen_amd/csrc/net.h b/eesen_amd/csrc/net.h
--- a/eesen_amd/csrc/net.h
+++ b/eesen_amd/csrc/net.h
@@ -15,6 +15,7 @@
   float coef = 1.f, max_grad = 0.f;
   size_t p_off = 0, p_n = 0;
   int H = 0, ndir = 0;
+  int lstm_index = 0;
   int din_f = 0, dout_f = 0, Hf = 0;
   int in_nb = 0, in_hf = 0, in_hi = 0, out_nb = 0, out_hf = 0, out_hi = 0;
   int in_col(int d) const { return in_nb ? (d / in_hf) * in_hi + d % in_hf : d; }
@@ -105,6 +106,12 @@
   bool fwd_bf16_rec = false;
   int info_fwd_bf16 = 0;
   DevBuf<unsigned> ctl;
+  size_t ctl_words = kCtlWords;
+  int n_lstm = 0;
+  unsigned* err_word() const { return ctl.p + ctl_words - 1; }
+  unsigned* ctl_slot(bool backward, const Layer& L) const { return ctl.p + (size_t)((backward ? std::max(1, n_lstm) : 0) + L.lstm_index) * kCtlHalf; }
+  unsigned* mile_slot(const Layer& L) const { return mile.p + (size_t)L.lstm_index * 32; }
+  bool fuse_small = true;
   Tuning tn;
   int persistent = 1;
   int info_fwd_persistent = 0, info_bwd_persistent = 0, info_lstm_layers = 0;
@@ -136,8 +143,11 @@
   float* am_wm(int li) { return amax.p + 1 + li; }
   GemmBound bound_one() const { return GemmBound{amax.p, 0}; }
   bool x_is_bounded(int li) const;
-  void measure(const float* P, long rows, int cols, int ld, DevBuf<float>& out_rows, DevBuf<float>& out_cols);
-  void ensure_weight_amax();
+  void measure(const float* P, long rows, int cols, int ld, DevBuf<float>& out_rows, DevBuf<float>& out_cols, bool rows_zeroed = false);
+  void reserve_bounds(long rows, int cols, DevBuf<float>& out_rows, DevBuf<float>& out_cols);
+  void ensure_weight_amax(FillList* fills = nullptr);
+  void ensure_weight_amax_run();
+  std::vector<AmaxJob> wjobs;
   PhaseTimer timer;
   Comm* comm = nullptr;
   std::vector<hipEvent_t> ev_ready, ev_bucket;
diff --git a/eesen_amd/csrc/optim.hip b/eesen_amd/csrc/optim.hip
--- a/eesen_amd/csrc/optim.hip
+++ b/eesen_amd/csrc/optim.hip
@@ -86,6 +86,66 @@
   }
 }
 
+__global__ __launch_bounds__(256) void copy2d_pad_kernel(const float* __restrict__ src, int lds, float* __restrict__ dst,
+                                                         int ldd, int rows, int cols) {
+  const size_t total = (size_t)rows * ldd;
+  for (size_t i = (size_t)blockIdx.x * blockDim.x + threadIdx.x; i < total; i += (size_t)gridDim.x * blockDim.x) {
+    const size_t r = i / ldd, c = i % ldd;
+    dst[i] = c < (size_t)cols ? src[r * lds + c] : 0.f;
+  }
+}
+
+struct FillArgs {
+  FillList::Region r[FillList::kMax];
+  int n;
+};
+__global__ __launch_bounds__(256) void fill_regions_kernel(const FillArgs a) {
+  const int bid = (int)blockIdx.x;
+  FillList::Region g = a.r[0];
+#pragma unroll
+  for (int i = 1; i < FillList::kMax; ++i)
+    if (i < a.n && bid >= a.r[i].block0) g = a.r[i];
+  unsigned* w = static_cast<unsigned*>(g.p);
+  const size_t n = g.bytes >> 2;
+  const size_t lead = ((16u - (unsigned)(reinterpret_cast<size_t>(g.p) & 15u)) & 15u) >> 2;
+  const size_t head = lead < n ? lead : n;
+  const size_t n4 = (n - head) >> 2, done = head + (n4 << 2);
+  const int b = bid - g.block0;
+  if (b == 0 && threadIdx.x < head) w[threadIdx.x] = g.value;
+  if (b == 0 && threadIdx.x < n - done) w[done + threadIdx.x] = g.value;
+  uint4* q = reinterpret_cast<uint4*>(w + head);
+  const uint4 v = make_uint4(g.value, g.value, g.value, g.value);
+  for (size_t i = (size_t)b * 256 + threadIdx.x; i < n4; i += (size_t)g.blocks * 256) q[i] = v;
+}
+
+constexpr int kTransposeJobs = 32;
+struct TransposeArgs {
+  struct Job { const float* src; float* dst; int rows, cols, block0, pad_; } j[kTransposeJobs];
+  int n;
+};
+__global__ __launch_bounds__(256) void transpose2d_multi_kernel(const TransposeArgs a) {
+  __shared__ float tile[32][33];
+  const int bid = (int)blockIdx.x;
+  TransposeArgs::Job g = a.j[0];
+#pragma unroll
+  for (int i = 1; i < kTransposeJobs; ++i)
+    if (i < a.n && bid >= a.j[i].block0) g = a.j[i];
+  const int bx = (g.cols + 31) / 32, b = bid - g.block0;
+  const int tx = threadIdx.x & 31, ty = threadIdx.x >> 5;
+  const int c0 = (b % bx) * 32, r0 = (b / bx) * 32;
+#pragma unroll
+  for (int i = 0; i < 32; i += 8) {
+    const int r = r0 + ty + i, c = c0 + tx;
+    if (r < g.rows && c < g.cols) tile[ty + i][tx] = g.src[(size_t)r * g.cols + c];
+  }
+  __syncthreads();
+#pragma unroll
+  for (int i = 0; i < 32; i += 8) {
+    const int c = c0 + ty + i, r = r0 + tx;
+    if (r < g.rows && c < g.cols) g.dst[(size_t)c * g.rows + r] = tile[tx][ty + i];
+  }
+}
+
 }
 
 void sgd_update(hipStream_t st, float* param, float* corr, const float* fresh, long n, float mmt, float lr_coef,
@@ -124,6 +184,49 @@
   check_launch("copy2d");
 }
 
+void copy2d_pad(hipStream_t st, const float* src, int lds, float* dst, int ldd, int rows, int cols) {
+  if (rows <= 0 || ldd <= 0) return;
+  const size_t total = (size_t)rows * ldd;
+  const int blocks = (int)std::min<size_t>((total + 255) / 256, 4096);
+  hipLaunchKernelGGL(copy2d_pad_kernel, dim3(blocks), dim3(256), 0, st, src, lds, dst, ldd, rows, cols);
+  check_launch("copy2d_pad");
+}
+
+void FillList::add(void* p, size_t bytes, unsigned value) {
+  if (!p || bytes == 0) return;
+  EESEN_REQUIRE((reinterpret_cast<size_t>(p) & 3) == 0 && (bytes & 3) == 0, EESEN_ERR_INVALID, "fill: a region is whole 32-bit words");
+  if (n_ == kMax) launch();
+  const int blocks = (int)std::min<size_t>(256, (bytes + 16383) / 16384);
+  r_[n_++] = Region{p, bytes, value, blocks_, blocks};
+  blocks_ += blocks;
+}
+
+void FillList::launch() {
+  if (n_ == 0) return;
+  FillArgs a;
+  std::copy(r_, r_ + n_, a.r);
+  for (int i = n_; i < kMax; ++i) a.r[i] = Region{nullptr, 0, 0u, 0, 0};
+  a.n = n_;
+  hipLaunchKernelGGL(fill_regions_kernel, dim3(blocks_), dim3(256), 0, st_, a);
+  check_launch("fill_regions");
+  n_ = blocks_ = 0;
+}
+
+void transpose2d_multi(hipStream_t st, const TransposeJob* jobs, int n) {
+  for (int j0 = 0; j0 < n; j0 += kTransposeJobs) {
+    TransposeArgs a{};
+    int blocks = 0;
+    a.n = std::min(kTransposeJobs, n - j0);
+    for (int k = 0; k < a.n; ++k) {
+      const TransposeJob& j = jobs[j0 + k];
+      a.j[k] = TransposeArgs::Job{j.src, j.dst, j.rows, j.cols, blocks, 0};
+      blocks += cdiv(j.cols, 32) * cdiv(j.rows, 32);
+    }
+    if (blocks == 0) continue;
+    hipLaunchKernelGGL(transpose2d_multi_kernel, dim3(blocks), dim3(256), 0, st, a);
+    check_launch("transpose2d_multi");
+  }
+}
 
 namespace {
 __device__ __forceinline__ float hash_uniform(unsigned long long seed, unsigned long long idx) {
diff --git a/eesen_amd/csrc/rec_plan.cpp b/eesen_amd/csrc/rec_plan.cpp
--- a/eesen_amd/csrc/rec_plan.cpp
+++ b/eesen_amd/csrc/rec_plan.cpp
@@ -259,15 +259,16 @@
 }
 
 void lstm_fwd_launch(hipStream_t st, const RecPlan& P, const LstmLayerDev& L0, unsigned* cnt, unsigned* err, int spin_limit,
-                     unsigned long long* trace, hipEvent_t after_reset) {
+                     unsigned long long* trace, hipEvent_t after_reset, bool counters_zeroed) {
   EESEN_REQUIRE(P.kind == kRecFwdBf || P.kind == kRecFwdMux || P.kind == kRecFwdF32, EESEN_ERR_STATE, "not a forward recurrence plan");
+  EESEN_REQUIRE(!counters_zeroed || rec_plan_counts_once(P), EESEN_ERR_STATE, "this forward plan reuses its counters inside the pass: it resets them itself");
   const RecRole role{P.grid[0], P.grid[1], P.grid[2], L0.xcd_map};
   for (int w = 0; w < P.windows; ++w) {
     LstmLayerDev L = L0;
     if (P.kind == kRecFwdMux) { L.s_begin = 0; L.s_count = 0; }
     else { L.s_count = L0.S / P.windows; L.s_begin = w * L.s_count; }
     if (P.kind != kRecFwdMux && P.wgs_per_cu >= 2 && !L0.poll_raw) L.poll_delay = L0.poll_delay * 7 / 4;
-    EESEN_HIP_CHECK(hipMemsetAsync(cnt, 0, sizeof(unsigned) * P.ctl_words, st));
+    if (!counters_zeroed) EESEN_HIP_CHECK(hipMemsetAsync(cnt, 0, sizeof(unsigned) * P.ctl_words, st));
     if (after_reset && P.one_window) EESEN_HIP_CHECK(hipEventRecord(after_reset, st));
     if (P.kind == kRecFwdMux) plan_launch(st, P.fn, P.wgs, L, cnt, err, spin_limit, role);
     else plan_launch(st, P.fn, P.wgs, L, cnt, err, spin_limit, trace, role);
@@ -348,7 +349,8 @@
 }
 
 void lstm_bwd_launch(hipStream_t st, const RecPlan& P, const LstmLayerDev& L0, const float* dY, int lddy, float* DG, unsigned* cnt,
-                     unsigned* err, int spin_limit, unsigned long long* trace) {
+                     unsigned* err, int spin_limit, unsigned long long* trace, bool zeroed) {
+  EESEN_REQUIRE(!zeroed || rec_plan_counts_once(P), EESEN_ERR_STATE, "this backward plan reuses its counters inside the pass: it resets them itself");
   EESEN_REQUIRE(P.kind == kRecBwdQ4 || P.kind == kRecBwdKsplit || P.kind == kRecBwdKsplitMux || P.kind == kRecBwdGeneric, EESEN_ERR_STATE, "not a backward recurrence plan");
   EESEN_REQUIRE(!P.need_px || (L0.PX && L0.px_floats >= P.need_px), EESEN_ERR_STATE, "the backward plan's partial-sum exchange space (RecPlan::need_px) was not handed over");
   EESEN_REQUIRE(!P.need_dgh || (L0.DGH && L0.EX), EESEN_ERR_STATE, "the backward plan's plane and exponent buffers (RecPlan::need_dgh, need_ex) were not handed over");
@@ -360,8 +362,10 @@
     LstmLayerDev L = L0;
     if (whole_batch) { L.s_begin = 0; L.s_count = 0; }
     else { L.s_count = L0.S / P.windows; L.s_begin = w * L.s_count; }
-    EESEN_HIP_CHECK(hipMemsetAsync(cnt, 0, sizeof(unsigned) * P.ctl_words, st));
-    if (P.need_px) EESEN_HIP_CHECK(hipMemsetAsync(L.PX, 0, sizeof(float) * P.need_px, st));
+    if (!zeroed) {
+      EESEN_HIP_CHECK(hipMemsetAsync(cnt, 0, sizeof(unsigned) * P.ctl_words, st));
+      if (P.need_px) EESEN_HIP_CHECK(hipMemsetAsync(L.PX, 0, sizeof(float) * P.need_px, st));
+    }
     if (P.kind == kRecBwdQ4) plan_launch(st, P.fn, P.wgs, L, dY, lddy, DG, cnt, err, spin_limit, trace, role);
     else if (P.kind == kRecBwdKsplitMux) plan_launch(st, P.fn, P.wgs, L, dY, lddy, DG, px, cnt, err, spin_limit, role, chunk);
     else if (P.kind == kRecBwdKsplit) plan_launch(st, P.fn, P.wgs, L, dY, lddy, DG, px, cnt, err, spin_limit, role, chunk, trace);
diff --git a/eesen_amd/csrc/tuning.h b/eesen_amd/csrc/tuning.h
--- a/eesen_amd/csrc/tuning.h
+++ b/eesen_amd/csrc/tuning.h
@@ -8,7 +8,7 @@
   int overlap = -1, gate_fwd = -1, side_lds_kb = -1;
   int spin_limit = 400000;
   bool spin_limit_set = false;
-  int bwd_q4 = 1, bwd_q4_st8 = 1, fwd_narrow2 = 1, fwd_t16_small = 1, bwd_ksplit = 1, fwd_mux = 1, bwd_mux = 1, xcd_map = 1, fwd_mid = 1, fwd_split = 1, fwd_f16 = 1, bwd_f16 = 1;
+  int bwd_q4 = 1, bwd_q4_st8 = 1, fwd_narrow2 = 1, fwd_t16_small = 1, bwd_ksplit = 1, fwd_mux = 1, bwd_mux = 1, xcd_map = 1, fwd_mid = 1, fwd_split = 1, fwd_f16 = 1, bwd_f16 = 1, fuse_small = 1;
   int comm_defer = -1;
   int trace = 0;
   bool print_flight = false;
@@ -38,6 +38,7 @@
     t.fwd_f16 = num("EESEN_FWD_F16", 1);
     t.bwd_f16 = num("EESEN_BWD_F16", 1);
     t.xcd_map = num("EESEN_XCD_MAP", 1);
+    t.fuse_small = num("EESEN_FUSE_SMALL", 1);
     t.comm_defer = num("EESEN_COMM_DEFER", -1);
     t.trace = num("EESEN_TRACE", 0);
     t.print_flight = getenv("EESEN_PRINT_FLIGHT") != nullptr;
```
